# facebookresearch/robust_cvd

Hardware: NVIDIA H100
Metric: flow_residual_constraints_per_sec_per_gn_iteration (higher is better)
Workload: dtype f64

## Files before the change

include/rcvd_hooks.h:

```cpp
#ifndef RCVD_HOOKS_H_
#define RCVD_HOOKS_H_
#include "rcvd.h"
#ifdef __cplusplus
extern "C" {
#endif

int64_t rcvd_launch_count(rcvd_problem* p);
int64_t rcvd_filter_launch_count(void);
int64_t rcvd_builder_launch_count(void);
int64_t rcvd_static_flag_launch_count(void);
int64_t rcvd_builder_last_rounds(void);

int32_t rcvd_structure_info(rcvd_problem* p, int32_t out[8]);

int32_t rcvd_debug_factor_plan(const rcvd_config* cfg, int32_t np, const int32_t* pairs, int32_t nt, const int32_t* trip_centers,
                               int32_t order_slack, int32_t nranks, int32_t rank, int32_t num_sms,
                               int32_t* order, int32_t* level, int32_t* owner, int32_t* perm, int32_t out[12]);

int32_t rcvd_debug_linear_solve(rcvd_problem* p, const double* S, const double* D2, const double* b, double* y);

int32_t rcvd_debug_solve_matrix(rcvd_problem* p, const double* H, const double* D2, const double* b, double* y);
int32_t rcvd_debug_factor_dense(rcvd_problem* p, int32_t* order, double* L, double* Linv);
int32_t rcvd_debug_linear_paths(rcvd_problem* p, int64_t out[13]);

int32_t rcvd_debug_linear_residual(rcvd_problem* p, double radius, double out[6]);

int32_t rcvd_debug_last_iteration(rcvd_problem* p, double* g, double* xc, double out[2]);

int32_t rcvd_debug_profile_linear(rcvd_problem* p, int32_t reps, double out_ms[8]);
int32_t rcvd_debug_level_profile(rcvd_problem* p, double* out, int32_t max_levels);
int32_t rcvd_debug_fp64_tensor_peak(int32_t device, int32_t shape, double* tflops);

int32_t rcvd_debug_set_fast_path(rcvd_problem* p, int32_t on);
int32_t rcvd_debug_set_overlap(rcvd_problem* p, int32_t on);
int32_t rcvd_debug_set_order_slack(rcvd_problem* p, int32_t slack);
int32_t rcvd_debug_set_eval_only(rcvd_problem* p, int32_t on);
int32_t rcvd_debug_set_distributed(rcvd_problem* p, int32_t on);
int32_t rcvd_distribution_info(rcvd_problem* p, int32_t out[4]);
int32_t rcvd_debug_set_update_kernel(rcvd_problem* p, int32_t tma, int32_t side_items_per_cta);

#ifdef __cplusplus
}
#endif
#endif
```

robust_cvd_b200/csrc/rcvd_api.cu:

```cuda
#include <algorithm>
#include <chrono>
#include <cmath>
#include <cstdarg>
#include <cstdio>
#include <cstring>
#include <dlfcn.h>
#include <limits>
#include <string>
#include <vector>

#include <cub/device/device_segmented_sort.cuh>
#include "rcvd_eval.cuh"
#include "rcvd_linalg.cuh"
#include "rcvd_update.cuh"
#include "rcvd_plan.h"
#include "rcvd_dense.cuh"
#include "rcvd_filter.cuh"
#include "rcvd_bilateral.cuh"
#include "rcvd_builder.cuh"
static int64_t g_filter_launches = 0;

using namespace rcvd;

#define RCVD_API extern "C" __attribute__((visibility("default")))

constexpr int kFastSmem = (3 * kTile * kJsLd + 4 * 256) * (int)sizeof(double);
static bool run_path_ok_host(const rcvd_config& c, const Layout& L);
static bool fast_path_ok_host(const rcvd_config& c, const Layout& L) {
  return L.k == 1 && c.spatial_type == RCVD_SPATIAL_IDENTITY && c.intr_opt != RCVD_INTR_SHARED && !c.fix_poses && !c.fix_depth_xforms &&
         !c.fix_spatial_xforms && (c.depth_type != RCVD_DEPTH_GRID || !c.depth_cubic);
}

static bool run_path_ok_host(const rcvd_config& c, const Layout& L) { return fast_path_ok_host(c, L) && c.depth_type == RCVD_DEPTH_GRID && L.G < 65535; }

static thread_local std::string g_err = "";
static int set_err(int code, const char* fmt, ...) {
  char buf[512]; va_list ap; va_start(ap, fmt); vsnprintf(buf, sizeof(buf), fmt, ap); va_end(ap);
  g_err = buf; return code;
}
#define CK(call) do { cudaError_t e_ = (call); if (e_ != cudaSuccess) return set_err(RCVD_ERR_CUDA, "%s failed: %s (%s:%d)", #call, cudaGetErrorString(e_), __FILE__, __LINE__); } while (0)

struct DevGuard {
  int prev = -1; cudaError_t err = cudaSuccess;
  explicit DevGuard(int d) { if (cudaGetDevice(&prev) != cudaSuccess) prev = -1; err = cudaSetDevice(d); }
  ~DevGuard() { if (prev >= 0) cudaSetDevice(prev); }
};
#define SET_DEVICE(d) DevGuard dev_guard_(d); if (dev_guard_.err != cudaSuccess) return set_err(RCVD_ERR_CUDA, "cudaSetDevice(%d) failed: %s", (int)(d), cudaGetErrorString(dev_guard_.err))

namespace nccl {
typedef struct { char internal[128]; } UniqueId;
typedef void* Comm;
static void* lib = nullptr;
static int (*GetUniqueId)(UniqueId*) = nullptr;
static int (*CommInitRank)(Comm*, int, UniqueId, int) = nullptr;
static int (*AllReduce)(const void*, void*, size_t, int, int, Comm, cudaStream_t) = nullptr;
static int (*CommDestroy)(Comm) = nullptr;
static const char* (*GetErrorString)(int) = nullptr;
static int (*GroupStart)() = nullptr;
static int (*GroupEnd)() = nullptr;
static int (*Broadcast)(const void*, void*, size_t, int, int, Comm, cudaStream_t) = nullptr;
static int (*Reduce)(const void*, void*, size_t, int, int, int, Comm, cudaStream_t) = nullptr;
static bool load() {
  if (lib) return true;
  const char* names[] = {"libnccl.so.2", "libnccl.so"};
  for (const char* n : names) { lib = dlopen(n, RTLD_NOW | RTLD_GLOBAL); if (lib) break; }
  if (!lib) return false;
  GetUniqueId = (int (*)(UniqueId*))dlsym(lib, "ncclGetUniqueId");
  CommInitRank = (int (*)(Comm*, int, UniqueId, int))dlsym(lib, "ncclCommInitRank");
  AllReduce = (int (*)(const void*, void*, size_t, int, int, Comm, cudaStream_t))dlsym(lib, "ncclAllReduce");
  CommDestroy = (int (*)(Comm))dlsym(lib, "ncclCommDestroy");
  GetErrorString = (const char* (*)(int))dlsym(lib, "ncclGetErrorString");
  GroupStart = (int (*)())dlsym(lib, "ncclGroupStart"); GroupEnd = (int (*)())dlsym(lib, "ncclGroupEnd");
  Broadcast = (int (*)(const void*, void*, size_t, int, int, Comm, cudaStream_t))dlsym(lib, "ncclBroadcast");
  Reduce = (int (*)(const void*, void*, size_t, int, int, int, Comm, cudaStream_t))dlsym(lib, "ncclReduce");
  return GetUniqueId && CommInitRank && AllReduce && CommDestroy && GroupStart && GroupEnd && Broadcast && Reduce;
}
constexpr int kFloat64 = 8, kUint8 = 1, kSum = 0, kMax = 2;
}

enum { SC_COST = 0, SC_CAND = 1, SC_GY = 2, SC_YHY = 3, SC_STEP2 = 4, SC_X2 = 5, SC_GMAX = 6, SC_GDOTD = 7, SC_DMAX = 8, SC_N = 16 };

__global__ void k_extract_diag(const double* __restrict__ H, double* __restrict__ diag, int N, int npad) {
  const int i = blockIdx.x * blockDim.x + threadIdx.x;
  if (i >= N * npad) return;
  const int f = i / npad, l = i % npad;
  diag[i] = H[(size_t)f * npad * npad + (size_t)l * npad + l];
}
__global__ void k_jacobi_scale(const double* __restrict__ diag, double* __restrict__ S, int n, int enable) {
  const int i = blockIdx.x * blockDim.x + threadIdx.x;
  if (i < n) S[i] = enable ? 1.0 / (1.0 + sqrt(diag[i])) : 1.0;
}
__global__ void k_lm_prepare(const double* __restrict__ diagH, const double* __restrict__ S, const double* __restrict__ g, double* __restrict__ lmdiag,
                             double* __restrict__ D2, double* __restrict__ gs, int n, int reuse, double radius, double dmin, double dmax) {
  const int i = blockIdx.x * blockDim.x + threadIdx.x;
  if (i >= n) return;
  const double s = S[i];
  double d = lmdiag[i];
  if (!reuse) { d = fmin(fmax(s * s * diagH[i], dmin), dmax); lmdiag[i] = d; }
  D2[i] = d / radius;
  gs[i] = s * g[i];
}
__global__ void k_mul(const double* __restrict__ a, const double* __restrict__ b, double* __restrict__ o, int n) {
  const int i = blockIdx.x * blockDim.x + threadIdx.x;
  if (i < n) o[i] = a[i] * b[i];
}
__device__ __forceinline__ double project_lb(const rcvd_config& c, const Layout& L, const uint8_t* in_range, int f, int l, double v) {
  if (c.depth_lower_bound && l >= L.offD && l < L.offS && ((l - L.offD) % L.k) == 0 && in_range[f]) return fmax(v, 0.0);
  return v;
}
__global__ void __launch_bounds__(256) k_state_norms(rcvd_config cfg, Layout L, const uint8_t* __restrict__ in_range, const uint8_t* __restrict__ active,
                                                      const double* __restrict__ x, const double* __restrict__ g, double* __restrict__ scal, int N) {
  const int i = blockIdx.x * blockDim.x + threadIdx.x;
  double x2 = 0.0, gm = 0.0;
  if (i < N * L.nf) {
    const int f = i / L.nf, l = i % L.nf;
    const size_t v = (size_t)f * L.npad + l;
    if (active[v]) {
      x2 = x[i] * x[i];
      gm = fabs(x[i] - project_lb(cfg, L, in_range, f, l, x[i] - g[v]));
    }
  }
  x2 = warp_sum(x2);
#pragma unroll
  for (int o = 16; o > 0; o >>= 1) gm = fmax(gm, __shfl_xor_sync(0xffffffffu, gm, o));
  if ((threadIdx.x & 31) == 0) {
    red_add(scal + SC_X2, x2);
    atomicMax((unsigned long long*)(scal + SC_GMAX), (unsigned long long)__double_as_longlong(gm));
  }
}
__global__ void __launch_bounds__(256) k_dot2(const double* __restrict__ a, const double* __restrict__ b, const double* __restrict__ c,
                                               const double* __restrict__ d, int n, double* __restrict__ scal, int s0, int s1) {
  const int i = blockIdx.x * blockDim.x + threadIdx.x;
  double p = 0.0, q = 0.0;
  if (i < n) { p = a[i] * b[i]; q = c[i] * d[i]; }
  p = warp_sum(p); q = warp_sum(q);
  if ((threadIdx.x & 31) == 0) { red_add(scal + s0, p); red_add(scal + s1, q); }
}
__global__ void k_finalize_mask(rcvd_config cfg, Layout L, uint8_t* __restrict__ mask, int N) {
  const int i = blockIdx.x * blockDim.x + threadIdx.x;
  if (i >= N * L.npad) return;
  const int l = i % L.npad;
  if (l >= L.nf || is_const_local(cfg, L, l)) mask[i] = 0;
}
__global__ void k_project_state(rcvd_config cfg, Layout L, const uint8_t* __restrict__ in_range, double* __restrict__ x, int N) {
  const int i = blockIdx.x * blockDim.x + threadIdx.x;
  if (i < N * L.nf) x[i] = project_lb(cfg, L, in_range, i / L.nf, i % L.nf, x[i]);
}
__global__ void k_h_to_dense(const double* __restrict__ H, const HBlock* __restrict__ hb, int nblocks, double* __restrict__ out, int N, int nf, int npad, const int* __restrict__ uperm) {
  const int b = blockIdx.y;
  const int e = blockIdx.x * blockDim.x + threadIdx.x;
  if (e >= nf * nf) return;
  const int i = e / nf, j = e % nf;
  const HBlock hbk = hb[b];
  if (hbk.r == hbk.c && j > i) return;
  const double v = H[(size_t)b * npad * npad + (size_t)i * npad + j];
  const size_t U = (size_t)N * nf;
  const int ur = uperm[hbk.r], uc = uperm[hbk.c];
  out[((size_t)ur * nf + i) * U + (size_t)uc * nf + j] = v;
  out[((size_t)uc * nf + j) * U + (size_t)ur * nf + i] = v;
}

enum { LP_POTRF_SMEM = 0, LP_POTRF_PANEL, LP_TRSM_LL4, LP_TRSM_LL2, LP_TRSM_GEMM, LP_UPD_TMA1, LP_UPD_TMA2, LP_UPD_GEMM, LP_SUB_LEVEL, LP_SUB_FUSED,
       LP_TRINV, LP_OTHER, LP_UPD_TMA1_MULTI, LP_N };

struct rcvd_problem {
  rcvd_config cfg; Layout L; int N = 0; int device = 0;
  cudaStream_t stream = nullptr;
  std::vector<uint8_t> in_range; std::vector<double> median, adaptive;
  std::vector<int32_t> pair_frames; std::vector<int64_t> offsets; std::vector<float> records_h;
  std::vector<int32_t> struct_pairs;
  std::vector<int32_t> trip_centers; std::vector<int64_t> trip_offsets; std::vector<float> trip_records;
  float* d_trip_records = nullptr; int32_t *d_trip_tile_center = nullptr, *d_trip_tile_count = nullptr; int64_t* d_trip_tile_begin = nullptr; int num_trip_tiles = 0;
  int first_frame = 0, last_frame = -1;
  float* d_records = nullptr; int32_t *d_tile_pair = nullptr, *d_tile_count = nullptr, *d_pair_frames = nullptr, *d_blk_of = nullptr;
  int64_t* d_tile_begin = nullptr; uint8_t *d_in_range = nullptr, *d_active = nullptr;
  double *d_median = nullptr, *d_adaptive = nullptr; float* d_scale_locs = nullptr; int nscale = 0;
  int num_tiles = 0; int64_t C = 0;
  double *d_x = nullptr, *d_xc = nullptr, *d_xsave = nullptr;
  double *d_g = nullptr, *d_S = nullptr, *d_diagH = nullptr, *d_lmdiag = nullptr, *d_D2 = nullptr, *d_gs = nullptr, *d_rhs = nullptr, *d_ytmp = nullptr,
         *d_y = nullptr, *d_Sy = nullptr, *d_Hy = nullptr, *d_partial = nullptr, *d_scal = nullptr;
  double* h_scal = nullptr;
  int npartial = 0;
  double *d_H = nullptr, *d_Lb = nullptr, *d_T = nullptr, *d_invL = nullptr, *d_invT = nullptr;
  HBlock *d_hblocks = nullptr, *d_lblocks = nullptr; int* d_fail = nullptr;
  FactorPlan plan;
  int *d_lvl_frames = nullptr; GemmTask *d_trsm_tasks = nullptr, *d_upd_tasks = nullptr; int2 *d_trsm_pairs = nullptr, *d_upd_pairs = nullptr;
  SubTask* d_sub_tasks = nullptr; int* d_sub_counters = nullptr; int* d_sub_need = nullptr;
  SolveTask* d_fwd_tasks = nullptr; TrsmTask* d_trsm_ll = nullptr; bool use_trsm_ll = false;
  cudaGraphExec_t solve_graph = nullptr;
  bool structure_ready = false, constraints_set = false, frames_set = false;
  int nranks = 1, rank = 0; nccl::Comm comm = nullptr;
  int64_t launches = 0, graph_launches = 0;
  std::vector<double> h_state; bool state_dirty = false; bool use_fast = true; bool overlap = true; int order_slack = 4;
  cudaStream_t side_stream = nullptr; cudaEvent_t ev_fork = nullptr, ev_join = nullptr;
  double *d_g2 = nullptr, *d_delta = nullptr; int* h_fail = nullptr;
  cudaEvent_t ev[8] = {nullptr};
  std::vector<void*> allocs;
  std::vector<std::pair<int, cudaEvent_t>>* prof = nullptr;
  bool eval_only = false;
  bool records_sorted = false;
  bool dist_enabled = true, graph_warm = false, force_full_H = false;
  int *d_lvl_own = nullptr, *d_own_lblocks = nullptr, *d_own_hblocks = nullptr, *d_uperm = nullptr;
  UpdItem* d_upd_items = nullptr; CUtensorMap tmapT; bool gemm_tma = true, tmap_ok = false; int num_sms = 0, upd_ipc = 0;
  std::vector<double> level_ms;
  bool factored = false;
  int64_t paths[LP_N] = {0}, graph_paths[LP_N] = {0};
  rcvd_problem() {}
};

template <class T> static int dalloc(rcvd_problem* p, T** ptr, size_t count) {
  *ptr = nullptr;
  if (count == 0) count = 1;
  cudaError_t e = cudaMallocAsync((void**)ptr, count * sizeof(T), p->stream);
  if (e != cudaSuccess) return set_err(RCVD_ERR_CUDA, "cudaMallocAsync(%zu bytes) failed: %s", count * sizeof(T), cudaGetErrorString(e));
  p->allocs.push_back(*ptr);
  return RCVD_OK;
}
template <class T> static int upload(rcvd_problem* p, T** ptr, const std::vector<T>& v) {
  int rc = dalloc(p, ptr, v.size()); if (rc) return rc;
  if (!v.empty()) CK(cudaMemcpyAsync(*ptr, v.data(), v.size() * sizeof(T), cudaMemcpyHostToDevice, p->stream));
  return RCVD_OK;
}
static void free_all(rcvd_problem* p) {
  if (p->solve_graph) { cudaGraphExecDestroy(p->solve_graph); p->solve_graph = nullptr; }
  if (p->side_stream) cudaStreamSynchronize(p->side_stream);
  for (void* q : p->allocs) cudaFreeAsync(q, p->stream);
  p->allocs.clear();
  if (p->stream) cudaStreamSynchronize(p->stream);
  if (p->h_scal) { cudaFreeHost(p->h_scal); p->h_scal = nullptr; }
  p->structure_ready = false; p->factored = false;
}

static DevProblem dev_problem(const rcvd_problem* p) {
  DevProblem d; d.cfg = p->cfg; d.L = p->L; d.N = p->N; d.num_tiles = p->num_tiles; d.num_constraints = p->C;
  d.records = p->d_records; d.tile_pair = p->d_tile_pair; d.tile_begin = p->d_tile_begin; d.tile_count = p->d_tile_count;
  d.pair_frames = p->d_pair_frames; d.blk_of = p->d_blk_of; d.in_range = p->d_in_range; d.median = p->d_median;
  d.adaptive = p->adaptive.empty() ? nullptr : p->d_adaptive; d.scale_locs = p->d_scale_locs; d.num_scale_locs = p->nscale;
  d.rank = p->rank; d.nranks = p->nranks;
  d.trip_records = p->d_trip_records; d.trip_tile_center = p->d_trip_tile_center; d.trip_tile_begin = p->d_trip_tile_begin; d.trip_tile_count = p->d_trip_tile_count; d.num_trip_tiles = p->num_trip_tiles;
  return d;
}

#define UP(ptr, vec) if ((rc = upload(p, &(ptr), vec))) return rc
#define DA(ptr, n) if ((rc = dalloc(p, &(ptr), (n)))) return rc
static int upload_plan(rcvd_problem* p) {
  const FactorPlan& pl = p->plan; int rc;
  UP(p->d_blk_of, pl.blk_of); UP(p->d_hblocks, pl.hblocks); UP(p->d_lblocks, pl.lblocks); UP(p->d_lvl_frames, pl.lvl_frames); UP(p->d_lvl_own, pl.lvl_own);
  UP(p->d_own_lblocks, pl.own_lblocks); UP(p->d_own_hblocks, pl.own_hblocks); UP(p->d_uperm, pl.uperm);
  UP(p->d_trsm_tasks, pl.trsm_tasks); UP(p->d_upd_tasks, pl.upd_tasks); UP(p->d_trsm_pairs, pl.trsm_pairs); UP(p->d_upd_pairs, pl.upd_pairs);
  UP(p->d_sub_tasks, pl.sub_tasks); UP(p->d_sub_need, pl.sub_need); DA(p->d_sub_counters, (size_t)4 * p->N + 4);
  UP(p->d_fwd_tasks, pl.fwd_tasks); UP(p->d_trsm_ll, pl.trsm_ll); UP(p->d_upd_items, pl.upd_items);
  return RCVD_OK;
}

static int set_up_problem_data(rcvd_problem* p) {
  const int N = p->N; const Layout& L = p->L; const std::vector<int>& uperm = p->plan.uperm; int rc;
  const int np = (int)(p->pair_frames.size() / 2);
  std::vector<int32_t> tile_pair, tile_count; std::vector<int64_t> tile_begin;
  for (int i = 0; i < np; ++i)
    for (int64_t b = p->offsets[i]; b < p->offsets[i + 1]; b += kTile) { tile_pair.push_back(i); tile_begin.push_back(b); tile_count.push_back((int32_t)std::min<int64_t>(kTile, p->offsets[i + 1] - b)); }
  p->num_tiles = (int)tile_pair.size(); p->C = p->offsets.empty() ? 0 : p->offsets.back();
  UP(p->d_tile_pair, tile_pair); UP(p->d_tile_begin, tile_begin); UP(p->d_tile_count, tile_count);
  {
    std::vector<int32_t> pf_int(p->pair_frames.size());
    for (size_t i = 0; i < pf_int.size(); ++i) pf_int[i] = p->plan.iperm[p->pair_frames[i]];
    UP(p->d_pair_frames, pf_int); UP(p->d_records, p->records_h);
  }
  p->records_sorted = false;
  if (run_path_ok_host(p->cfg, L) && p->C > 0 && p->C < (int64_t)0x7fffffff) {
    const long long n = p->C;
    unsigned *d_k0 = nullptr, *d_k1 = nullptr; int *d_i0 = nullptr, *d_i1 = nullptr; float* d_sorted = nullptr; int64_t* d_off = nullptr; void* d_tmp = nullptr;
    int rcs;
    if ((rcs = dalloc(p, &d_k0, (size_t)n)) || (rcs = dalloc(p, &d_k1, (size_t)n)) || (rcs = dalloc(p, &d_i0, (size_t)n)) || (rcs = dalloc(p, &d_i1, (size_t)n)) || (rcs = dalloc(p, &d_sorted, (size_t)n * 6)) ||
        (rcs = upload(p, &d_off, p->offsets))) return rcs;
    k_record_keys<<<(unsigned)((n + 255) / 256), 256, 0, p->stream>>>(p->cfg, p->d_records, n, d_k0, d_i0);
    size_t tmp_bytes = 0;
    CK(cub::DeviceSegmentedSort::SortPairs(nullptr, tmp_bytes, d_k0, d_k1, d_i0, d_i1, (int)n, np, d_off, d_off + 1, p->stream));
    CK(cudaMallocAsync(&d_tmp, std::max<size_t>(tmp_bytes, 16), p->stream));
    CK(cub::DeviceSegmentedSort::SortPairs(d_tmp, tmp_bytes, d_k0, d_k1, d_i0, d_i1, (int)n, np, d_off, d_off + 1, p->stream));
    k_gather_records<<<(unsigned)((n * 6 + 255) / 256), 256, 0, p->stream>>>(p->d_records, d_i1, n, d_sorted);
    CK(cudaFreeAsync(d_tmp, p->stream));
    CK(cudaGetLastError());
    p->d_records = d_sorted; p->records_sorted = true;
  }
  {
    std::vector<int32_t> tc, tn; std::vector<int64_t> tb;
    for (size_t i = 0; i < p->trip_centers.size(); ++i)
      for (int64_t b = p->trip_offsets[i]; b < p->trip_offsets[i + 1]; b += kTile) { tc.push_back(p->trip_centers[i]); tb.push_back(b); tn.push_back((int32_t)std::min<int64_t>(kTile, p->trip_offsets[i + 1] - b)); }
    p->num_trip_tiles = (int)tc.size();
    UP(p->d_trip_tile_center, tc); UP(p->d_trip_tile_begin, tb); UP(p->d_trip_tile_count, tn); UP(p->d_trip_records, p->trip_records);
  }
  {
    std::vector<uint8_t> ir(N); std::vector<double> md(N), ad;
    for (int i = 0; i < N; ++i) { ir[i] = p->in_range[uperm[i]]; md[i] = p->median[uperm[i]]; }
    UP(p->d_in_range, ir); UP(p->d_median, md);
    if (!p->adaptive.empty()) {
      const size_t G = p->adaptive.size() / N; ad.resize(p->adaptive.size());
      for (int i = 0; i < N; ++i) std::copy(p->adaptive.begin() + (size_t)uperm[i] * G, p->adaptive.begin() + (size_t)(uperm[i] + 1) * G, ad.begin() + (size_t)i * G);
      UP(p->d_adaptive, ad);
    }
  }
  {
    std::vector<float> locs; const int gx = p->cfg.scale_grid_x, gy = p->cfg.scale_grid_y;
    for (int y = 0; y < gy; ++y) for (int x = 0; x < gx; ++x) {
      const float fx = -1.f + 2.f * x / (gx - 1);
      const float fy = -1.f + 2.f * y / (gy - 1);
      locs.push_back(fx); locs.push_back(fy);
    }
    p->nscale = (int)(locs.size() / 2);
    UP(p->d_scale_locs, locs);
  }
  p->first_frame = 0; p->last_frame = -1;
  { bool any = false; for (int f = 0; f < N; ++f) if (p->in_range[f]) { if (!any) { p->first_frame = f; any = true; } p->last_frame = f; } }
  return RCVD_OK;
}
#undef UP

static int allocate_storage(rcvd_problem* p) {
  const int N = p->N; const Layout& L = p->L; const int npad = L.npad, nLoff = p->plan.nLoff; const size_t bs = (size_t)npad * npad; int rc;
  const size_t Upad = (size_t)N * npad, U = (size_t)N * L.nf;
  DA(p->d_x, U); DA(p->d_xc, U); DA(p->d_xsave, U);
  DA(p->d_g, 2 * Upad + 8); p->d_diagH = p->d_g + Upad + 8;
  DA(p->d_S, Upad); DA(p->d_lmdiag, Upad); DA(p->d_D2, Upad); DA(p->d_gs, Upad); DA(p->d_rhs, Upad);
  DA(p->d_g2, Upad + 8); DA(p->d_delta, Upad);
  DA(p->d_ytmp, Upad); DA(p->d_y, Upad); DA(p->d_Sy, Upad); DA(p->d_Hy, Upad); DA(p->d_scal, SC_N); DA(p->d_active, Upad); DA(p->d_fail, 1);
  const RegCounts rcn = reg_counts(p->cfg, L, N, p->nscale);
  p->npartial = p->num_tiles + (rcn.total + 127) / 128 + p->num_trip_tiles + 1;
  DA(p->d_partial, (size_t)p->npartial);
  if (p->eval_only) { DA(p->d_H, 1); DA(p->d_Lb, 1); DA(p->d_T, 1); DA(p->d_invL, 1); DA(p->d_invT, 1); }
  else {
    DA(p->d_H, p->plan.hblocks.size() * bs); DA(p->d_Lb, (size_t)(N + nLoff) * bs); DA(p->d_T, (size_t)std::max(nLoff, 1) * bs);
    DA(p->d_invL, (size_t)N * bs); DA(p->d_invT, (size_t)N * npad * 16);
  }
#undef DA
  {
    p->tmap_ok = false;
    typedef CUresult (*EncodeFn)(CUtensorMap*, CUtensorMapDataType, cuuint32_t, void*, const cuuint64_t*, const cuuint64_t*, const cuuint32_t*, const cuuint32_t*,
                                 CUtensorMapInterleave, CUtensorMapSwizzle, CUtensorMapL2promotion, CUtensorMapFloatOOBfill);
    void* fn = nullptr; cudaDriverEntryPointQueryResult qres;
    if (cudaGetDriverEntryPoint("cuTensorMapEncodeTiled", &fn, cudaEnableDefault, &qres) == cudaSuccess && fn && qres == cudaDriverEntryPointSuccess) {
      const cuuint64_t gdim[2] = {(cuuint64_t)npad, (cuuint64_t)std::max(nLoff, 1) * npad};
      const cuuint64_t gstr[1] = {(cuuint64_t)npad * sizeof(double)};
      const cuuint32_t box[2] = {16u, (cuuint32_t)p->plan.upd_rb};
      const cuuint32_t estr[2] = {1u, 1u};
      const CUresult r = ((EncodeFn)fn)(&p->tmapT, CU_TENSOR_MAP_DATA_TYPE_FLOAT64, 2, p->d_T, gdim, gstr, box, estr, CU_TENSOR_MAP_INTERLEAVE_NONE,
                                        CU_TENSOR_MAP_SWIZZLE_128B, CU_TENSOR_MAP_L2_PROMOTION_L2_128B, CU_TENSOR_MAP_FLOAT_OOB_FILL_NONE);
      p->tmap_ok = (r == CUDA_SUCCESS);
    }
    cudaGetLastError();
    if (p->tmap_ok) { CK(cudaFuncSetAttribute(k_update_tma<1>, cudaFuncAttributeMaxDynamicSharedMemorySize, (int)upd_smem_bytes(p->plan.upd_rb, 1))); CK(cudaFuncSetAttribute(k_update_tma<2>, cudaFuncAttributeMaxDynamicSharedMemorySize, (int)upd_smem_bytes(p->plan.upd_rb, 2))); }
    else if (p->gemm_tma) return set_err(RCVD_ERR_CUDA, "cuTensorMapEncodeTiled unavailable or failed: the TMA update kernel cannot run");
  }
  CK(cudaMallocHost((void**)&p->h_scal, (SC_N + 2) * sizeof(double)));
  p->h_fail = (int*)(p->h_scal + SC_N);
  CK(cudaMemsetAsync(p->d_x, 0, U * sizeof(double), p->stream));
  CK(cudaMemsetAsync(p->d_lmdiag, 0, Upad * sizeof(double), p->stream));
  CK(cudaMemsetAsync(p->d_S, 0, Upad * sizeof(double), p->stream));
  CK(cudaMemsetAsync(p->d_active, 0, Upad, p->stream));
  DevProblem d = dev_problem(p);
  if (p->num_tiles > 0) k_mark_static<<<p->num_tiles, kTile, 0, p->stream>>>(d, p->d_active);
  if (rcn.total > 0) {
    DevProblem d1 = d; d1.nranks = 1; d1.rank = 0;
    k_regularisers<2><<<(rcn.total + 127) / 128, 128, 0, p->stream>>>(d1, rcn, p->d_x, nullptr, nullptr, nullptr, p->d_active, p->first_frame, p->last_frame);
  }
  if (p->num_trip_tiles > 0) k_triplets<2><<<p->num_trip_tiles, kTile, 0, p->stream>>>(d, p->d_x, nullptr, nullptr, nullptr, p->d_active);
  k_finalize_mask<<<(int)((Upad + 255) / 256), 256, 0, p->stream>>>(p->cfg, L, p->d_active, N);
  CK(cudaGetLastError());
  if (p->nranks > 1) {
    const int r = nccl::AllReduce(p->d_active, p->d_active, Upad, nccl::kUint8, nccl::kMax, p->comm, p->stream);
    if (r != 0) return set_err(RCVD_ERR_NCCL, "ncclAllReduce(active mask) failed");
  }
  if ((npad * 16 + 16 * (npad + 1)) * (int)sizeof(double) > 220 * 1024) return set_err(RCVD_ERR_INVALID, "frame block too large for the panel-inverse kernel (npad=%d)", npad);
  CK(cudaFuncSetAttribute(k_trinv, cudaFuncAttributeMaxDynamicSharedMemorySize, (npad * 16 + 16 * (npad + 1)) * (int)sizeof(double)));
  CK(cudaFuncSetAttribute(k_accumulate_fast, cudaFuncAttributeMaxDynamicSharedMemorySize, kFastSmem));
  CK(cudaFuncSetAttribute(k_accumulate_runs, cudaFuncAttributeMaxDynamicSharedMemorySize, kRunSmem));
  p->use_trsm_ll = trsm_ll_smem_bytes(npad) <= 220 * 1024;
  if (p->use_trsm_ll) { CK(cudaFuncSetAttribute(k_trsm_ll<2>, cudaFuncAttributeMaxDynamicSharedMemorySize, (int)trsm_ll_smem_bytes(npad, 2))); if (trsm_ll_smem_bytes(npad, 4) <= 220 * 1024) CK(cudaFuncSetAttribute(k_trsm_ll<4>, cudaFuncAttributeMaxDynamicSharedMemorySize, (int)trsm_ll_smem_bytes(npad, 4))); }
  if (potrf_smem_bytes(npad) <= 220 * 1024) CK(cudaFuncSetAttribute(k_potrf_smem, cudaFuncAttributeMaxDynamicSharedMemorySize, (int)potrf_smem_bytes(npad)));
  return RCVD_OK;
}

static int build_structure(rcvd_problem* p) {
  free_all(p);
  CK(cudaSetDevice(p->device));
  if (const char* e = make_factor_plan(p->plan, p->cfg, p->struct_pairs.empty() ? p->pair_frames : p->struct_pairs, p->trip_centers, p->order_slack,
                                       p->nranks, p->rank, p->dist_enabled, p->num_sms))
    return set_err(RCVD_ERR_INVALID, "%s", e);
  int rc;
  if ((rc = upload_plan(p)) || (rc = set_up_problem_data(p)) || (rc = allocate_storage(p))) return rc;
  CK(cudaStreamSynchronize(p->stream));
  p->structure_ready = true;
  return RCVD_OK;
}

static int allreduce(rcvd_problem* p, double* buf, size_t count) {
  if (p->nranks <= 1) return RCVD_OK;
  const int r = nccl::AllReduce(buf, buf, count, nccl::kFloat64, nccl::kSum, p->comm, p->stream);
  if (r != 0) return set_err(RCVD_ERR_NCCL, "ncclAllReduce failed: %s", nccl::GetErrorString ? nccl::GetErrorString(r) : "?");
  return RCVD_OK;
}
struct Seg { size_t first, count; };
static int grouped(rcvd_problem* p, double* base, size_t unit, const std::vector<Seg>& segs, bool bcast) {
  int r = nccl::GroupStart();
  for (size_t i = 0; i < segs.size() && r == 0; ++i) {
    if (segs[i].count == 0) continue;
    const int root = (int)(i % (size_t)p->nranks);
    double* ptr = base + segs[i].first * unit;
    r = bcast ? nccl::Broadcast(ptr, ptr, segs[i].count * unit, nccl::kFloat64, root, p->comm, p->stream)
              : nccl::Reduce(ptr, ptr, segs[i].count * unit, nccl::kFloat64, nccl::kSum, root, p->comm, p->stream);
  }
  const int r2 = nccl::GroupEnd();
  if (r == 0) r = r2;
  if (r != 0) return set_err(RCVD_ERR_NCCL, "grouped NCCL %s failed: %s", bcast ? "broadcast" : "reduce", nccl::GetErrorString ? nccl::GetErrorString(r) : "?");
  return RCVD_OK;
}

static int enqueue_factor_solve(rcvd_problem* p) {
  const Layout& L = p->L; const int N = p->N, npad = L.npad; cudaStream_t st = p->stream;
  const int nL = N + p->plan.nLoff;
  const int tiles = (npad + 63) / 64;
  enum { P_LOAD = 0, P_POTRF, P_TRINV, P_TRSM, P_GEMM, P_SOLVE };
  int prof_level = 0;
  auto mark = [&](int cls) {
    if (!p->prof) return;
    cudaEvent_t e; cudaEventCreate(&e); cudaEventRecord(e, st); p->prof->push_back({cls < 0 ? cls : (cls | (prof_level << 8)), e});
  };
  const int neff = std::min(npad, (L.nf + 7) / 8 * 8);
  auto gemm = [&](cudaStream_t cs, int ntasks, double* dstp, const double* A, const double* B, const GemmTask* tasks, const int2* prs, double alpha, double beta) {
    k_gemm_nt<<<dim3(tiles, tiles, ntasks), 128, 0, cs>>>(dstp, A, B, tasks, prs, npad, beta != 0.0 ? neff : npad, alpha, beta);
  };
  mark(-1);
  k_load_factor<<<dim3((npad * npad + 255) / 256, p->plan.dist ? (int)p->plan.own_lblocks.size() : nL), 256, 0, st>>>(p->d_H, p->d_Lb, p->d_lblocks, p->d_S, p->d_D2, npad, L.nf, p->plan.dist ? p->d_own_lblocks : nullptr);
  p->launches += 1; p->paths[LP_OTHER]++; mark(P_LOAD);
  cudaStream_t side = p->side_stream;
  bool side_pending = false, side_used = false;
  const size_t bsz = (size_t)npad * npad;
  auto phase_boundary = [&]() -> int {
    if (side_pending || side_used) { CK(cudaEventRecord(p->ev_join, side)); CK(cudaStreamWaitEvent(st, p->ev_join, 0)); side_pending = false; }
    std::vector<Seg> inv, tr;
    for (int q = 0; q < p->nranks; ++q) inv.push_back({(size_t)p->plan.fa_off[q], (size_t)p->plan.fa_cnt[q]});
    for (int q = 0; q < p->nranks; ++q) tr.push_back({(size_t)p->plan.fb_off[q], (size_t)p->plan.fb_cnt[q]});
    for (int q = 0; q < p->nranks; ++q) tr.push_back({(size_t)N + (size_t)p->plan.bseg[2 * q], (size_t)p->plan.bseg[2 * q + 1]});
    int rc = grouped(p, p->d_invL, bsz, inv, true); if (rc) return rc;
    return grouped(p, p->d_Lb, bsz, tr, true);
  };
  for (size_t li = 0; li < p->plan.levels.size(); ++li) {
    const Level& lv = p->plan.levels[li]; prof_level = (int)li;
    if (p->plan.dist && (int)li == p->plan.LB) { int rc = phase_boundary(); if (rc) return rc; }
    const int* lframes = p->d_lvl_own + lv.own_off; const int nfr = lv.nown;
    if (nfr > 0) {
    if (potrf_smem_bytes(npad) <= 220 * 1024) {
      k_potrf_smem<<<nfr, kPotrfSmemThreads, potrf_smem_bytes(npad), st>>>(p->d_Lb, p->d_invT, lframes, npad, p->d_fail);
      p->paths[LP_POTRF_SMEM]++;
    } else {
      const int nt16 = npad / 16;
      for (int jb = 0; jb < nt16; ++jb) {
        k_potrf_panel<<<nfr, kPotrfThreads, 0, st>>>(p->d_Lb, p->d_invT, lframes, npad, jb, p->d_fail);
        p->launches += 1; p->paths[LP_POTRF_PANEL]++;
        const int m = npad - (jb + 1) * 16;
        if (m > 0) { const int n64 = (m + 63) / 64; k_potrf_trail<<<dim3(n64 * (n64 + 1) / 2, nfr), 128, 0, st>>>(p->d_Lb, lframes, npad, jb); p->launches += 1; p->paths[LP_OTHER]++; }
      }
      p->launches -= 1;
    }
    p->launches += 1; mark(P_POTRF);
    if (p->use_trsm_ll) {
      cudaStream_t is = st;
      if (p->overlap) { CK(cudaEventRecord(p->ev_fork, st)); CK(cudaStreamWaitEvent(side, p->ev_fork, 0)); is = side; side_used = true; }
      k_trinv<<<dim3(npad / 16, nfr), 256, (npad * 16 + 16 * (npad + 1)) * sizeof(double), is>>>(p->d_Lb, p->d_invT, p->d_invL, lframes, npad);
      p->launches += 1; p->paths[LP_TRINV]++; mark(P_TRINV);
      if (lv.ntrsm > 0) {
        const int strips = (npad + kTrsmStrip - 1) / kTrsmStrip;
        if (strips * lv.ntrsm <= p->num_sms && trsm_ll_smem_bytes(npad, 4) <= 220 * 1024) {
          k_trsm_ll<4><<<dim3(strips, lv.ntrsm), 128, trsm_ll_smem_bytes(npad, 4), st>>>(p->d_T, p->d_Lb, p->d_invT, p->d_trsm_ll + lv.trsm_off, npad);
          p->paths[LP_TRSM_LL4]++;
        } else {
          k_trsm_ll<2><<<dim3(strips, lv.ntrsm), 128, trsm_ll_smem_bytes(npad, 2), st>>>(p->d_T, p->d_Lb, p->d_invT, p->d_trsm_ll + lv.trsm_off, npad);
          p->paths[LP_TRSM_LL2]++;
        }
        p->launches++; mark(P_TRSM);
      }
    } else {
      k_trinv<<<dim3(npad / 16, nfr), 256, (npad * 16 + 16 * (npad + 1)) * sizeof(double), st>>>(p->d_Lb, p->d_invT, p->d_invL, lframes, npad);
      p->launches += 1; p->paths[LP_TRINV]++; mark(P_TRINV);
      if (lv.ntrsm > 0) { gemm(st, lv.ntrsm, p->d_T, p->d_Lb, p->d_invL, p->d_trsm_tasks + lv.trsm_off, p->d_trsm_pairs, 1.0, 0.0); p->launches++; p->paths[LP_TRSM_GEMM]++; mark(P_TRSM); }
    }
    }
    if (p->plan.dist && (int)li < p->plan.LB) {
      std::vector<Seg> segs;
      for (int q = 0; q < p->nranks; ++q) segs.push_back({(size_t)p->plan.tseg[(li * p->nranks + q) * 2], (size_t)p->plan.tseg[(li * p->nranks + q) * 2 + 1]});
      int rc = grouped(p, p->d_T, bsz, segs, true); if (rc) return rc;
    }
    if (lv.nupd2 > 0 && p->overlap) {
      CK(cudaEventRecord(p->ev_fork, st)); CK(cudaStreamWaitEvent(side, p->ev_fork, 0));
    }
    if (side_pending) { CK(cudaStreamWaitEvent(st, p->ev_join, 0)); side_pending = false; }
    auto update = [&](cudaStream_t cs, int off, int n) {
      if (n <= p->num_sms) {
        k_update_tma<2><<<n, UpdShape<2>::threads, upd_smem_bytes(p->plan.upd_rb, 2), cs>>>(p->tmapT, p->d_Lb, p->d_upd_items + off, n, p->d_upd_pairs, npad, p->plan.upd_neff, p->plan.upd_rb, 0);
        p->paths[LP_UPD_TMA2]++;
      } else {
        int grid = std::min(n, 2 * p->num_sms);
        if (p->upd_ipc > 0) grid = std::max(grid, (n + p->upd_ipc - 1) / p->upd_ipc);
        k_update_tma<1><<<grid, UpdShape<1>::threads, upd_smem_bytes(p->plan.upd_rb, 1), cs>>>(p->tmapT, p->d_Lb, p->d_upd_items + off, n, p->d_upd_pairs, npad, p->plan.upd_neff, p->plan.upd_rb, 0);
        p->paths[LP_UPD_TMA1]++; if (grid < n) p->paths[LP_UPD_TMA1_MULTI]++;
      }
    };
    if (p->gemm_tma) {
      if (lv.nit > 0) { update(st, lv.it_off, lv.nit); p->launches++; mark(P_GEMM); }
      if (lv.nit2 > 0) {
        update(p->overlap ? side : st, lv.it2_off, lv.nit2); p->launches++; mark(P_GEMM);
        if (p->overlap) { CK(cudaEventRecord(p->ev_join, side)); side_pending = true; side_used = true; }
      }
      continue;
    }
    if (lv.nupd > 0) { gemm(st, lv.nupd, p->d_Lb, p->d_T, p->d_T, p->d_upd_tasks + lv.upd_off, p->d_upd_pairs, -1.0, 1.0); p->launches++; p->paths[LP_UPD_GEMM]++; mark(P_GEMM); }
    if (lv.nupd2 > 0) {
      gemm(p->overlap ? side : st, lv.nupd2, p->d_Lb, p->d_T, p->d_T, p->d_upd_tasks + lv.upd2_off, p->d_upd_pairs, -1.0, 1.0); p->launches++; p->paths[LP_UPD_GEMM]++; mark(P_GEMM);
      if (p->overlap) { CK(cudaEventRecord(p->ev_join, side)); side_pending = true; side_used = true; }
    }
  }
  if (p->plan.dist && p->plan.LB >= (int)p->plan.levels.size()) { int rc = phase_boundary(); if (rc) return rc; }
  if (side_pending || side_used) { CK(cudaEventRecord(p->ev_join, side)); CK(cudaStreamWaitEvent(st, p->ev_join, 0)); }
  CK(cudaMemcpyAsync(p->d_rhs, p->d_gs, (size_t)N * npad * sizeof(double), cudaMemcpyDeviceToDevice, st));
  const int nlv = (int)p->plan.levels.size();
  const int LS = p->plan.sub_first_level;
  for (int l = 0; l < LS; ++l) {
    const Level& lv = p->plan.levels[l];
    k_fwd_diag<<<dim3((npad + 7) / 8, lv.nframes), 256, 0, st>>>(p->d_invL, p->d_rhs, p->d_ytmp, p->d_lvl_frames + lv.frame_off, npad);
    p->launches++; p->paths[LP_SUB_LEVEL]++;
    if (lv.nfwd > 0) { k_fwd_update<<<dim3((npad + 7) / 8, lv.nfwd), 256, 0, st>>>(p->d_T, p->d_ytmp, p->d_rhs, p->d_fwd_tasks + lv.fwd_off, npad); p->launches++; p->paths[LP_SUB_LEVEL]++; }
  }
  if (LS < nlv && !p->plan.sub_tasks.empty()) {
    CK(cudaMemsetAsync(p->d_sub_counters, 0, ((size_t)4 * N + 4) * sizeof(int), st));
    SubCounters cn; cn.ticket = p->d_sub_counters; cn.fin = p->d_sub_counters + 4; cn.fdone = cn.fin + N; cn.bin = cn.fdone + N; cn.bdone = cn.bin + N;
    cn.fin_need = p->d_sub_need; cn.bin_need = p->d_sub_need + N;
    k_substitution<<<std::min((int)p->plan.sub_tasks.size(), p->num_sms), kSubThreads, substitution_smem_bytes(npad), st>>>(p->d_invL, p->d_T, p->d_rhs, p->d_ytmp, p->d_y, p->d_sub_tasks, (int)p->plan.sub_tasks.size(), cn, npad);
    p->launches++; p->paths[LP_SUB_FUSED]++;
  }
  for (int l = LS - 1; l >= 0; --l) {
    const Level& lv = p->plan.levels[l];
    if (lv.nfwd > 0) { k_bwd_update<<<dim3((npad + 31) / 32, lv.nfwd), 256, 0, st>>>(p->d_T, p->d_y, p->d_ytmp, p->d_fwd_tasks + lv.fwd_off, npad); p->launches++; p->paths[LP_SUB_LEVEL]++; }
    k_bwd_diag<<<dim3((npad + 31) / 32, lv.nframes), 256, 0, st>>>(p->d_invL, p->d_ytmp, p->d_y, p->d_lvl_frames + lv.frame_off, npad);
    p->launches += 1; p->paths[LP_SUB_LEVEL]++;
  }
  mark(P_SOLVE);
  CK(cudaGetLastError());
  return RCVD_OK;
}

static int factor_solve(rcvd_problem* p) {
  if (p->nranks > 1 && !p->graph_warm) {
    p->graph_warm = true; p->factored = true;
    return enqueue_factor_solve(p);
  }
  if (!p->solve_graph) {
    cudaGraph_t graph;
    const int64_t l0 = p->launches;
    int64_t paths0[LP_N]; std::copy(p->paths, p->paths + LP_N, paths0);
    CK(cudaStreamBeginCapture(p->stream, cudaStreamCaptureModeThreadLocal));
    int rc = enqueue_factor_solve(p);
    cudaError_t e = cudaStreamEndCapture(p->stream, &graph);
    for (int i = 0; i < LP_N; ++i) { p->graph_paths[i] = p->paths[i] - paths0[i]; p->paths[i] = paths0[i]; }
    if (rc) return rc;
    if (e != cudaSuccess) return set_err(RCVD_ERR_CUDA, "graph capture failed: %s", cudaGetErrorString(e));
    CK(cudaGraphInstantiate(&p->solve_graph, graph, 0));
    cudaGraphDestroy(graph);
    p->graph_launches = p->launches - l0;
    p->launches = l0;
  }
  CK(cudaGraphLaunch(p->solve_graph, p->stream));
  p->launches += p->graph_launches;
  for (int i = 0; i < LP_N; ++i) p->paths[i] += p->graph_paths[i];
  p->factored = true;
  return RCVD_OK;
}


static int enqueue_evaluate(rcvd_problem* p, const double* x, bool wantG, bool wantH, double* gout, int slot) {
  if (wantH && p->eval_only) return set_err(RCVD_ERR_INVALID, "this handle was set to evaluation-only (rcvd_debug_set_eval_only): no normal matrix");
  const Layout& L = p->L; const int N = p->N, npad = L.npad; cudaStream_t st = p->stream;
  const size_t bs = (size_t)npad * npad, Upad = (size_t)N * npad;
  DevProblem d = dev_problem(p);
  const RegCounts rcn = reg_counts(p->cfg, L, N, p->nscale);
  const int regblocks = (rcn.total + 127) / 128;
  if (wantH) CK(cudaMemsetAsync(p->d_H, 0, p->plan.hblocks.size() * bs * sizeof(double), st));
  if (wantG) CK(cudaMemsetAsync(gout, 0, (Upad + 8) * sizeof(double), st));
  if (p->num_tiles > 0) {
    if (wantH && p->use_fast && p->records_sorted) k_accumulate_runs<<<p->num_tiles, kTile, kRunSmem, st>>>(d, x, p->d_H, gout, p->d_partial);
    else if (wantH && p->use_fast && fast_path_ok_host(p->cfg, L)) k_accumulate_fast<<<p->num_tiles, kTile, kFastSmem, st>>>(d, x, p->d_H, gout, p->d_partial);
    else if (wantH) k_accumulate_generic<true><<<p->num_tiles, kTile, 0, st>>>(d, x, p->d_H, gout, p->d_partial);
    else if (wantG) k_accumulate_generic<false><<<p->num_tiles, kTile, 0, st>>>(d, x, nullptr, gout, p->d_partial);
    else k_cost_static<<<p->num_tiles, kTile, 0, st>>>(d, x, p->d_partial);
    p->launches++;
  }
  if (regblocks > 0) {
    double* part = p->d_partial + p->num_tiles;
    if (wantH) k_regularisers<1><<<regblocks, 128, 0, st>>>(d, rcn, x, p->d_H, gout, part, nullptr, p->first_frame, p->last_frame);
    else if (wantG) k_regularisers<3><<<regblocks, 128, 0, st>>>(d, rcn, x, nullptr, gout, part, nullptr, p->first_frame, p->last_frame);
    else k_regularisers<0><<<regblocks, 128, 0, st>>>(d, rcn, x, nullptr, nullptr, part, nullptr, p->first_frame, p->last_frame);
    p->launches++;
  }
  if (p->num_trip_tiles > 0) {
    double* part = p->d_partial + p->num_tiles + regblocks;
    if (wantH) k_triplets<1><<<p->num_trip_tiles, kTile, 0, st>>>(d, x, p->d_H, gout, part, nullptr);
    else if (wantG) k_triplets<3><<<p->num_trip_tiles, kTile, 0, st>>>(d, x, nullptr, gout, part, nullptr);
    else k_triplets<0><<<p->num_trip_tiles, kTile, 0, st>>>(d, x, nullptr, nullptr, part, nullptr);
    p->launches++;
  }
  k_reduce_partials<<<1, 1024, 0, st>>>(p->d_partial, p->num_tiles + regblocks + p->num_trip_tiles, p->d_scal, slot);
  p->launches++;
  CK(cudaGetLastError());
  if (p->nranks > 1) {
    int rc;
    if (wantG) {
      CK(cudaMemcpyAsync(gout + Upad, p->d_scal + slot, sizeof(double), cudaMemcpyDeviceToDevice, st));
      size_t cnt = Upad + 8;
      if (wantH && gout == p->d_g) { k_extract_diag<<<(int)((Upad + 255) / 256), 256, 0, st>>>(p->d_H, p->d_diagH, N, npad); p->launches++; cnt = 2 * Upad + 8; }
      if ((rc = allreduce(p, gout, cnt))) return rc;
      CK(cudaMemcpyAsync(p->d_scal + slot, gout + Upad, sizeof(double), cudaMemcpyDeviceToDevice, st));
    } else if ((rc = allreduce(p, p->d_scal + slot, 1))) return rc;
    if (wantH) {
      if (p->plan.dist && !p->force_full_H) {
        std::vector<Seg> segs;
        for (int q = 0; q < p->nranks; ++q) segs.push_back({(size_t)p->plan.fa_off[q], (size_t)(p->plan.fa_cnt[q] + p->plan.fb_cnt[q])});
        for (int q = 0; q < p->nranks; ++q) segs.push_back({(size_t)p->plan.hseg[2 * q], (size_t)p->plan.hseg[2 * q + 1]});
        if ((rc = grouped(p, p->d_H, bs, segs, false))) return rc;
      } else if ((rc = allreduce(p, p->d_H, p->plan.hblocks.size() * bs))) return rc;
    }
  }
  return RCVD_OK;
}

static int upload_frames(rcvd_problem* p, double* dst, const double* src_user, int stride_dst, int stride_src, int count) {
  std::vector<double> tmp((size_t)p->N * stride_dst, 0.0);
  for (int i = 0; i < p->N; ++i) memcpy(tmp.data() + (size_t)i * stride_dst, src_user + (size_t)p->plan.uperm[i] * stride_src, (size_t)count * sizeof(double));
  CK(cudaMemcpyAsync(dst, tmp.data(), tmp.size() * sizeof(double), cudaMemcpyHostToDevice, p->stream));
  CK(cudaStreamSynchronize(p->stream));
  return RCVD_OK;
}
static int download_frames(rcvd_problem* p, double* dst_user, const double* src, int stride_dst, int stride_src, int count) {
  std::vector<double> tmp((size_t)p->N * stride_src);
  CK(cudaMemcpyAsync(tmp.data(), src, tmp.size() * sizeof(double), cudaMemcpyDeviceToHost, p->stream));
  CK(cudaStreamSynchronize(p->stream));
  for (int i = 0; i < p->N; ++i) memcpy(dst_user + (size_t)p->plan.uperm[i] * stride_dst, tmp.data() + (size_t)i * stride_src, (size_t)count * sizeof(double));
  return RCVD_OK;
}
static int save_state(rcvd_problem* p) {
  DevGuard g(p->device); cudaStreamSynchronize(p->stream);
  if (p->h_state.size() != (size_t)p->N * p->L.nf) p->h_state.assign((size_t)p->N * p->L.nf, 0.0);
  return download_frames(p, p->h_state.data(), p->d_x, p->L.nf, p->L.nf, p->L.nf);
}

static int ensure_ready(rcvd_problem* p) {
  if (!p->structure_ready) {
    if (p->offsets.empty()) { p->offsets.assign(1, 0); }
    if (p->in_range.empty()) p->in_range.assign(p->N, 1);
    if (p->median.empty()) p->median.assign(p->N, 1.0);
    int rc = build_structure(p); if (rc) return rc;
    p->state_dirty = true;
  }
  if (p->state_dirty) {
    if (p->h_state.size() != (size_t)p->N * p->L.nf) p->h_state.assign((size_t)p->N * p->L.nf, 0.0);
    { int rc = upload_frames(p, p->d_x, p->h_state.data(), p->L.nf, p->L.nf, p->L.nf); if (rc) return rc; }
    p->state_dirty = false;
  }
  return RCVD_OK;
}

static int read_scalars(rcvd_problem* p) {
  CK(cudaMemcpyAsync(p->h_scal, p->d_scal, SC_N * sizeof(double), cudaMemcpyDeviceToHost, p->stream));
  CK(cudaMemcpyAsync(p->h_fail, p->d_fail, sizeof(int), cudaMemcpyDeviceToHost, p->stream));
  CK(cudaStreamSynchronize(p->stream));
  return RCVD_OK;
}

// ... 125 lines not shown
  CK(cudaMemcpyAsync(p->d_xsave, p->d_x, U * sizeof(double), cudaMemcpyDeviceToDevice, st));

  auto full_eval = [&]() -> int {
    CK(cudaMemsetAsync(p->d_scal, 0, SC_N * sizeof(double), st));
    CK(cudaEventRecord(p->ev[0], st));
    int r = enqueue_evaluate(p, p->d_x, true, true, p->d_g, SC_COST); if (r) return r;
    CK(cudaEventRecord(p->ev[1], st));
    if (p->nranks <= 1) k_extract_diag<<<nblk(Upad), 256, 0, st>>>(p->d_H, p->d_diagH, N, npad);
    k_state_norms<<<nblk(U), 256, 0, st>>>(p->cfg, L, p->d_in_range, p->d_active, p->d_x, p->d_g, p->d_scal, N);
    p->launches += 2;
    r = read_scalars(p); if (r) return r;
    sum.eval_ms += ev_ms(p->ev[0], p->ev[1]);
    return RCVD_OK;
  };
  if ((rc = full_eval())) return rc;
  double xCost = p->h_scal[SC_COST], xNorm = std::sqrt(p->h_scal[SC_X2]), gmax = p->h_scal[SC_GMAX];
  sum.initial_cost = xCost;
  k_jacobi_scale<<<nblk(Upad), 256, 0, st>>>(p->d_diagH, p->d_S, (int)Upad, o.jacobi_scaling);
  p->launches++;
  double radius = o.initial_radius, decrease = 2.0; bool reuseDiag = false;
  double minimumCost = xCost;
  int iter = 0, invalid = 0; bool stepSuccessful = true;
  auto finish = [&](int term, const char* msg) { sum.termination = term; snprintf(sum.message, sizeof(sum.message), "%s", msg); };
  finish(RCVD_TERM_NO_CONVERGENCE, "");
  if (o.verbose) fprintf(stderr, "[rcvd] iter      cost      cost_change  |gradient|   |step|    tr_ratio  tr_radius\n[rcvd] %4d %.6e %10.2e %10.2e %10.2e %10.2e %10.2e\n", 0, xCost, 0.0, gmax, 0.0, 0.0, radius);
  for (;;) {
    if (stepSuccessful) {
      ++sum.num_successful_steps;
      if (xCost < minimumCost || iter == 0) { minimumCost = xCost; CK(cudaMemcpyAsync(p->d_xsave, p->d_x, U * sizeof(double), cudaMemcpyDeviceToDevice, st)); }
    } else ++sum.num_unsuccessful_steps;
    if (iter >= o.max_iterations) { finish(RCVD_TERM_NO_CONVERGENCE, "Maximum number of iterations reached."); break; }
    if (stepSuccessful && gmax <= o.gradient_tolerance) { finish(RCVD_TERM_CONVERGENCE, "Gradient tolerance reached."); break; }
    if (radius <= o.min_radius) { finish(RCVD_TERM_CONVERGENCE, "Minimum trust region radius reached."); break; }
    ++iter; stepSuccessful = false;
    CK(cudaMemsetAsync(p->d_scal, 0, SC_N * sizeof(double), st));
    CK(cudaMemsetAsync(p->d_fail, 0, sizeof(int), st));
    CK(cudaEventRecord(p->ev[2], st));
    k_lm_prepare<<<nblk(Upad), 256, 0, st>>>(p->d_diagH, p->d_S, p->d_g, p->d_lmdiag, p->d_D2, p->d_gs, (int)Upad, reuseDiag ? 1 : 0, radius, o.min_lm_diagonal, o.max_lm_diagonal);
    p->launches++;
    reuseDiag = true;
    if ((rc = factor_solve(p))) return rc;
    if ((rc = enqueue_model_terms(p))) return rc;
    CK(cudaEventRecord(p->ev[3], st));
    double alpha = 1.0;
    if (!constrained) {
      if ((rc = enqueue_candidate(p, 1.0, p->d_g))) return rc;
      if ((rc = enqueue_evaluate(p, p->d_xc, false, false, nullptr, SC_CAND))) return rc;
      CK(cudaEventRecord(p->ev[4], st));
    }
    if ((rc = read_scalars(p))) return rc;
    sum.linear_ms += ev_ms(p->ev[2], p->ev[3]);
    if (!constrained) sum.cost_ms += ev_ms(p->ev[3], p->ev[4]);
    const double gy = p->h_scal[SC_GY], yHy = p->h_scal[SC_YHY];
    const double modelChange = gy - 0.5 * yHy;
    const bool ok = (*p->h_fail == 0) && std::isfinite(gy) && std::isfinite(yHy);
    if (!(ok && modelChange > 0.0)) {
      if (++invalid >= o.max_consecutive_invalid_steps) { finish(RCVD_TERM_FAILURE, "Number of consecutive invalid steps more than max_num_consecutive_invalid_steps."); break; }
      radius = radius / decrease; decrease *= 2.0; reuseDiag = true;
      if (o.verbose) fprintf(stderr, "[rcvd] %4d invalid step (fail=%d model=%g), radius %.3e\n", iter, *p->h_fail, modelChange, radius);
      continue;
    }
    invalid = 0;
    if (constrained) {
      auto trial = [&](double a, ls::Sample& s) -> int {
        CK(cudaMemsetAsync(p->d_scal, 0, SC_N * sizeof(double), st));
        int r = enqueue_candidate(p, a, p->d_g); if (r) return r;
        r = enqueue_evaluate(p, p->d_xc, true, false, p->d_g2, SC_CAND); if (r) return r;
        k_dot2<<<nblk(Upad), 256, 0, st>>>(p->d_g2, p->d_delta, p->d_g2, p->d_delta, (int)Upad, p->d_scal, SC_GY, SC_YHY);
        p->launches++;
        r = read_scalars(p); if (r) return r;
        s.x = a; s.value = p->h_scal[SC_CAND]; s.valueValid = std::isfinite(s.value);
        s.gradient = p->h_scal[SC_GY]; s.gradValid = s.valueValid && std::isfinite(s.gradient);
        return RCVD_OK;
      };
      ls::Sample cur, prev{0, 0, 0, false, false};
      if ((rc = trial(1.0, cur))) return rc;
      const double gd = p->h_scal[SC_GDOTD], dirMax = p->h_scal[SC_DMAX];
      ls::Sample init{0.0, xCost, gd, true, true};
      int lsIter = 0; bool success = true;
      while (!cur.valueValid || cur.value > xCost + 1e-4 * gd * cur.x) {
        if (++lsIter >= 20) { success = false; break; }
        const double lo = 1e-3 * cur.x, hi = 0.6 * cur.x;
        double ss;
        if (!cur.valueValid) ss = std::min(std::max(cur.x * 0.5, lo), hi);
        else { std::vector<ls::Sample> sm{init, cur}; if (prev.valueValid) sm.push_back(prev); ss = ls::minimizeInterpolating(sm, lo, hi); }
        if (ss * dirMax < 1e-9) { success = false; break; }
        prev = cur;
        if ((rc = trial(ss, cur))) return rc;
      }
      alpha = success ? cur.x : 1.0;
      CK(cudaMemsetAsync(p->d_scal, 0, SC_N * sizeof(double), st));
      if ((rc = enqueue_candidate(p, alpha, p->d_g))) return rc;
      if ((rc = enqueue_evaluate(p, p->d_xc, false, false, nullptr, SC_CAND))) return rc;
      if ((rc = read_scalars(p))) return rc;
    }
    double candCost = p->h_scal[SC_CAND];
    if (!std::isfinite(candCost)) candCost = std::numeric_limits<double>::max();
    const double stepNorm = std::sqrt(p->h_scal[SC_STEP2]);
    if (stepNorm <= o.parameter_tolerance * (xNorm + o.parameter_tolerance)) { finish(RCVD_TERM_CONVERGENCE, "Parameter tolerance reached."); break; }
    const double costChange = xCost - candCost;
    if (std::fabs(costChange) <= o.function_tolerance * xCost) { finish(RCVD_TERM_CONVERGENCE, "Function tolerance reached."); break; }
    const double relDecrease = (candCost >= std::numeric_limits<double>::max()) ? std::numeric_limits<double>::lowest() : costChange / modelChange;
    if (relDecrease > o.min_relative_decrease) {
      std::swap(p->d_x, p->d_xc);
      if ((rc = full_eval())) return rc;
      xCost = p->h_scal[SC_COST]; xNorm = std::sqrt(p->h_scal[SC_X2]); gmax = p->h_scal[SC_GMAX];
      stepSuccessful = true;
      radius = radius / std::max(1.0 / 3.0, 1.0 - std::pow(2.0 * relDecrease - 1.0, 3));
      radius = std::min(o.max_radius, radius); decrease = 2.0; reuseDiag = false;
    } else {
      radius = radius / decrease; decrease *= 2.0; reuseDiag = true;
    }
    if (o.verbose) fprintf(stderr, "[rcvd] %4d %.6e %10.2e %10.2e %10.2e %10.2e %10.2e\n", iter, stepSuccessful ? xCost : candCost, costChange, gmax, stepNorm, relDecrease, radius);
  }
  CK(cudaMemcpyAsync(p->d_x, p->d_xsave, U * sizeof(double), cudaMemcpyDeviceToDevice, st));
  CK(cudaStreamSynchronize(st));
  sum.iterations = iter; sum.final_cost = minimumCost;
  sum.gpu_launches = p->launches - launches0;
  sum.total_ms = std::chrono::duration<double, std::milli>(clk::now() - t0).count();
  return RCVD_OK;
}

RCVD_API const char* rcvd_last_error(void) { return g_err.c_str(); }
RCVD_API int32_t rcvd_abi_version(void) { return 1; }
RCVD_API int32_t rcvd_frame_stride(const rcvd_config* c) { Layout L; return (c && make_layout(*c, L)) ? L.nf : -1; }
RCVD_API int32_t rcvd_depth_param_offset(const rcvd_config* c) { Layout L; return (c && make_layout(*c, L)) ? L.offD : -1; }
RCVD_API int32_t rcvd_spatial_param_offset(const rcvd_config* c) { Layout L; return (c && make_layout(*c, L)) ? L.offS : -1; }
RCVD_API void rcvd_default_solve_options(rcvd_solve_options* o) {
  o->max_iterations = 1000; o->verbose = 0; o->function_tolerance = 1e-6; o->gradient_tolerance = 1e-10; o->parameter_tolerance = 1e-8;
  o->initial_radius = 1e4; o->max_radius = 1e16; o->min_radius = 1e-32; o->min_relative_decrease = 1e-3; o->min_lm_diagonal = 1e-6;
  o->max_lm_diagonal = 1e32; o->max_consecutive_invalid_steps = 5; o->jacobi_scaling = 1;
}

RCVD_API int32_t rcvd_problem_create(const rcvd_config* cfg, int32_t device, rcvd_problem** out) {
  if (!cfg || !out) return set_err(RCVD_ERR_INVALID, "null argument");
  Layout L;
  if (!make_layout(*cfg, L) || cfg->num_frames <= 0) return set_err(RCVD_ERR_INVALID, "unsupported transform configuration");
  int ndev = 0;
  cudaError_t e = cudaGetDeviceCount(&ndev);
  if (e != cudaSuccess || ndev <= 0 || device < 0 || device >= ndev)
    return set_err(RCVD_ERR_NO_DEVICE, "no usable CUDA device (%s); this library has no CPU fallback", e != cudaSuccess ? cudaGetErrorString(e) : "device ordinal out of range");
  SET_DEVICE(device);
  {
    cudaMemPool_t pool; unsigned long long keep = ~0ull;
    if (cudaDeviceGetDefaultMemPool(&pool, device) == cudaSuccess) cudaMemPoolSetAttribute(pool, cudaMemPoolAttrReleaseThreshold, &keep);
  }
  rcvd_problem* p = new rcvd_problem();
  p->cfg = *cfg; p->L = L; p->N = cfg->num_frames; p->device = device;
  e = cudaDeviceGetAttribute(&p->num_sms, cudaDevAttrMultiProcessorCount, device);
  if (e != cudaSuccess) { delete p; return set_err(RCVD_ERR_CUDA, "cudaDeviceGetAttribute(multiprocessor count): %s", cudaGetErrorString(e)); }
  int prio_lo = 0, prio_hi = 0; cudaDeviceGetStreamPriorityRange(&prio_lo, &prio_hi);
  e = cudaStreamCreateWithPriority(&p->stream, cudaStreamNonBlocking, prio_hi);
  if (e == cudaSuccess) e = cudaStreamCreateWithPriority(&p->side_stream, cudaStreamNonBlocking, prio_lo);
  if (e == cudaSuccess) e = cudaEventCreateWithFlags(&p->ev_fork, cudaEventDisableTiming);
  if (e == cudaSuccess) e = cudaEventCreateWithFlags(&p->ev_join, cudaEventDisableTiming);
  if (e != cudaSuccess) { delete p; return set_err(RCVD_ERR_CUDA, "cudaStreamCreate: %s", cudaGetErrorString(e)); }
  *out = p; return RCVD_OK;
}
RCVD_API void rcvd_problem_destroy(rcvd_problem* p) {
  if (!p) return;
  DevGuard dev_guard_(p->device);
  free_all(p);
  for (int i = 0; i < 8; ++i) if (p->ev[i]) cudaEventDestroy(p->ev[i]);
  if (p->comm && nccl::CommDestroy) nccl::CommDestroy(p->comm);
  if (p->ev_fork) cudaEventDestroy(p->ev_fork);
  if (p->ev_join) cudaEventDestroy(p->ev_join);
  if (p->side_stream) cudaStreamDestroy(p->side_stream);
  if (p->stream) cudaStreamDestroy(p->stream);
  delete p;
}
RCVD_API int32_t rcvd_problem_set_frames(rcvd_problem* p, const uint8_t* in_range, const double* median, const double* adaptive) {
  if (!p) return set_err(RCVD_ERR_INVALID, "null problem");
  if (in_range) p->in_range.assign(in_range, in_range + p->N); else p->in_range.assign(p->N, 1);
  if (median) p->median.assign(median, median + p->N); else p->median.assign(p->N, 1.0);
  if (adaptive && p->cfg.depth_type == RCVD_DEPTH_GRID) p->adaptive.assign(adaptive, adaptive + (size_t)p->N * p->cfg.depth_grid_x * p->cfg.depth_grid_y); else p->adaptive.clear();
  if (p->cfg.adaptive_deform > 0.0 && p->adaptive.empty()) return set_err(RCVD_ERR_INVALID, "adaptive deformation cost requires node weights");
  if (p->structure_ready) { int rc_ = save_state(p); if (rc_) return rc_; }
  p->structure_ready = false;
  return RCVD_OK;
}
RCVD_API int32_t rcvd_problem_set_constraints(rcvd_problem* p, int32_t np, const int32_t* pf, const int64_t* off, const float* rec) {
  if (!p || np < 0 || (np > 0 && (!pf || !off))) return set_err(RCVD_ERR_INVALID, "bad constraint arrays");
  if (p->structure_ready) { int rc_ = save_state(p); if (rc_) return rc_; }
  p->pair_frames.assign(pf, pf + 2 * (size_t)np);
  if (np > 0) p->offsets.assign(off, off + np + 1); else p->offsets.assign(1, 0);
  for (int i = 0; i < np; ++i) {
    if (p->offsets[i + 1] < p->offsets[i]) return set_err(RCVD_ERR_INVALID, "offsets must be non-decreasing");
    if (pf[2 * i] < 0 || pf[2 * i] >= p->N || pf[2 * i + 1] < 0 || pf[2 * i + 1] >= p->N || pf[2 * i] == pf[2 * i + 1]) return set_err(RCVD_ERR_INVALID, "bad frame pair %d", i);
  }
  const int64_t C = p->offsets.back();
  if (C > 0 && !rec) return set_err(RCVD_ERR_INVALID, "null records");
  p->records_h.assign(rec, rec + (size_t)C * 6);
  p->structure_ready = false;
  return RCVD_OK;
}
RCVD_API int32_t rcvd_problem_set_triplets(rcvd_problem* p, int32_t nt, const int32_t* centers, const int64_t* off, const float* rec) {
  if (!p || nt < 0 || (nt > 0 && (!centers || !off))) return set_err(RCVD_ERR_INVALID, "bad triplet arrays");
  if (p->structure_ready) { int rc_ = save_state(p); if (rc_) return rc_; }
  p->trip_centers.assign(centers, centers + nt);
  if (nt > 0) p->trip_offsets.assign(off, off + nt + 1); else p->trip_offsets.assign(1, 0);
  for (int i = 0; i < nt; ++i) if (p->trip_offsets[i + 1] < p->trip_offsets[i] || centers[i] < 1 || centers[i] + 1 >= p->N) return set_err(RCVD_ERR_INVALID, "bad triplet group %d", i);
  const int64_t n = p->trip_offsets.back();
  if (n > 0 && !rec) return set_err(RCVD_ERR_INVALID, "null triplet records");
  p->trip_records.assign(rec, rec + (size_t)n * 10);
  p->structure_ready = false;
  return RCVD_OK;
}
RCVD_API int32_t rcvd_problem_set_structure(rcvd_problem* p, int32_t np, const int32_t* pf) {
  if (!p) return set_err(RCVD_ERR_INVALID, "null problem");
  p->struct_pairs.assign(pf, pf + 2 * (size_t)np);
  p->structure_ready = false;
  return RCVD_OK;
}
RCVD_API int32_t rcvd_nccl_unique_id(uint8_t out[128]) {
  if (!nccl::load()) return set_err(RCVD_ERR_NCCL, "libnccl.so.2 not found");
  nccl::UniqueId id; const int r = nccl::GetUniqueId(&id);
  if (r != 0) return set_err(RCVD_ERR_NCCL, "ncclGetUniqueId failed (%d)", r);
  memcpy(out, id.internal, 128); return RCVD_OK;
}
RCVD_API int32_t rcvd_problem_init_comm(rcvd_problem* p, int32_t nranks, int32_t rank, const uint8_t uid[128]) {
  if (!p || nranks < 1 || rank < 0 || rank >= nranks) return set_err(RCVD_ERR_INVALID, "bad rank/nranks");
  if (nranks == 1) { p->nranks = 1; p->rank = 0; return RCVD_OK; }
  if (!nccl::load()) return set_err(RCVD_ERR_NCCL, "libnccl.so.2 not found");
  SET_DEVICE(p->device);
  nccl::UniqueId id; memcpy(id.internal, uid, 128);
  const int r = nccl::CommInitRank(&p->comm, nranks, id, rank);
  if (r != 0) return set_err(RCVD_ERR_NCCL, "ncclCommInitRank failed: %s", nccl::GetErrorString ? nccl::GetErrorString(r) : "?");
  p->nranks = nranks; p->rank = rank; p->structure_ready = false;
  return RCVD_OK;
}
RCVD_API int32_t rcvd_problem_set_state(rcvd_problem* p, const double* x) {
  if (!p || !x) return set_err(RCVD_ERR_INVALID, "null argument");
  p->h_state.assign(x, x + (size_t)p->N * p->L.nf); p->state_dirty = true;
  return RCVD_OK;
}
RCVD_API int32_t rcvd_problem_get_state(rcvd_problem* p, double* x) {
  if (!p || !x) return set_err(RCVD_ERR_INVALID, "null argument");
  const size_t U = (size_t)p->N * p->L.nf;
  if (!p->structure_ready || p->state_dirty) { if (p->h_state.size() != U) p->h_state.assign(U, 0.0); memcpy(x, p->h_state.data(), U * sizeof(double)); return RCVD_OK; }
  SET_DEVICE(p->device);
  return download_frames(p, x, p->d_x, p->L.nf, p->L.nf, p->L.nf);
}
RCVD_API int32_t rcvd_evaluate(rcvd_problem* p, double* cost, double* gradient) {
  if (!p || !cost) return set_err(RCVD_ERR_INVALID, "null argument");
  SET_DEVICE(p->device);
  int rc = ensure_ready(p); if (rc) return rc;
  CK(cudaMemsetAsync(p->d_scal, 0, SC_N * sizeof(double), p->stream));
  rc = enqueue_evaluate(p, p->d_x, gradient != nullptr, false, p->d_g, SC_COST); if (rc) return rc;
  rc = read_scalars(p); if (rc) return rc;
  *cost = p->h_scal[SC_COST];
  if (gradient) {
    if ((rc = download_frames(p, gradient, p->d_g, p->L.nf, p->L.npad, p->L.nf))) return rc;
  }
  return RCVD_OK;
}
RCVD_API int32_t rcvd_normal_matrix_dense(rcvd_problem* p, double* Hout) {
  if (!p || !Hout) return set_err(RCVD_ERR_INVALID, "null argument");
  SET_DEVICE(p->device);
  int rc = ensure_ready(p); if (rc) return rc;
  p->force_full_H = true;
  rc = enqueue_evaluate(p, p->d_x, true, true, p->d_g, SC_COST);
  p->force_full_H = false;
  if (rc) return rc;
  const size_t U = (size_t)p->N * p->L.nf;
  double* d_out = nullptr;
  CK(cudaMalloc((void**)&d_out, U * U * sizeof(double)));
  CK(cudaMemsetAsync(d_out, 0, U * U * sizeof(double), p->stream));
  k_h_to_dense<<<dim3(nblk((size_t)p->L.nf * p->L.nf), (int)p->plan.hblocks.size()), 256, 0, p->stream>>>(p->d_H, p->d_hblocks, (int)p->plan.hblocks.size(), d_out, p->N, p->L.nf, p->L.npad, p->d_uperm);
  cudaError_t e = cudaMemcpyAsync(Hout, d_out, U * U * sizeof(double), cudaMemcpyDeviceToHost, p->stream);
  cudaStreamSynchronize(p->stream); cudaFree(d_out);
  if (e != cudaSuccess) return set_err(RCVD_ERR_CUDA, "copy failed: %s", cudaGetErrorString(e));
  return RCVD_OK;
}
static int solve_loaded(rcvd_problem* p, const double* S, const double* D2, const double* b, double* y) {
  const int N = p->N, nf = p->L.nf, npad = p->L.npad; const size_t Upad = (size_t)N * npad;
  std::vector<double> hs(Upad, 1.0), hd(Upad, 1.0), hb(Upad, 0.0);
  for (int f = 0; f < N; ++f) for (int l = 0; l < nf; ++l) { const size_t u = (size_t)p->plan.uperm[f] * nf + l; hs[(size_t)f * npad + l] = S ? S[u] : 1.0; hd[(size_t)f * npad + l] = D2[u]; hb[(size_t)f * npad + l] = b[u]; }
  CK(cudaMemcpyAsync(p->d_S, hs.data(), Upad * 8, cudaMemcpyHostToDevice, p->stream));
  CK(cudaMemcpyAsync(p->d_D2, hd.data(), Upad * 8, cudaMemcpyHostToDevice, p->stream));
  CK(cudaMemcpyAsync(p->d_gs, hb.data(), Upad * 8, cudaMemcpyHostToDevice, p->stream));
  CK(cudaMemsetAsync(p->d_fail, 0, sizeof(int), p->stream));
  int rc = factor_solve(p); if (rc) return rc;
  std::vector<double> hy(Upad);
  CK(cudaMemcpyAsync(hy.data(), p->d_y, Upad * 8, cudaMemcpyDeviceToHost, p->stream));
  rc = read_scalars(p); if (rc) return rc;
  for (int f = 0; f < N; ++f) for (int l = 0; l < nf; ++l) y[(size_t)p->plan.uperm[f] * nf + l] = hy[(size_t)f * npad + l];
  if (*p->h_fail) return set_err(RCVD_ERR_NUMERIC, "factorisation hit a non-positive pivot");
  return RCVD_OK;
}
RCVD_API int32_t rcvd_debug_linear_solve(rcvd_problem* p, const double* S, const double* D2, const double* b, double* y) {
  if (!p) return set_err(RCVD_ERR_INVALID, "null argument");
  SET_DEVICE(p->device);
  int rc = ensure_ready(p); if (rc) return rc;
  rc = enqueue_evaluate(p, p->d_x, true, true, p->d_g, SC_COST); if (rc) return rc;
  return solve_loaded(p, S, D2, b, y);
}
RCVD_API int32_t rcvd_debug_solve_matrix(rcvd_problem* p, const double* H, const double* D2, const double* b, double* y) {
  if (!p || !H || !D2 || !b || !y) return set_err(RCVD_ERR_INVALID, "null argument");
  if (p->nranks > 1) return set_err(RCVD_ERR_INVALID, "rcvd_debug_solve_matrix works on single-GPU handles only");
  if (p->eval_only) return set_err(RCVD_ERR_INVALID, "this handle was set to evaluation-only (rcvd_debug_set_eval_only): no factor storage");
  SET_DEVICE(p->device);
  int rc = ensure_ready(p); if (rc) return rc;
  const int N = p->N, nf = p->L.nf, npad = p->L.npad; const size_t U = (size_t)N * nf, bs = (size_t)npad * npad;
  std::vector<uint8_t> coupled((size_t)N * N, 0);
  for (const HBlock& hb : p->plan.hblocks) { const int a = p->plan.uperm[hb.r], c = p->plan.uperm[hb.c]; coupled[(size_t)a * N + c] = coupled[(size_t)c * N + a] = 1; }
  for (int a = 0; a < N; ++a) for (int c = 0; c < N; ++c) {
    if (coupled[(size_t)a * N + c]) continue;
    for (int i = 0; i < nf; ++i) for (int j = 0; j < nf; ++j)
      if (H[((size_t)a * nf + i) * U + (size_t)c * nf + j] != 0.0)
        return set_err(RCVD_ERR_INVALID, "H couples frames %d and %d, which the problem's frame graph does not couple", a, c);
  }
  std::vector<double> hH(p->plan.hblocks.size() * bs, 0.0);
  for (int h = 0; h < (int)p->plan.hblocks.size(); ++h) {
    const int a = p->plan.uperm[p->plan.hblocks[h].r], c = p->plan.uperm[p->plan.hblocks[h].c];
    for (int i = 0; i < nf; ++i) for (int j = 0; j < nf; ++j) hH[h * bs + (size_t)i * npad + j] = H[((size_t)a * nf + i) * U + (size_t)c * nf + j];
  }
  CK(cudaMemcpyAsync(p->d_H, hH.data(), hH.size() * sizeof(double), cudaMemcpyHostToDevice, p->stream));
  return solve_loaded(p, nullptr, D2, b, y);
}
RCVD_API int32_t rcvd_debug_factor_dense(rcvd_problem* p, int32_t* order, double* L, double* Linv) {
  if (!p || !order || !L) return set_err(RCVD_ERR_INVALID, "null argument");
  if (!p->structure_ready || !p->factored) return set_err(RCVD_ERR_INVALID, "no factorisation has run on this handle");
  if (p->plan.dist) return set_err(RCVD_ERR_INVALID, "the distributed factorisation keeps its blocks on their owners");
  SET_DEVICE(p->device);
  CK(cudaStreamSynchronize(p->side_stream)); CK(cudaStreamSynchronize(p->stream));
  const int N = p->N, nf = p->L.nf, npad = p->L.npad, nT = p->plan.nLoff; const size_t U = (size_t)N * nf, bs = (size_t)npad * npad;
  std::vector<double> hL((size_t)N * bs), hT((size_t)nT * bs);
  CK(cudaMemcpy(hL.data(), p->d_Lb, hL.size() * sizeof(double), cudaMemcpyDeviceToHost));
  if (nT > 0) CK(cudaMemcpy(hT.data(), p->d_T, hT.size() * sizeof(double), cudaMemcpyDeviceToHost));
  std::vector<size_t> off(N);
  for (int q = 0; q < N; ++q) { off[p->plan.elim_order[q]] = (size_t)q * nf; order[q] = p->plan.uperm[p->plan.elim_order[q]]; }
  std::fill(L, L + U * U, 0.0);
  for (int f = 0; f < N; ++f)
    for (int i = 0; i < nf; ++i) for (int j = 0; j <= i; ++j) L[(off[f] + i) * U + off[f] + j] = hL[f * bs + (size_t)i * npad + j];
  for (int t = 0; t < nT; ++t) {
    const HBlock& b = p->plan.lblocks[N + t];
    for (int i = 0; i < nf; ++i) for (int j = 0; j < nf; ++j) L[(off[b.r] + i) * U + off[b.c] + j] = hT[t * bs + (size_t)i * npad + j];
  }
  if (Linv) {
    CK(cudaMemcpy(hL.data(), p->d_invL, hL.size() * sizeof(double), cudaMemcpyDeviceToHost));
    for (int f = 0; f < N; ++f) {
      double* out = Linv + off[f] * nf;
      for (int i = 0; i < nf; ++i) for (int j = 0; j < nf; ++j) out[(size_t)i * nf + j] = j <= i ? hL[f * bs + (size_t)i * npad + j] : 0.0;
    }
  }
  return RCVD_OK;
}
RCVD_API int32_t rcvd_debug_linear_paths(rcvd_problem* p, int64_t out[13]) {
  if (!p || !out) return set_err(RCVD_ERR_INVALID, "null argument");
  static_assert(LP_N == 13, "include/rcvd_hooks.h documents thirteen counters");
  std::copy(p->paths, p->paths + LP_N, out);
  return RCVD_OK;
}
RCVD_API int32_t rcvd_time_accumulate(rcvd_problem* p, int32_t iters, double* ms) {
  if (!p || iters <= 0) return set_err(RCVD_ERR_INVALID, "bad argument");
  SET_DEVICE(p->device);
  int rc = ensure_ready(p); if (rc) return rc;
  for (int i = 0; i < 2; ++i) if (!p->ev[i]) CK(cudaEventCreate(&p->ev[i]));
  if ((rc = enqueue_evaluate(p, p->d_x, true, true, p->d_g, SC_COST))) return rc;
  CK(cudaEventRecord(p->ev[0], p->stream));
  for (int i = 0; i < iters; ++i) if ((rc = enqueue_evaluate(p, p->d_x, true, true, p->d_g, SC_COST))) return rc;
  CK(cudaEventRecord(p->ev[1], p->stream));
  CK(cudaStreamSynchronize(p->stream));
  *ms = ev_ms(p->ev[0], p->ev[1]) / iters;
  return RCVD_OK;
}
RCVD_API int32_t rcvd_time_iteration(rcvd_problem* p, int32_t iters, double radius, double* ms_iter, double* ms_acc, double* ms_lin, double* ms_cost) {
  if (!p || iters <= 0) return set_err(RCVD_ERR_INVALID, "bad argument");
  SET_DEVICE(p->device);
  int rc = ensure_ready(p); if (rc) return rc;
  const int N = p->N, npad = p->L.npad; const size_t Upad = (size_t)N * npad; cudaStream_t st = p->stream;
  for (int i = 0; i < 8; ++i) if (!p->ev[i]) CK(cudaEventCreate(&p->ev[i]));
  double ta = 0, tl = 0, tc = 0, tt = 0;
  for (int it = -1; it < iters; ++it) {
    CK(cudaMemsetAsync(p->d_scal, 0, SC_N * sizeof(double), st));
    CK(cudaMemsetAsync(p->d_fail, 0, sizeof(int), st));
    CK(cudaEventRecord(p->ev[0], st));
    if ((rc = enqueue_evaluate(p, p->d_x, true, true, p->d_g, SC_COST))) return rc;
    if (p->nranks <= 1) k_extract_diag<<<nblk(Upad), 256, 0, st>>>(p->d_H, p->d_diagH, N, npad);
    k_jacobi_scale<<<nblk(Upad), 256, 0, st>>>(p->d_diagH, p->d_S, (int)Upad, 1);
    CK(cudaEventRecord(p->ev[1], st));
    k_lm_prepare<<<nblk(Upad), 256, 0, st>>>(p->d_diagH, p->d_S, p->d_g, p->d_lmdiag, p->d_D2, p->d_gs, (int)Upad, 0, radius, 1e-6, 1e32);
    if ((rc = factor_solve(p))) return rc;
    if ((rc = enqueue_model_terms(p))) return rc;
    CK(cudaEventRecord(p->ev[2], st));
    if ((rc = enqueue_candidate(p, 1.0, p->d_g))) return rc;
    if ((rc = enqueue_evaluate(p, p->d_xc, false, false, nullptr, SC_CAND))) return rc;
    CK(cudaEventRecord(p->ev[3], st));
    if ((rc = read_scalars(p))) return rc;
    if (it >= 0) { ta += ev_ms(p->ev[0], p->ev[1]); tl += ev_ms(p->ev[1], p->ev[2]); tc += ev_ms(p->ev[2], p->ev[3]); tt += ev_ms(p->ev[0], p->ev[3]); }
  }
  *ms_iter = tt / iters; if (ms_acc) *ms_acc = ta / iters; if (ms_lin) *ms_lin = tl / iters; if (ms_cost) *ms_cost = tc / iters;
  return RCVD_OK;
}
RCVD_API int32_t rcvd_debug_last_iteration(rcvd_problem* p, double* g, double* xc, double out[2]) {
  if (!p || !g || !xc || !out) return set_err(RCVD_ERR_INVALID, "null argument");
  if (!p->structure_ready) return set_err(RCVD_ERR_INVALID, "no iteration has run on this handle");
  SET_DEVICE(p->device);
  int rc = read_scalars(p); if (rc) return rc;
  out[0] = p->h_scal[SC_COST]; out[1] = p->h_scal[SC_CAND];
  if ((rc = download_frames(p, g, p->d_g, p->L.nf, p->L.npad, p->L.nf))) return rc;
  return download_frames(p, xc, p->d_xc, p->L.nf, p->L.nf, p->L.nf);
}
RCVD_API int32_t rcvd_debug_profile_linear(rcvd_problem* p, int32_t reps, double out_ms[8]) {
  const bool keep_overlap = reps < 0; if (reps < 0) reps = -reps;
  if (!p || !out_ms || reps == 0) return set_err(RCVD_ERR_INVALID, "bad argument");
  SET_DEVICE(p->device);
  int rc = ensure_ready(p); if (rc) return rc;
  const bool ov = p->overlap; if (!keep_overlap) p->overlap = false;
  for (int i = 0; i < 8; ++i) out_ms[i] = 0.0;
  std::vector<std::pair<int, cudaEvent_t>> evs;
  p->level_ms.assign(p->plan.levels.size() * 6, 0.0);
  for (int r = -1; r < reps; ++r) {
    CK(cudaMemsetAsync(p->d_fail, 0, sizeof(int), p->stream));
    evs.clear(); p->prof = &evs;
    rc = enqueue_factor_solve(p);
    p->prof = nullptr; p->factored = true;
    cudaStreamSynchronize(p->stream); cudaStreamSynchronize(p->side_stream);
    double ngemm = 0;
    for (size_t i = 1; i < evs.size(); ++i) {
      float ms = 0; cudaEventElapsedTime(&ms, evs[i - 1].second, evs[i].second);
      const int cls = evs[i].first < 0 ? -1 : (evs[i].first & 0xff), lvl = evs[i].first < 0 ? 0 : (evs[i].first >> 8);
      if (r >= 0 && cls >= 0 && cls < 6) out_ms[cls] += ms;
      if (cls == 4) ngemm += 1;
      if (r == reps - 1 && cls >= 0 && cls < 6 && p->level_ms.size() >= (size_t)(lvl + 1) * 6) p->level_ms[(size_t)lvl * 6 + cls] += ms;
    }
    for (auto& e : evs) cudaEventDestroy(e.second);
    out_ms[6] = ngemm;
    if (rc) break;
  }
  p->overlap = ov;
  for (int i = 0; i < 6; ++i) out_ms[i] /= reps;
  out_ms[7] = p->plan.upd_flops;
  return rc;
}
template <int SHAPE>
__global__ void k_dmma_peak(double* out, int iters) {
  double c[8][4];
#pragma unroll
  for (int i = 0; i < 8; ++i) { c[i][0] = 0; c[i][1] = 0; c[i][2] = 0; c[i][3] = 0; }
  const double a = threadIdx.x * 1e-3, b = 1.0 + threadIdx.x * 1e-6;
  for (int it = 0; it < iters; ++it) {
#pragma unroll
    for (int i = 0; i < 8; ++i) {
      if (SHAPE == 0) dmma_8x8x4(c[i][0], c[i][1], a, b);
      if (SHAPE == 1) dmma_16x8x4(c[i][0], c[i][1], c[i][2], c[i][3], a, a, b);
      if (SHAPE == 2)
        asm volatile("mma.sync.aligned.m16n8k8.row.col.f64.f64.f64.f64 {%0,%1,%2,%3}, {%4,%4,%4,%4}, {%5,%5}, {%0,%1,%2,%3};"
                     : "+d"(c[i][0]), "+d"(c[i][1]), "+d"(c[i][2]), "+d"(c[i][3]) : "d"(a), "d"(b));
      if (SHAPE == 3)
        asm volatile("mma.sync.aligned.m16n8k16.row.col.f64.f64.f64.f64 {%0,%1,%2,%3}, {%4,%4,%4,%4,%4,%4,%4,%4}, {%5,%5,%5,%5}, {%0,%1,%2,%3};"
                     : "+d"(c[i][0]), "+d"(c[i][1]), "+d"(c[i][2]), "+d"(c[i][3]) : "d"(a), "d"(b));
    }
  }
  double s = 0;
#pragma unroll
  for (int i = 0; i < 8; ++i) s += c[i][0] + c[i][1] + c[i][2] + c[i][3];
  out[(size_t)blockIdx.x * blockDim.x + threadIdx.x] = s;
}
RCVD_API int32_t rcvd_debug_fp64_tensor_peak(int32_t device, int32_t shape, double* tflops) {
  if (!tflops || shape < 0 || shape > 3) return set_err(RCVD_ERR_INVALID, "bad argument");
  int ndev = 0;
  if (cudaGetDeviceCount(&ndev) != cudaSuccess || device < 0 || device >= ndev) return set_err(RCVD_ERR_NO_DEVICE, "no usable CUDA device");
  SET_DEVICE(device);
  cudaDeviceProp prop; CK(cudaGetDeviceProperties(&prop, device));
  const int threads = 512, blocks = prop.multiProcessorCount * 4, iters = 20000 >> shape;
  const double flops_per_mma = 512.0 * (1 << shape);
  double* out = nullptr; CK(cudaMalloc((void**)&out, (size_t)blocks * threads * sizeof(double)));
  cudaEvent_t e0, e1; cudaEventCreate(&e0); cudaEventCreate(&e1);
  double best = 0;
  for (int rep = 0; rep < 4; ++rep) {
    cudaEventRecord(e0);
    switch (shape) {
      case 0: k_dmma_peak<0><<<blocks, threads>>>(out, iters); break;
      case 1: k_dmma_peak<1><<<blocks, threads>>>(out, iters); break;
      case 2: k_dmma_peak<2><<<blocks, threads>>>(out, iters); break;
      default: k_dmma_peak<3><<<blocks, threads>>>(out, iters); break;
    }
    cudaEventRecord(e1); cudaEventSynchronize(e1);
    float ms = 0; cudaEventElapsedTime(&ms, e0, e1);
    const double tf = flops_per_mma * 8 * iters * (double)blocks * (threads / 32) / (ms * 1e-3) / 1e12;
    if (rep > 0 && tf > best) best = tf;
  }
  cudaEventDestroy(e0); cudaEventDestroy(e1); cudaFree(out);
  CK(cudaGetLastError());
  *tflops = best; return RCVD_OK;
}
__global__ void __launch_bounds__(256) k_lin_residual(const double* __restrict__ S, const double* __restrict__ HSy, const double* __restrict__ D2,
                                                       const double* __restrict__ y, const double* __restrict__ gs, const double* __restrict__ g,
                                                       int n, double* __restrict__ out) {
  const int i = blockIdx.x * blockDim.x + threadIdx.x;
  double r2 = 0.0, b2 = 0.0, g2 = 0.0, y2 = 0.0;
  if (i < n) { const double r = S[i] * HSy[i] + D2[i] * y[i] - gs[i]; r2 = r * r; b2 = gs[i] * gs[i]; g2 = g[i] * g[i]; y2 = y[i] * y[i]; }
  r2 = warp_sum(r2); b2 = warp_sum(b2); g2 = warp_sum(g2); y2 = warp_sum(y2);
  if ((threadIdx.x & 31) == 0) { red_add(out + 0, r2); red_add(out + 1, b2); red_add(out + 2, g2); red_add(out + 3, y2); }
}
RCVD_API int32_t rcvd_debug_linear_residual(rcvd_problem* p, double radius, double out[6]) {
  if (!p || !out || !(radius > 0.0)) return set_err(RCVD_ERR_INVALID, "bad argument");
  SET_DEVICE(p->device);
  int rc = ensure_ready(p); if (rc) return rc;
  const int N = p->N, npad = p->L.npad; const size_t Upad = (size_t)N * npad; cudaStream_t st = p->stream;
  CK(cudaMemsetAsync(p->d_scal, 0, SC_N * sizeof(double), st));
  CK(cudaMemsetAsync(p->d_fail, 0, sizeof(int), st));
  if ((rc = enqueue_evaluate(p, p->d_x, true, true, p->d_g, SC_COST))) return rc;
  if (p->nranks <= 1) k_extract_diag<<<nblk(Upad), 256, 0, st>>>(p->d_H, p->d_diagH, N, npad);
  k_jacobi_scale<<<nblk(Upad), 256, 0, st>>>(p->d_diagH, p->d_S, (int)Upad, 1);
  k_lm_prepare<<<nblk(Upad), 256, 0, st>>>(p->d_diagH, p->d_S, p->d_g, p->d_lmdiag, p->d_D2, p->d_gs, (int)Upad, 0, radius, 1e-6, 1e32);
  if ((rc = factor_solve(p))) return rc;
  if ((rc = enqueue_model_terms(p))) return rc;
  if (p->plan.dist && (rc = allreduce(p, p->d_Hy, Upad))) return rc;
  double* d_out = p->d_scal + 9;
  k_lin_residual<<<nblk(Upad), 256, 0, st>>>(p->d_S, p->d_Hy, p->d_D2, p->d_y, p->d_gs, p->d_g, (int)Upad, d_out);
  p->launches += 4;
  if ((rc = read_scalars(p))) return rc;
  const double r2 = p->h_scal[9], b2 = p->h_scal[10];
  out[0] = b2 > 0.0 ? std::sqrt(r2 / b2) : std::sqrt(r2); out[1] = std::sqrt(b2); out[2] = p->h_scal[SC_COST];
  out[3] = std::sqrt(p->h_scal[11]); out[4] = std::sqrt(p->h_scal[12]); out[5] = (double)*p->h_fail;
  return RCVD_OK;
}
RCVD_API int32_t rcvd_debug_level_profile(rcvd_problem* p, double* out, int32_t max_levels) {
  if (!p || !out) return -1;
  const int n = std::min<int>(max_levels, (int)(p->level_ms.size() / 6));
  for (int i = 0; i < n * 6; ++i) out[i] = p->level_ms[i];
  return n;
}
RCVD_API int64_t rcvd_launch_count(rcvd_problem* p) { return p ? p->launches : 0; }
RCVD_API int32_t rcvd_debug_set_order_slack(rcvd_problem* p, int32_t slack) { if (!p) return RCVD_ERR_INVALID; p->order_slack = slack; p->structure_ready = false; return RCVD_OK; }
RCVD_API int32_t rcvd_debug_set_overlap(rcvd_problem* p, int32_t on) { if (!p) return RCVD_ERR_INVALID; p->overlap = on != 0; if (p->solve_graph) { cudaGraphExecDestroy(p->solve_graph); p->solve_graph = nullptr; } return RCVD_OK; }
RCVD_API int32_t rcvd_debug_set_update_kernel(rcvd_problem* p, int32_t tma, int32_t side_items_per_cta) {
  if (!p) return RCVD_ERR_INVALID;
  p->gemm_tma = tma != 0; p->upd_ipc = side_items_per_cta;
  if (p->solve_graph) { cudaGraphExecDestroy(p->solve_graph); p->solve_graph = nullptr; }
  if (p->gemm_tma && !p->tmap_ok) p->structure_ready = false;
  return RCVD_OK;
}
RCVD_API int32_t rcvd_debug_set_eval_only(rcvd_problem* p, int32_t on) { if (!p) return RCVD_ERR_INVALID; p->eval_only = on != 0; p->structure_ready = false; return RCVD_OK; }
RCVD_API int32_t rcvd_debug_set_distributed(rcvd_problem* p, int32_t on) { if (!p) return RCVD_ERR_INVALID; p->dist_enabled = on != 0; if (p->structure_ready) { int rc_ = save_state(p); if (rc_) return rc_; p->state_dirty = true; } p->structure_ready = false; return RCVD_OK; }
RCVD_API int32_t rcvd_distribution_info(rcvd_problem* p, int32_t out[4]) {
  if (!p || !out) return set_err(RCVD_ERR_INVALID, "null argument");
  SET_DEVICE(p->device);
  int rc = ensure_ready(p); if (rc) return rc;
  out[0] = p->plan.dist ? 1 : 0; out[1] = p->plan.LB; out[2] = (int)p->plan.levels.size(); out[3] = p->plan.dist ? p->plan.fa_cnt[p->rank] + p->plan.fb_cnt[p->rank] : p->N;
  return RCVD_OK;
}
RCVD_API int32_t rcvd_debug_set_fast_path(rcvd_problem* p, int32_t on) { if (!p) return RCVD_ERR_INVALID; p->use_fast = on != 0; return RCVD_OK; }
RCVD_API int32_t rcvd_solve(rcvd_problem* p, const rcvd_solve_options* opt, rcvd_solve_summary* summary) {
  if (!p || !summary) return set_err(RCVD_ERR_INVALID, "null argument");
  SET_DEVICE(p->device);
  rcvd_solve_options o; if (opt) o = *opt; else rcvd_default_solve_options(&o);
  return lm_solve(p, o, *summary);
}
RCVD_API int32_t rcvd_debug_factor_plan(const rcvd_config* cfg, int32_t np, const int32_t* pairs, int32_t nt, const int32_t* trip_centers,
                                        int32_t order_slack, int32_t nranks, int32_t rank, int32_t num_sms,
                                        int32_t* order, int32_t* level, int32_t* owner, int32_t* perm, int32_t out[12]) {
  if (!cfg || np < 0 || nt < 0 || (np > 0 && !pairs) || (nt > 0 && !trip_centers) || !order || !level || !owner || !perm || !out)
    return set_err(RCVD_ERR_INVALID, "null or negative argument");
  if (nranks < 1 || rank < 0 || rank >= nranks || num_sms < 1) return set_err(RCVD_ERR_INVALID, "bad rank/nranks/num_sms");
  FactorPlan pl;
  if (const char* e = make_factor_plan(pl, *cfg, std::vector<int32_t>(pairs, pairs + 2 * (size_t)np), std::vector<int32_t>(trip_centers, trip_centers + nt),
                                       order_slack, nranks, rank, true, num_sms))
    return set_err(RCVD_ERR_INVALID, "%s", e);
  const int N = cfg->num_frames;
  for (int i = 0; i < N; ++i) {
    const int f = pl.uperm[i];
    order[i] = pl.uperm[pl.elim_order[i]]; level[f] = pl.level[i]; owner[f] = pl.owner[i]; perm[i] = f;
  }
  int upd = 0; for (const Level& l : pl.levels) upd += l.nupd + l.nupd2;
  const int32_t v[12] = {(int32_t)pl.levels.size(), pl.nLoff, (int32_t)pl.hblocks.size(), upd, (int32_t)pl.upd_items.size(), (int32_t)pl.sub_tasks.size(),
                         pl.dist ? 1 : 0, pl.LB, pl.sub_first_level, (int32_t)pl.own_lblocks.size(), (int32_t)pl.own_hblocks.size(),
                         pl.dist ? pl.fa_cnt[rank] + pl.fb_cnt[rank] : N};
  std::copy(v, v + 12, out);
// ... 410 lines not shown
```

robust_cvd_b200/csrc/rcvd_linalg.cuh:

```cuda
#pragma once
#include "rcvd_device.cuh"

namespace rcvd {

constexpr int kPotrfThreads = 256;

__global__ void __launch_bounds__(kPotrfThreads) k_potrf_panel(double* __restrict__ Lb, double* __restrict__ invT,
                                                                const int* __restrict__ frames, int npad, int jb, int* __restrict__ fail) {
  __shared__ double D[16][17];
  __shared__ double Di[16][17];
  const int frame = frames[blockIdx.x];
  double* A = Lb + (size_t)frame * npad * npad;
  double* iT = invT + (size_t)frame * npad * 16;
  const int tid = threadIdx.x;
  const int j0 = jb * 16;
  {
    const int r = tid >> 4, cc = tid & 15;
    D[r][cc] = (cc <= r) ? A[(size_t)(j0 + r) * npad + j0 + cc] : 0.0;
  }
  __syncthreads();
  if (tid < 32) {
    const int i = tid;
    for (int j = 0; j < 16; ++j) {
      if (i == j) {
        double d = D[j][j];
        for (int q = 0; q < j; ++q) d -= D[j][q] * D[j][q];
        if (!(d > 0.0) || !isfinite(d)) { *fail = 1; d = 1.0; }
        D[j][j] = sqrt(d);
      }
      __syncwarp();
      if (i > j && i < 16) {
        double s = D[i][j];
        for (int q = 0; q < j; ++q) s -= D[i][q] * D[j][q];
        D[i][j] = s / D[j][j];
      }
      __syncwarp();
    }
    if (i < 16) {
      const int cidx = i;
      double xcol[16];
#pragma unroll
      for (int r = 0; r < 16; ++r) {
        double s = (r == cidx) ? 1.0 : 0.0;
#pragma unroll
        for (int q = 0; q < 16; ++q) if (q < r) s -= D[r][q] * xcol[q];
        xcol[r] = (r < cidx) ? 0.0 : s / D[r][r];
      }
#pragma unroll
      for (int r = 0; r < 16; ++r) Di[r][cidx] = xcol[r];
    }
  }
  __syncthreads();
  {
    const int r = tid >> 4, cc = tid & 15;
    A[(size_t)(j0 + r) * npad + j0 + cc] = D[r][cc];
    iT[(size_t)jb * 256 + r * 16 + cc] = Di[r][cc];
  }
  const int below = npad - (j0 + 16);
  for (int rr = tid; rr < below; rr += kPotrfThreads) {
    double a[16], xo[16];
    double* row = A + (size_t)(j0 + 16 + rr) * npad + j0;
#pragma unroll
    for (int q = 0; q < 16; ++q) a[q] = row[q];
#pragma unroll
    for (int cc = 0; cc < 16; ++cc) {
      double s = 0.0;
#pragma unroll
      for (int q = 0; q < 16; ++q) if (q <= cc) s += a[q] * Di[cc][q];
      xo[cc] = s;
    }
#pragma unroll
    for (int q = 0; q < 16; ++q) row[q] = xo[q];
  }
}

constexpr int kPotrfSmemThreads = 512;
constexpr int kTileSz = 256;
__host__ __device__ inline size_t potrf_smem_bytes(int npad) { const int nt = npad / 16; return (size_t)(nt * (nt + 1) / 2 + 1) * kTileSz * sizeof(double); }
__device__ __forceinline__ int swz(int r, int k) { return r * 16 + (k ^ ((r & 3) << 2)); }
__device__ __forceinline__ void cp_async16_fwd(void* smem, const void* gmem) {
  const unsigned sa = (unsigned)__cvta_generic_to_shared(smem);
  asm volatile("cp.async.cg.shared.global [%0], [%1], 16;" ::"r"(sa), "l"(gmem) : "memory");
}
__device__ __forceinline__ void dmma_8x8x4_fwd(double& c0, double& c1, double a, double b) {
  asm volatile("mma.sync.aligned.m8n8k4.row.col.f64.f64.f64.f64 {%0,%1}, {%2}, {%3}, {%0,%1};"
               : "+d"(c0), "+d"(c1) : "d"(a), "d"(b));
}

__device__ __forceinline__ void tile_mma_nt(const double* __restrict__ At, const double* __restrict__ Bt, double acc[2][2][2], int g, int t) {
#pragma unroll
  for (int k4 = 0; k4 < 4; ++k4) {
    double af[2], bf[2];
#pragma unroll
    for (int i = 0; i < 2; ++i) { af[i] = At[swz(i * 8 + g, k4 * 4 + t)]; bf[i] = Bt[swz(i * 8 + g, k4 * 4 + t)]; }
#pragma unroll
    for (int i = 0; i < 2; ++i)
#pragma unroll
      for (int j = 0; j < 2; ++j) dmma_8x8x4_fwd(acc[i][j][0], acc[i][j][1], af[i], bf[j]);
  }
}

#ifdef RCVD_POTRF_PHASES
__device__ long long g_potrf_phase[16];
#define POTRF_PHASE(n) do { if (threadIdx.x == 0 && blockIdx.x == 0) { const long long now_ = clock64(); g_potrf_phase[n] += now_ - last_; last_ = now_; } } while (0)
#define CHOL_PHASE(n) do { if (threadIdx.x == 0 && blockIdx.x == 0) { const long long now_ = clock64(); g_potrf_phase[n] += now_ - cl_; cl_ = now_; } } while (0)
#else
#define CHOL_PHASE(n) do { } while (0)
#define POTRF_PHASE(n) do { } while (0)
#endif

__device__ __forceinline__ void warp_chol16_blocked(double* __restrict__ D, double* __restrict__ pinv, int lane, int* __restrict__ fail) {
  const int g = lane >> 2, t = lane & 3;
  double c[3][2];
  const int ui[3] = {0, 1, 1}, uj[3] = {0, 0, 1};
#pragma unroll
  for (int u = 0; u < 3; ++u) { const double2 v = *reinterpret_cast<const double2*>(&D[swz(8 * ui[u] + g, 8 * uj[u] + 2 * t)]); c[u][0] = v.x; c[u][1] = v.y; }
  bool bad = false;
#ifdef RCVD_POTRF_PHASES
  long long cl_ = clock64();
#endif
#pragma unroll
  for (int b = 0; b < 4; ++b) {
    const int k0 = 4 * b;
    if (b > 0) {
#pragma unroll
      for (int u = 0; u < 3; ++u) if (8 * uj[u] + 2 * t >= k0) *reinterpret_cast<double2*>(&D[swz(8 * ui[u] + g, 8 * uj[u] + 2 * t)]) = make_double2(c[u][0], c[u][1]);
    }
    __syncwarp();
    double a00 = D[swz(k0, k0)], a10 = D[swz(k0 + 1, k0)], a11 = D[swz(k0 + 1, k0 + 1)], a20 = D[swz(k0 + 2, k0)], a21 = D[swz(k0 + 2, k0 + 1)],
           a22 = D[swz(k0 + 2, k0 + 2)], a30 = D[swz(k0 + 3, k0)], a31 = D[swz(k0 + 3, k0 + 1)], a32 = D[swz(k0 + 3, k0 + 2)], a33 = D[swz(k0 + 3, k0 + 3)];
    CHOL_PHASE(8);
    double t01 = a10 * a10;
    double det01 = fma(a00, a11, -t01);
    if (!(a00 > 0.0) || !isfinite(a00)) { bad = true; a00 = 1.0; det01 = 1.0; }
    if (!(det01 > 0.0) || !isfinite(det01)) { bad = true; det01 = a00; }
    const double p0 = rsqrt(a00), r01 = rsqrt(det01);
    const double sq0 = a00 * p0;
    const double p1 = r01 * sq0;
    const double l11 = det01 * r01 * p0;
    const double l10 = a10 * p0, l20 = a20 * p0, l30 = a30 * p0;
    const double l21 = (a21 - l20 * l10) * p1, l31 = (a31 - l30 * l10) * p1;
    double b22 = fma(-l21, l21, fma(-l20, l20, a22)), b33 = fma(-l31, l31, fma(-l30, l30, a33));
    const double b32 = fma(-l31, l21, fma(-l30, l20, a32));
    double det23 = fma(b22, b33, -(b32 * b32));
    if (!(b22 > 0.0) || !isfinite(b22)) { bad = true; b22 = 1.0; det23 = 1.0; }
    if (!(det23 > 0.0) || !isfinite(det23)) { bad = true; det23 = b22; }
    const double p2 = rsqrt(b22), r23 = rsqrt(det23);
    const double sq2 = b22 * p2;
    const double p3 = r23 * sq2;
    const double l33 = det23 * r23 * p2;
    const double l32 = b32 * p2;
    CHOL_PHASE(9);
    const int r = lane & 15;
    const bool below = lane < 16 && r >= k0 + 4;
    double x0 = D[swz(r, k0)] * p0;
    double x1 = (D[swz(r, k0 + 1)] - x0 * l10) * p1;
    double x2 = (D[swz(r, k0 + 2)] - x0 * l20 - x1 * l21) * p2;
    double x3 = (D[swz(r, k0 + 3)] - x0 * l30 - x1 * l31 - x2 * l32) * p3;
    if (below) { D[swz(r, k0)] = x0; D[swz(r, k0 + 1)] = x1; D[swz(r, k0 + 2)] = x2; D[swz(r, k0 + 3)] = x3; }
    __syncwarp();
    CHOL_PHASE(10);
    if (lane == 0) {
      *reinterpret_cast<double2*>(&D[swz(k0, k0)]) = make_double2(sq0, 0.0);         *reinterpret_cast<double2*>(&D[swz(k0, k0 + 2)]) = make_double2(0.0, 0.0);
      *reinterpret_cast<double2*>(&D[swz(k0 + 1, k0)]) = make_double2(l10, l11);     *reinterpret_cast<double2*>(&D[swz(k0 + 1, k0 + 2)]) = make_double2(0.0, 0.0);
      *reinterpret_cast<double2*>(&D[swz(k0 + 2, k0)]) = make_double2(l20, l21);          *reinterpret_cast<double2*>(&D[swz(k0 + 2, k0 + 2)]) = make_double2(sq2, 0.0);
      *reinterpret_cast<double2*>(&D[swz(k0 + 3, k0)]) = make_double2(l30, l31);          *reinterpret_cast<double2*>(&D[swz(k0 + 3, k0 + 2)]) = make_double2(l32, l33);
      *reinterpret_cast<double2*>(&pinv[k0]) = make_double2(p0, p1);                      *reinterpret_cast<double2*>(&pinv[k0 + 2]) = make_double2(p2, p3);
    }
    if (b < 3) {
      double pa[2];
#pragma unroll
      for (int i = 0; i < 2; ++i) { const int r = 8 * i + g; pa[i] = r >= k0 + 4 ? D[swz(r, k0 + t)] : 0.0; }
#pragma unroll
      for (int u = 0; u < 3; ++u) dmma_8x8x4_fwd(c[u][0], c[u][1], -pa[ui[u]], pa[uj[u]]);
    }
    CHOL_PHASE(11);
  }
  if (bad && lane == 0) *fail = 1;
}


__global__ void __launch_bounds__(kPotrfSmemThreads) k_potrf_smem(double* __restrict__ Lb, double* __restrict__ invT,
                                                                   const int* __restrict__ frames, int npad, int* __restrict__ fail) {
  extern __shared__ __align__(16) double tiles[];
  const int frame = frames[blockIdx.x];
  double* A = Lb + (size_t)frame * npad * npad;
  double* iT = invT + (size_t)frame * npad * 16;
  const int nt = npad / 16, ntl = nt * (nt + 1) / 2;
  double* pinv = tiles + (size_t)ntl * kTileSz;
  const int tid = threadIdx.x, warp = tid >> 5, lane = tid & 31, nw = kPotrfSmemThreads / 32;
  const int g = lane >> 2, t = lane & 3;
#ifdef RCVD_POTRF_PHASES
  long long last_ = clock64();
#endif
  for (int idx = tid; idx < ntl * 128; idx += kPotrfSmemThreads) {
    const int tl = idx >> 7, e = idx & 127, r = e >> 3, c = (e & 7) * 2;
    int ti = (int)((sqrtf(8.f * tl + 1.f) - 1.f) * 0.5f);
    while ((ti + 1) * (ti + 2) / 2 <= tl) ++ti;
    while (ti * (ti + 1) / 2 > tl) --ti;
    const int tj = tl - ti * (ti + 1) / 2;
    cp_async16_fwd(&tiles[(size_t)tl * kTileSz + swz(r, c)], &A[(size_t)(ti * 16 + r) * npad + tj * 16 + c]);
  }
  asm volatile("cp.async.commit_group;" ::: "memory");
  asm volatile("cp.async.wait_group 0;" ::: "memory");
  __syncthreads();
  POTRF_PHASE(0);
  if (warp == 0) warp_chol16_blocked(tiles, pinv, lane, fail);
  __syncthreads();
  POTRF_PHASE(1);
  for (int jb = 0; jb < nt; ++jb) {
    const double* D = tiles + (size_t)(jb * (jb + 1) / 2 + jb) * kTileSz;
    const double* pv = pinv + jb * 16;
    const int rows = (nt - jb - 1) * 16;
    int prow = -1;
    const int nwork = nw - 1, widx = warp - 1;
    if (warp == 0) { if (lane < 16 && rows > 0) prow = lane; } else if (widx * 32 + lane < rows - 16) prow = 16 + widx * 32 + lane;
    if (warp != 0) asm volatile("bar.sync 2, %0;" ::"n"(kPotrfSmemThreads) : "memory");
    if (prow >= 0) {
      const int ti = jb + 1 + (prow >> 4), r = prow & 15;
      double* Tt = tiles + (size_t)(ti * (ti + 1) / 2 + jb) * kTileSz;
      double a[16];
#pragma unroll
      for (int q = 0; q < 16; q += 2) { const double2 v = *reinterpret_cast<const double2*>(&Tt[swz(r, q)]); a[q] = v.x; a[q + 1] = v.y; }
#pragma unroll
      for (int q = 0; q < 16; q += 2) {
        const double2 pq = *reinterpret_cast<const double2*>(&pv[q]);
        const double2 dq = *reinterpret_cast<const double2*>(&D[swz(q + 1, q)]);
        a[q] *= pq.x;
        a[q + 1] = (a[q + 1] - a[q] * dq.x) * pq.y;
#pragma unroll
        for (int c = 0; c < 16; ++c) if (c > q + 1) { const double2 l = *reinterpret_cast<const double2*>(&D[swz(c, q)]); a[c] -= a[q] * l.x; a[c] -= a[q + 1] * l.y; }
      }
#pragma unroll
      for (int q = 0; q < 16; q += 2) *reinterpret_cast<double2*>(&Tt[swz(r, q)]) = make_double2(a[q], a[q + 1]);
    } else if (warp == nw - 1 && lane < 16) {
      const int cidx = lane;
      double xcol[16];
#pragma unroll
      for (int r = 0; r < 16; ++r) xcol[r] = (r == cidx) ? 1.0 : 0.0;
#pragma unroll
      for (int q = 0; q < 16; q += 2) {
        const double2 pq = *reinterpret_cast<const double2*>(&pv[q]);
        const double2 dq = *reinterpret_cast<const double2*>(&D[swz(q + 1, q)]);
        xcol[q] *= pq.x;
        xcol[q + 1] = (xcol[q + 1] - xcol[q] * dq.x) * pq.y;
#pragma unroll
        for (int r = 0; r < 16; ++r) if (r > q + 1) { const double2 l = *reinterpret_cast<const double2*>(&D[swz(r, q)]); xcol[r] -= l.x * xcol[q]; xcol[r] -= l.y * xcol[q + 1]; }
      }
#pragma unroll
      for (int r = 0; r < 16; ++r) iT[(size_t)jb * 256 + r * 16 + cidx] = xcol[r];
    }
    POTRF_PHASE(2);
    if (warp != 0) asm volatile("bar.sync 3, %0;" ::"n"(kPotrfSmemThreads - 32) : "memory");
    POTRF_PHASE(3);
    const int m = nt - jb - 1, ntr = m * (m + 1) / 2;
    auto upd_tile = [&](int gi, int gj) -> double* {
      const double* Xi = tiles + (size_t)(gi * (gi + 1) / 2 + jb) * kTileSz;
      const double* Xj = tiles + (size_t)(gj * (gj + 1) / 2 + jb) * kTileSz;
      double* Ct = tiles + (size_t)(gi * (gi + 1) / 2 + gj) * kTileSz;
      double acc[2][2][2] = {{{0.0, 0.0}, {0.0, 0.0}}, {{0.0, 0.0}, {0.0, 0.0}}};
      tile_mma_nt(Xi, Xj, acc, g, t);
#pragma unroll
      for (int i = 0; i < 2; ++i)
#pragma unroll
        for (int j = 0; j < 2; ++j) {
          double2* ptr = reinterpret_cast<double2*>(&Ct[swz(i * 8 + g, j * 8 + 2 * t)]);
          double2 v = *ptr; v.x -= acc[i][j][0]; v.y -= acc[i][j][1]; *ptr = v;
        }
      return Ct;
    };
    auto tile_of = [&](int tl, int& gi, int& gj) {
      int ti = (int)((sqrtf(8.f * tl + 1.f) - 1.f) * 0.5f);
      while ((ti + 1) * (ti + 2) / 2 <= tl) ++ti;
      while (ti * (ti + 1) / 2 > tl) --ti;
      gi = jb + 1 + ti; gj = jb + 1 + (tl - ti * (ti + 1) / 2);
    };
    if (warp == 0) {
      double* Ct = nullptr;
      if (ntr > 0) { __syncwarp(); Ct = upd_tile(jb + 1, jb + 1); }
      __threadfence_block();
      asm volatile("bar.arrive 2, %0;" ::"n"(kPotrfSmemThreads) : "memory");
      POTRF_PHASE(4);
      if (ntr > 0) { __syncwarp(); warp_chol16_blocked(Ct, pinv + (jb + 1) * 16, lane, fail); }
      POTRF_PHASE(5);
    } else {
      for (int tl = 1 + widx; tl < ntr; tl += nwork) { int gi, gj; tile_of(tl, gi, gj); upd_tile(gi, gj); }
    }
    POTRF_PHASE(6);
    __syncthreads();
    POTRF_PHASE(7);
  }
  for (int idx = tid; idx < ntl * 128; idx += kPotrfSmemThreads) {
    const int tl = idx >> 7, e = idx & 127, r = e >> 3, c = (e & 7) * 2;
    int ti = (int)((sqrtf(8.f * tl + 1.f) - 1.f) * 0.5f);
    while ((ti + 1) * (ti + 2) / 2 <= tl) ++ti;
    while (ti * (ti + 1) / 2 > tl) --ti;
    const int tj = tl - ti * (ti + 1) / 2;
    double2 v = *reinterpret_cast<const double2*>(&tiles[(size_t)tl * kTileSz + swz(r, c)]);
    if (ti == tj) { if (c > r) v.x = 0.0; if (c + 1 > r) v.y = 0.0; }
    *reinterpret_cast<double2*>(&A[(size_t)(ti * 16 + r) * npad + tj * 16 + c]) = v;
  }
}

__global__ void __launch_bounds__(256) k_trinv(const double* __restrict__ Lb, const double* __restrict__ invT, double* __restrict__ invL,
                                                const int* __restrict__ frames, int npad) {
  extern __shared__ double Z[];
  __shared__ double W[16][17];
  const int frame = frames[blockIdx.y];
  const int j = blockIdx.x;
  const int nt = npad / 16;
  double* Lrow_s = Z + (size_t)nt * 256;
  const int ldp = npad + 1;
  const double* A = Lb + (size_t)frame * npad * npad;
  const double* iT = invT + (size_t)frame * npad * 16;
  double* out = invL + (size_t)frame * npad * npad;
  const int tid = threadIdx.x, r = tid >> 4, c = tid & 15;
  for (int i = 0; i < j; ++i) out[(size_t)(i * 16 + r) * npad + j * 16 + c] = 0.0;
  Z[(size_t)j * 256 + tid] = iT[(size_t)j * 256 + tid];
  out[(size_t)(j * 16 + r) * npad + j * 16 + c] = Z[(size_t)j * 256 + tid];
  __syncthreads();
  for (int i = j + 1; i < nt; ++i) {
    const int kw = (i - j) * 16;
    for (int e = tid; e < 16 * kw; e += 256) { const int rr = e / kw, kk = e % kw; Lrow_s[rr * ldp + kk] = A[(size_t)(i * 16 + rr) * npad + j * 16 + kk]; }
    __syncthreads();
    double s0 = 0.0, s1 = 0.0, s2 = 0.0, s3 = 0.0;
    const double* lr = Lrow_s + r * ldp;
    const double* zp = Z + (size_t)j * 256 + c;
    for (int kk = 0; kk < kw; kk += 4) {
      s0 += lr[kk] * zp[(size_t)kk * 16]; s1 += lr[kk + 1] * zp[(size_t)(kk + 1) * 16];
      s2 += lr[kk + 2] * zp[(size_t)(kk + 2) * 16]; s3 += lr[kk + 3] * zp[(size_t)(kk + 3) * 16];
    }
    W[r][c] = (s0 + s1) + (s2 + s3);
    __syncthreads();
    double zv = 0.0;
    const double* ti = iT + (size_t)i * 256;
#pragma unroll
    for (int q = 0; q < 16; ++q) zv -= ti[r * 16 + q] * W[q][c];
    Z[(size_t)i * 256 + tid] = zv;
    out[(size_t)(i * 16 + r) * npad + j * 16 + c] = zv;
    __syncthreads();
  }
}

struct GemmTask { int dst; int first; int count; int lower_only; };

constexpr int kGemmLd = 20;

__device__ __forceinline__ void cp_async16(void* smem, const void* gmem, bool valid) {
  const unsigned s = (unsigned)__cvta_generic_to_shared(smem);
  const int sz = valid ? 16 : 0;
  asm volatile("cp.async.cg.shared.global [%0], [%1], 16, %2;" ::"r"(s), "l"(gmem), "r"(sz) : "memory");
}
__device__ __forceinline__ void cp_async_commit() { asm volatile("cp.async.commit_group;" ::: "memory"); }
template <int N> __device__ __forceinline__ void cp_async_wait() { asm volatile("cp.async.wait_group %0;" ::"n"(N) : "memory"); }

__device__ __forceinline__ void dmma_8x8x4(double& c0, double& c1, double a, double b) {
  asm volatile("mma.sync.aligned.m8n8k4.row.col.f64.f64.f64.f64 {%0,%1}, {%2}, {%3}, {%0,%1};"
               : "+d"(c0), "+d"(c1) : "d"(a), "d"(b));
}
__device__ __forceinline__ void dmma_16x8x4(double& c0, double& c1, double& c2, double& c3, double a0, double a1, double b) {
  asm volatile("mma.sync.aligned.m16n8k4.row.col.f64.f64.f64.f64 {%0,%1,%2,%3}, {%4,%5}, {%6}, {%0,%1,%2,%3};"
               : "+d"(c0), "+d"(c1), "+d"(c2), "+d"(c3) : "d"(a0), "d"(a1), "d"(b));
}

template <int NI, int NJ, int K4 = 4>
__device__ __forceinline__ void gemm_stage(const double* __restrict__ as, const double* __restrict__ bsm, double (&acc)[4][4][2], int wm, int wn, int g, int t) {
#pragma unroll
  for (int k4 = 0; k4 < K4; ++k4) {
    double af[NI > 0 ? NI : 1], bf[NJ > 0 ? NJ : 1];
#pragma unroll
    for (int i = 0; i < NI; ++i) af[i] = as[(wm + i * 8 + g) * kGemmLd + k4 * 4 + t];
#pragma unroll
    for (int j = 0; j < NJ; ++j) bf[j] = bsm[(wn + j * 8 + g) * kGemmLd + k4 * 4 + t];
#pragma unroll
    for (int i = 0; i < NI; ++i)
#pragma unroll
      for (int j = 0; j < NJ; ++j) dmma_8x8x4(acc[i][j][0], acc[i][j][1], af[i], bf[j]);
  }
}

__global__ void __launch_bounds__(128, 4) k_gemm_nt(double* __restrict__ dst, const double* __restrict__ Abase, const double* __restrict__ Bbase,
                                                  const GemmTask* __restrict__ tasks, const int2* __restrict__ pairs,
                                                  int npad, int neff, double alpha, double beta) {
  __shared__ __align__(16) double As[2][64 * kGemmLd];
  __shared__ __align__(16) double Bs[2][64 * kGemmLd];
  const GemmTask task = tasks[blockIdx.z];
  const int m0 = blockIdx.y * 64, n0 = blockIdx.x * 64;
  if ((task.lower_only & 1) && n0 > m0) return;
  const size_t bs = (size_t)npad * npad;
  const int tid = threadIdx.x, warp = tid >> 5, lane = tid & 31;
  const int wm = (warp >> 1) * 32, wn = (warp & 1) * 32;
  const int g = lane >> 2, t = lane & 3;
  const int kchunks = (task.lower_only & 2) ? min(npad, n0 + 64) / 16 : npad / 16;
  const int total = task.count * kchunks;
  const int ni = min(4, max(0, (neff - (m0 + wm)) / 8)), nj = min(4, max(0, (neff - (n0 + wn)) / 8));
  const int lastk = (task.lower_only & 2) ? -1 : kchunks - 1;
  const int tailk4 = (neff - 16 * (npad / 16 - 1) + 3) / 4;
  double acc[4][4][2];
#pragma unroll
  for (int i = 0; i < 4; ++i)
#pragma unroll
    for (int j = 0; j < 4; ++j) { acc[i][j][0] = 0.0; acc[i][j][1] = 0.0; }

  auto load_stage = [&](int st, int kk) {
    const int2 pr = pairs[task.first + kk / kchunks];
    const int k0 = (kk % kchunks) * 16;
    const double* Ag = Abase + (size_t)pr.x * bs + k0;
    const double* Bg = Bbase + (size_t)pr.y * bs + k0;
#pragma unroll
    for (int q = 0; q < 4; ++q) {
      const int cidx = tid + q * 128;
      const int row = cidx >> 3, kc = (cidx & 7) * 2;
      const bool va = (m0 + row) < npad, vb = (n0 + row) < npad;
      cp_async16(&As[st][row * kGemmLd + kc], Ag + (size_t)(va ? m0 + row : 0) * npad + kc, va);
      cp_async16(&Bs[st][row * kGemmLd + kc], Bg + (size_t)(vb ? n0 + row : 0) * npad + kc, vb);
    }
    cp_async_commit();
  };

  if (total > 0) load_stage(0, 0);
  for (int kk = 0; kk < total; ++kk) {
    const int st = kk & 1;
    if (kk + 1 < total) { load_stage(st ^ 1, kk + 1); cp_async_wait<1>(); } else { cp_async_wait<0>(); }
    __syncthreads();
    const double* as = As[st]; const double* bsm = Bs[st];
    const bool tail = (kk % kchunks) == lastk && tailk4 == 2;
#define RCVD_GS(NI_, NJ_) case NI_ * 8 + NJ_: if (tail) gemm_stage<NI_, NJ_, 2>(as, bsm, acc, wm, wn, g, t); else gemm_stage<NI_, NJ_, 4>(as, bsm, acc, wm, wn, g, t); break;
    if (ni == 4 && nj == 4 && !tail) gemm_stage<4, 4, 4>(as, bsm, acc, wm, wn, g, t);
    else switch (ni * 8 + nj) {
      RCVD_GS(4, 4) RCVD_GS(4, 3) RCVD_GS(4, 2) RCVD_GS(4, 1)
      RCVD_GS(3, 4) RCVD_GS(3, 3) RCVD_GS(3, 2) RCVD_GS(3, 1)
      RCVD_GS(2, 4) RCVD_GS(2, 3) RCVD_GS(2, 2) RCVD_GS(2, 1)
      RCVD_GS(1, 4) RCVD_GS(1, 3) RCVD_GS(1, 2) RCVD_GS(1, 1)
      default: break;
    }
#undef RCVD_GS
    __syncthreads();
  }
  double* C = dst + (size_t)task.dst * bs;
#pragma unroll
  for (int i = 0; i < 4; ++i) {
    const int row = m0 + wm + i * 8 + g;
    if (row >= neff) continue;
#pragma unroll
    for (int j = 0; j < 4; ++j) {
      const int col = n0 + wn + j * 8 + 2 * t;
      if (col >= neff) continue;
      double2* ptr = reinterpret_cast<double2*>(C + (size_t)row * npad + col);
      double2 o;
      if (beta != 0.0) { o = *ptr; o.x = beta * o.x + alpha * acc[i][j][0]; o.y = beta * o.y + alpha * acc[i][j][1]; }
      else { o.x = alpha * acc[i][j][0]; o.y = alpha * acc[i][j][1]; }
      *ptr = o;
    }
  }
}

__global__ void __launch_bounds__(128, 4) k_potrf_trail(double* __restrict__ Lb, const int* __restrict__ frames, int npad, int jb) {
  __shared__ __align__(16) double Ps[2][64 * kGemmLd];
  const int frame = frames[blockIdx.y];
  double* A = Lb + (size_t)frame * npad * npad;
  const int j0 = jb * 16, j1 = j0 + 16;
  int ti = (int)((sqrtf(8.f * blockIdx.x + 1.f) - 1.f) * 0.5f);
  while ((ti + 1) * (ti + 2) / 2 <= (int)blockIdx.x) ++ti;
  while (ti * (ti + 1) / 2 > (int)blockIdx.x) --ti;
  const int tj = blockIdx.x - ti * (ti + 1) / 2;
  const int m0 = j1 + ti * 64, n0 = j1 + tj * 64;
  const int tid = threadIdx.x, warp = tid >> 5, lane = tid & 31, g = lane >> 2, t = lane & 3;
  const int wm = (warp >> 1) * 32, wn = (warp & 1) * 32;
  for (int e = tid; e < 64 * 8; e += 128) {
    const int row = e >> 3, kc = (e & 7) * 2;
    const bool va = (m0 + row) < npad, vb = (n0 + row) < npad;
    cp_async16(&Ps[0][row * kGemmLd + kc], A + (size_t)(va ? m0 + row : 0) * npad + j0 + kc, va);
    cp_async16(&Ps[1][row * kGemmLd + kc], A + (size_t)(vb ? n0 + row : 0) * npad + j0 + kc, vb);
  }
  cp_async_commit(); cp_async_wait<0>();
  __syncthreads();
  const int ni = min(4, max(0, (npad - (m0 + wm)) / 8)), nj = min(4, max(0, (npad - (n0 + wn)) / 8));
  double acc[4][4][2];
#pragma unroll
  for (int i = 0; i < 4; ++i)
#pragma unroll
    for (int j = 0; j < 4; ++j) { acc[i][j][0] = 0.0; acc[i][j][1] = 0.0; }
  if (ni == 4 && nj == 4) gemm_stage<4, 4>(Ps[0], Ps[1], acc, wm, wn, g, t);
  else if (ni == 4 && nj == 2) gemm_stage<4, 2>(Ps[0], Ps[1], acc, wm, wn, g, t);
  else if (ni == 2 && nj == 4) gemm_stage<2, 4>(Ps[0], Ps[1], acc, wm, wn, g, t);
  else if (ni == 2 && nj == 2) gemm_stage<2, 2>(Ps[0], Ps[1], acc, wm, wn, g, t);
#pragma unroll
  for (int i = 0; i < 4; ++i) {
    const int row = m0 + wm + i * 8 + g;
    if (i >= ni) continue;
#pragma unroll
    for (int j = 0; j < 4; ++j) {
      const int col = n0 + wn + j * 8 + 2 * t;
      if (j >= nj || col > row) continue;
      double* ptr = A + (size_t)row * npad + col;
      if (col + 1 <= row) { double2 o = *reinterpret_cast<double2*>(ptr); o.x -= acc[i][j][0]; o.y -= acc[i][j][1]; *reinterpret_cast<double2*>(ptr) = o; }
      else ptr[0] -= acc[i][j][0];
    }
  }
}

struct TrsmTask { int dst; int src; int kframe; };
constexpr int kTrsmRW = 8;
constexpr int kTrsmStrip = 4 * kTrsmRW;
__host__ __device__ inline size_t trsm_ll_smem_bytes(int npad, int ahead = 2) { return ((size_t)kTrsmStrip * (npad + 4) + ahead * 16 * (size_t)(npad + 4) + ahead * 16 * 20) * sizeof(double); }

template <int kTrsmAhead>
__global__ void __launch_bounds__(128) k_trsm_ll(double* __restrict__ T, const double* __restrict__ Lb, const double* __restrict__ invT,
                                                  const TrsmTask* __restrict__ tasks, int npad) {
  extern __shared__ __align__(16) double smx[];
  const int ld = npad + 4;
  double* Xs = smx;
  double* Ls = smx + (size_t)kTrsmStrip * ld;
  double* Ds = Ls + (size_t)kTrsmAhead * 16 * ld;
  const TrsmTask task = tasks[blockIdx.y];
  const int m0 = blockIdx.x * kTrsmStrip;
  const size_t bs = (size_t)npad * npad;
  const double* A = Lb + (size_t)task.src * bs;
  const double* Lk = Lb + (size_t)task.kframe * bs;
  const double* iT = invT + (size_t)task.kframe * npad * 16;
  double* X = T + (size_t)task.dst * bs;
  const int tid = threadIdx.x, warp = tid >> 5, lane = tid & 31, g = lane >> 2, t = lane & 3;
  const int nt = npad / 16;
  const int rows = min(kTrsmStrip, npad - m0);
  for (int r = tid >> 3; r < kTrsmStrip; r += 16) {
    const bool v = r < rows;
    const double* src = A + (size_t)(v ? m0 + r : 0) * npad;
    for (int c = (tid & 7) * 2; c < npad; c += 16) cp_async16(&Xs[(size_t)r * ld + c], src + c, v);
  }
  auto stage = [&](int jt) {
    if (jt < nt) {
      double* ls = Ls + (size_t)(jt % kTrsmAhead) * 16 * ld; double* dsm = Ds + (jt % kTrsmAhead) * 320;
      const int kw = jt * 16;
      { const int r = tid >> 3; const double* src = Lk + (size_t)(jt * 16 + r) * npad; for (int c = (tid & 7) * 2; c < kw; c += 16) cp_async16(&ls[(size_t)r * ld + c], src + c, true); }
      { const int r = tid >> 3, c = (tid & 7) * 2; cp_async16(&dsm[r * 20 + c], iT + (size_t)jt * 256 + r * 16 + c, true); }
    }
    cp_async_commit();
  };
#pragma unroll
  for (int q = 0; q < kTrsmAhead; ++q) stage(q);
  constexpr int NI = kTrsmRW / 8;
  const int wr = warp * kTrsmRW;
  for (int jt = 0; jt < nt; ++jt) {
    cp_async_wait<kTrsmAhead - 1>();
    __syncthreads();
    const double* ls = Ls + (size_t)(jt % kTrsmAhead) * 16 * ld; const double* dsm = Ds + (jt % kTrsmAhead) * 320;
    double acc[NI][2][2];
#pragma unroll
    for (int i = 0; i < NI; ++i) { acc[i][0][0] = acc[i][0][1] = acc[i][1][0] = acc[i][1][1] = 0.0; }
    {
      double af[2][4][NI], bf[2][4][2];
      auto frag = [&](int kt, int buf) {
#pragma unroll
        for (int q = 0; q < 4; ++q) {
#pragma unroll
          for (int i = 0; i < NI; ++i) af[buf][q][i] = Xs[(size_t)(wr + i * 8 + g) * ld + kt * 16 + q * 4 + t];
#pragma unroll
          for (int j = 0; j < 2; ++j) bf[buf][q][j] = ls[(size_t)(j * 8 + g) * ld + kt * 16 + q * 4 + t];
        }
      };
      if (jt > 0) frag(0, 0);
      for (int kt = 0; kt < jt; kt += 2) {
        if (kt + 1 < jt) frag(kt + 1, 1);
#pragma unroll
        for (int q = 0; q < 4; ++q)
#pragma unroll
          for (int i = 0; i < NI; ++i)
#pragma unroll
            for (int j = 0; j < 2; ++j) dmma_8x8x4(acc[i][j][0], acc[i][j][1], af[0][q][i], bf[0][q][j]);
        if (kt + 1 < jt) {
          if (kt + 2 < jt) frag(kt + 2, 0);
#pragma unroll
          for (int q = 0; q < 4; ++q)
#pragma unroll
            for (int i = 0; i < NI; ++i)
#pragma unroll
              for (int j = 0; j < 2; ++j) dmma_8x8x4(acc[i][j][0], acc[i][j][1], af[1][q][i], bf[1][q][j]);
        }
      }
    }
#pragma unroll
    for (int i = 0; i < NI; ++i)
#pragma unroll
      for (int j = 0; j < 2; ++j) {
        double2* ptr = reinterpret_cast<double2*>(&Xs[(size_t)(wr + i * 8 + g) * ld + jt * 16 + j * 8 + 2 * t]);
        double2 v = *ptr; v.x -= acc[i][j][0]; v.y -= acc[i][j][1]; *ptr = v;
      }
    __syncwarp();
    double out[NI][2][2];
#pragma unroll
    for (int i = 0; i < NI; ++i) { out[i][0][0] = out[i][0][1] = out[i][1][0] = out[i][1][1] = 0.0; }
#pragma unroll
    for (int k4 = 0; k4 < 4; ++k4) {
      double af[NI], bf[2];
#pragma unroll
      for (int i = 0; i < NI; ++i) af[i] = Xs[(size_t)(wr + i * 8 + g) * ld + jt * 16 + k4 * 4 + t];
#pragma unroll
      for (int j = 0; j < 2; ++j) bf[j] = dsm[(j * 8 + g) * 20 + k4 * 4 + t];
#pragma unroll
      for (int i = 0; i < NI; ++i)
#pragma unroll
        for (int j = 0; j < 2; ++j) dmma_8x8x4(out[i][j][0], out[i][j][1], af[i], bf[j]);
    }
    __syncwarp();
#pragma unroll
    for (int i = 0; i < NI; ++i)
#pragma unroll
      for (int j = 0; j < 2; ++j) {
        const int r = wr + i * 8 + g, cidx = jt * 16 + j * 8 + 2 * t;
        const double2 v = make_double2(out[i][j][0], out[i][j][1]);
        *reinterpret_cast<double2*>(&Xs[(size_t)r * ld + cidx]) = v;
        if (r < rows) *reinterpret_cast<double2*>(&X[(size_t)(m0 + r) * npad + cidx]) = v;
      }
    __syncthreads();
    stage(jt + kTrsmAhead);
  }
}


__global__ void __launch_bounds__(256) k_fwd_diag(const double* __restrict__ invL, const double* __restrict__ rhs, double* __restrict__ y,
                                                   const int* __restrict__ frames, int npad) {
  const int frame = frames[blockIdx.y];
  const int row = blockIdx.x * 8 + (threadIdx.x >> 5);
  const int lane = threadIdx.x & 31;
  if (row >= npad) return;
  const double* M = invL + (size_t)frame * npad * npad + (size_t)row * npad;
  const double* b = rhs + (size_t)frame * npad;
  double s = 0.0;
  for (int q = lane; q <= row; q += 32) s += M[q] * b[q];
  s = warp_sum(s);
  if (lane == 0) y[(size_t)frame * npad + row] = s;
}
struct SolveTask { int blk; int r; int k; };
__global__ void __launch_bounds__(256) k_fwd_update(const double* __restrict__ T, const double* __restrict__ y, double* __restrict__ rhs,
                                                     const SolveTask* __restrict__ tasks, int npad) {
  const SolveTask tk = tasks[blockIdx.y];
  const int row = blockIdx.x * 8 + (threadIdx.x >> 5);
  const int lane = threadIdx.x & 31;
  if (row >= npad) return;
  const double* M = T + (size_t)tk.blk * npad * npad + (size_t)row * npad;
  const double* v = y + (size_t)tk.k * npad;
  double s = 0.0;
  for (int q = lane; q < npad; q += 32) s += M[q] * v[q];
  s = warp_sum(s);
  if (lane == 0) red_add(rhs + (size_t)tk.r * npad + row, -s);
}
__global__ void __launch_bounds__(256) k_bwd_update(const double* __restrict__ T, const double* __restrict__ x, double* __restrict__ y,
                                                     const SolveTask* __restrict__ tasks, int npad) {
  __shared__ double red[8][33];
  const SolveTask tk = tasks[blockIdx.y];
  const int cl = threadIdx.x & 31, rg = threadIdx.x >> 5;
  const int j = blockIdx.x * 32 + cl;
  double acc = 0.0;
  if (j < npad) {
    const double* M = T + (size_t)tk.blk * npad * npad + j;
    const double* xr = x + (size_t)tk.r * npad;
    for (int i = rg; i < npad; i += 8) acc += M[(size_t)i * npad] * xr[i];
  }
  red[rg][cl] = acc;
  __syncthreads();
  if (rg == 0 && j < npad) {
    double s = 0.0;
#pragma unroll
    for (int q = 0; q < 8; ++q) s += red[q][cl];
    if (s != 0.0) red_add(y + (size_t)tk.k * npad + j, -s);
  }
}
__global__ void __launch_bounds__(256) k_bwd_diag(const double* __restrict__ invL, const double* __restrict__ y, double* __restrict__ x,
                                                   const int* __restrict__ frames, int npad) {
  __shared__ double red[8][33];
  const int frame = frames[blockIdx.y];
  const int cl = threadIdx.x & 31, rg = threadIdx.x >> 5;
  const int j = blockIdx.x * 32 + cl;
  double acc = 0.0;
  if (j < npad) {
    const double* M = invL + (size_t)frame * npad * npad + j;
    const double* v = y + (size_t)frame * npad;
    const int i0 = j - (j % 8) + rg;
    for (int i = (i0 < j ? i0 + 8 : i0); i < npad; i += 8) acc += M[(size_t)i * npad] * v[i];
  }
  red[rg][cl] = acc;
  __syncthreads();
  if (rg == 0 && j < npad) {
    double s = 0.0;
#pragma unroll
    for (int q = 0; q < 8; ++q) s += red[q][cl];
    x[(size_t)frame * npad + j] = s;
  }
}

constexpr int kSubChunk = 64;
constexpr int kSubThreads = 256;
struct SubTask { int type; int blk; int r; int k; int chunk; };
struct SubCounters { int* ticket; int* fin; int* fdone; int* bin; int* bdone; const int* fin_need; const int* bin_need; };

__device__ __forceinline__ int ld_acquire_gpu(const int* p) { int v; asm volatile("ld.acquire.gpu.global.s32 %0, [%1];" : "=r"(v) : "l"(p) : "memory"); return v; }
__device__ __forceinline__ void sub_wait(const int* c, int need) { while (ld_acquire_gpu(c) < need) __nanosleep(20); }

__device__ __forceinline__ void red_release_add(int* p, int v) { asm volatile("red.release.gpu.global.add.s32 [%0], %1;" ::"l"(p), "r"(v) : "memory"); }
__device__ __forceinline__ double2 ldcg2(const double* p) { return __ldcg(reinterpret_cast<const double2*>(p)); }

__global__ void __launch_bounds__(kSubThreads) k_substitution(const double* __restrict__ invL, const double* __restrict__ T, double* rhs, double* y, double* x,
                                                              const SubTask* __restrict__ tasks, int ntasks, SubCounters cn, int npad) {
  extern __shared__ __align__(16) double red[];
  __shared__ int s_task;
  const int tid = threadIdx.x, warp = tid >> 5, lane = tid & 31;
  const int nchunks = (npad + kSubChunk - 1) / kSubChunk;
  const size_t bs = (size_t)npad * npad;
  for (;;) {
    if (tid == 0) s_task = atomicAdd(cn.ticket, 1);
    __syncthreads();
    const int ti = s_task;
    if (ti >= ntasks) break;
    const SubTask tk = tasks[ti];
    const int c0 = tk.chunk * kSubChunk, c1 = min(npad, c0 + kSubChunk);
    const double* vin = tk.type == 0 ? rhs + (size_t)tk.k * npad : (tk.type == 2 ? x + (size_t)tk.r * npad : y + (size_t)tk.k * npad);
    const double* M = (tk.type == 0 || tk.type == 3) ? invL + (size_t)tk.k * bs : T + (size_t)tk.blk * bs;
    auto dep_wait = [&]() {
      if (tid == 0) {
        if (tk.type == 0) sub_wait(cn.fin + tk.k, cn.fin_need[tk.k]);
        else if (tk.type == 1) sub_wait(cn.fdone + tk.k, nchunks);
        else if (tk.type == 2) sub_wait(cn.bdone + tk.r, nchunks);
        else { sub_wait(cn.fdone + tk.k, nchunks); sub_wait(cn.bin + tk.k, cn.bin_need[tk.k]); }
      }
      __syncthreads();
    };
    if (tk.type <= 1) {
      constexpr int RW = kSubChunk / (kSubThreads / 32);
      const int r0 = c0 + warp * RW;
      double acc[RW];
#pragma unroll
      for (int i = 0; i < RW; ++i) acc[i] = 0.0;
      for (int qb = 0; qb < npad; qb += 256) {
        double2 m[4][RW];
#pragma unroll
        for (int qi = 0; qi < 4; ++qi) {
          const int q = qb + qi * 64 + 2 * lane;
#pragma unroll
          for (int i = 0; i < RW; ++i) {
            const int row = r0 + i;
            const int len = tk.type == 0 ? row + 1 : npad;
            m[qi][i] = (row < c1 && q < len) ? *reinterpret_cast<const double2*>(M + (size_t)row * npad + q) : make_double2(0.0, 0.0);
            if (q + 1 >= len) m[qi][i].y = 0.0;
          }
        }
        if (qb == 0) dep_wait();
        double2 v[4];
#pragma unroll
        for (int qi = 0; qi < 4; ++qi) { const int q = qb + qi * 64 + 2 * lane; v[qi] = q < npad ? ldcg2(vin + q) : make_double2(0.0, 0.0); }
#pragma unroll
        for (int qi = 0; qi < 4; ++qi)
#pragma unroll
          for (int i = 0; i < RW; ++i) acc[i] += m[qi][i].x * v[qi].x + m[qi][i].y * v[qi].y;
      }
#pragma unroll
      for (int i = 0; i < RW; ++i) {
        const double sum = warp_sum(acc[i]);
        const int row = r0 + i;
        if (lane == 0 && row < c1) { if (tk.type == 0) y[(size_t)tk.k * npad + row] = sum; else red_add(rhs + (size_t)tk.r * npad + row, -sum); }
      }
    } else {
      const int cl = tid & 31, rg = tid >> 5, j = c0 + 2 * cl;
      double ax = 0.0, ay = 0.0;
      const int ifirst = tk.type == 3 ? j + ((rg - j) & 7) : rg;
      for (int ib = ifirst; ib < npad || ib == ifirst; ib += 256) {
        double2 m[32];
#pragma unroll
        for (int u = 0; u < 32; ++u) { const int i = ib + 8 * u; m[u] = (i < npad && j < c1) ? *reinterpret_cast<const double2*>(M + (size_t)i * npad + j) : make_double2(0.0, 0.0); }
        if (ib == ifirst) dep_wait();
        double vi[32];
#pragma unroll
        for (int u = 0; u < 32; ++u) { const int i = ib + 8 * u; vi[u] = i < npad ? __ldcg(vin + i) : 0.0; }
#pragma unroll
        for (int u = 0; u < 32; ++u) { const int i = ib + 8 * u; ax += m[u].x * vi[u]; if (tk.type != 3 || i > j) ay += m[u].y * vi[u]; }
      }
      red[rg * (kSubChunk + 2) + 2 * cl] = ax; red[rg * (kSubChunk + 2) + 2 * cl + 1] = ay;
      __syncthreads();
      if (tid < kSubChunk && c0 + tid < c1) {
        double sum = 0.0;
#pragma unroll
        for (int q = 0; q < 8; ++q) sum += red[q * (kSubChunk + 2) + tid];
        if (tk.type == 3) x[(size_t)tk.k * npad + c0 + tid] = sum; else red_add(y + (size_t)tk.k * npad + c0 + tid, -sum);
      }
    }
    __syncthreads();
    if (tid == 0) red_release_add(tk.type == 0 ? cn.fdone + tk.k : (tk.type == 1 ? cn.fin + tk.r : (tk.type == 2 ? cn.bin + tk.k : cn.bdone + tk.k)), 1);
  }
}
__host__ __device__ inline size_t substitution_smem_bytes(int) { return (size_t)8 * (kSubChunk + 2) * sizeof(double); }

struct HBlock { int lblk; int r; int c; };
__global__ void __launch_bounds__(256) k_load_factor(const double* __restrict__ H, double* __restrict__ Lb, const HBlock* __restrict__ lb,
                                                      const double* __restrict__ S, const double* __restrict__ D2, int npad, int nf, const int* __restrict__ blist) {
  const int bid = blist ? blist[blockIdx.y] : blockIdx.y;
  const HBlock b = lb[bid];
  const int e = blockIdx.x * 256 + threadIdx.x;
  if (e >= npad * npad) return;
  const int i = e / npad, j = e % npad;
  const size_t bs = (size_t)npad * npad;
  double v = 0.0;
  if (b.r == b.c) {
    if (j > i) v = 0.0;
    else if (i >= nf) v = (i == j) ? 1.0 : 0.0;
    else {
      v = H[(size_t)b.lblk * bs + e] * S[(size_t)b.r * npad + i] * S[(size_t)b.c * npad + j];
      if (i == j) v += D2[(size_t)b.r * npad + i];
    }
  } else if (b.lblk >= 0 && i < nf && j < nf) {
    v = H[(size_t)b.lblk * bs + e] * S[(size_t)b.r * npad + i] * S[(size_t)b.c * npad + j];
  }
  Lb[(size_t)bid * bs + e] = v;
}

__global__ void __launch_bounds__(256) k_spmv_sym(const double* __restrict__ H, const HBlock* __restrict__ hb, const double* __restrict__ v,
                                                   double* __restrict__ out, int npad, const int* __restrict__ blist) {
  const int bid = blist ? blist[blockIdx.y] : blockIdx.y;
  const HBlock b = hb[bid];
  const int row = blockIdx.x * 8 + (threadIdx.x >> 5);
  const int lane = threadIdx.x & 31;
  if (row >= npad) return;
  const double* M = H + (size_t)bid * npad * npad + (size_t)row * npad;
  const double* vc = v + (size_t)b.c * npad;
  const double vr = v[(size_t)b.r * npad + row];
  double s = 0.0;
  if (b.r == b.c) {
    for (int q = lane; q <= row; q += 32) {
      const double m = M[q];
      s += m * vc[q];
      if (q < row && m != 0.0) red_add(out + (size_t)b.c * npad + q, m * vr);
    }
  } else {
    for (int q = lane; q < npad; q += 32) {
      const double m = M[q];
      s += m * vc[q];
      if (m != 0.0 && vr != 0.0) red_add(out + (size_t)b.c * npad + q, m * vr);
    }
  }
  s = warp_sum(s);
  if (lane == 0 && s != 0.0) red_add(out + (size_t)b.r * npad + row, s);
}

}
```

robust_cvd_b200/csrc/rcvd_update.cuh:

```cuda
#pragma once
#include <cuda.h>
#include <stdint.h>
#include "rcvd_linalg.cuh"

namespace rcvd {

struct UpdItem {
  int dst;
  int first, count;
  short m0, n0;
  short mrows, ncols;
  int flags;
};

constexpr int kUpdMaxTile = 80;
constexpr int kUpdPartial = 4 * 25 * 32 * 2;
template <int TEAMS> struct UpdShape { static constexpr int stages = TEAMS == 2 ? 8 : 5, threads = TEAMS * 128 + 32, ctas = TEAMS == 2 ? 1 : 2; };
__host__ __device__ inline size_t upd_smem_bytes(int rb, int teams) {
  const int stages = teams == 2 ? 8 : 5;
  return (size_t)stages * 2 * rb * 16 * sizeof(double) + (teams == 2 ? (size_t)kUpdPartial * sizeof(double) : 0) + 2 * stages * sizeof(uint64_t) + 1024;
}

__device__ __forceinline__ uint32_t smem_u32(const void* p) { return (uint32_t)__cvta_generic_to_shared(p); }
__device__ __forceinline__ void mbar_init(uint64_t* bar, int count) { asm volatile("mbarrier.init.shared::cta.b64 [%0], %1;" ::"r"(smem_u32(bar)), "r"(count) : "memory"); }
__device__ __forceinline__ void mbar_expect_tx(uint64_t* bar, uint32_t bytes) {
  asm volatile("mbarrier.arrive.expect_tx.shared::cta.b64 _, [%0], %1;" ::"r"(smem_u32(bar)), "r"(bytes) : "memory");
}
__device__ __forceinline__ void mbar_arrive(uint64_t* bar) { asm volatile("mbarrier.arrive.shared::cta.b64 _, [%0];" ::"r"(smem_u32(bar)) : "memory"); }
__device__ __forceinline__ void mbar_wait(uint64_t* bar, uint32_t parity) {
  asm volatile(
      "{\n"
      ".reg .pred P1;\n"
      "LAB_WAIT:\n"
      "mbarrier.try_wait.parity.shared::cta.b64 P1, [%0], %1;\n"
      "@P1 bra DONE;\n"
      "bra LAB_WAIT;\n"
      "DONE:\n"
      "}" ::"r"(smem_u32(bar)), "r"(parity) : "memory");
}
__device__ __forceinline__ void tma_load_2d(void* dst, const CUtensorMap* map, uint64_t* bar, int c0, int c1) {
  asm volatile("cp.async.bulk.tensor.2d.shared::cluster.global.mbarrier::complete_tx::bytes [%0], [%1, {%3, %4}], [%2];"
               ::"r"(smem_u32(dst)), "l"(reinterpret_cast<uint64_t>(map)), "r"(smem_u32(bar)), "r"(c0), "r"(c1) : "memory");
}

template <int NI, int NJ>
__device__ __forceinline__ void upd_mma(const double (&af)[NI], const double (&bf)[NJ], double (&acc)[5][5][2]) {
#pragma unroll
  for (int i = 0; i + 1 < NI; i += 2)
#pragma unroll
    for (int j = 0; j < NJ; ++j) dmma_16x8x4(acc[i][j][0], acc[i][j][1], acc[i + 1][j][0], acc[i + 1][j][1], af[i], af[i + 1], bf[j]);
  if (NI & 1) {
#pragma unroll
    for (int j = 0; j < NJ; ++j) dmma_8x8x4(acc[NI - 1][j][0], acc[NI - 1][j][1], af[NI - 1], bf[j]);
  }
}

template <int NI, int NJ>
__device__ __forceinline__ void upd_stage(const unsigned char* __restrict__ As, const unsigned char* __restrict__ Bs, const int (&kc)[4], int k4n, double (&acc)[5][5][2]) {
  if (k4n == 4) {
#pragma unroll
    for (int k4 = 0; k4 < 4; ++k4) {
      double af[NI], bf[NJ];
#pragma unroll
      for (int i = 0; i < NI; ++i) af[i] = *reinterpret_cast<const double*>(As + kc[k4] + i * 1024);
#pragma unroll
      for (int j = 0; j < NJ; ++j) bf[j] = *reinterpret_cast<const double*>(Bs + kc[k4] + j * 1024);
      upd_mma<NI, NJ>(af, bf, acc);
    }
  } else {
#pragma unroll
    for (int k4 = 0; k4 < 4; ++k4) {
      if (k4 < k4n) {
        double af[NI], bf[NJ];
#pragma unroll
        for (int i = 0; i < NI; ++i) af[i] = *reinterpret_cast<const double*>(As + kc[k4] + i * 1024);
#pragma unroll
        for (int j = 0; j < NJ; ++j) bf[j] = *reinterpret_cast<const double*>(Bs + kc[k4] + j * 1024);
        upd_mma<NI, NJ>(af, bf, acc);
      }
    }
  }
}

template <int NI, int NJ>
__device__ __forceinline__ void upd_epilogue(double* __restrict__ C, int npad, const double (&acc)[5][5][2], int t, const double* __restrict__ part) {
  const bool hi = (t & 2) != 0;
#pragma unroll
  for (int i = 0; i < NI; ++i) {
    double2 v[NJ];
#pragma unroll
    for (int j = 0; j < NJ; ++j) v[j] = *reinterpret_cast<const double2*>(C + (size_t)i * 8 * npad + j * 8);
#pragma unroll
    for (int j = 0; j < NJ; ++j) {
      double a0 = acc[i][j][0], a1 = acc[i][j][1];
      if (part) { const double2 q = *reinterpret_cast<const double2*>(part + (size_t)(i * 5 + j) * 64); a0 += q.x; a1 += q.y; }
      const double give = hi ? a0 : a1;
      const double got = __shfl_xor_sync(0xffffffffu, give, 2);
      const double lo = hi ? got : a0, up = hi ? a1 : got;
      v[j].x -= lo; v[j].y -= up;
      *reinterpret_cast<double2*>(C + (size_t)i * 8 * npad + j * 8) = v[j];
    }
  }
}
template <int NI, int NJ>
__device__ __forceinline__ void upd_store_partial(double* __restrict__ part, const double (&acc)[5][5][2]) {
#pragma unroll
  for (int i = 0; i < NI; ++i)
#pragma unroll
    for (int j = 0; j < NJ; ++j) *reinterpret_cast<double2*>(part + (size_t)(i * 5 + j) * 64) = make_double2(acc[i][j][0], acc[i][j][1]);
}
__device__ __forceinline__ void named_bar_sync(int id, int n) { asm volatile("bar.sync %0, %1;" ::"r"(id), "r"(n) : "memory"); }
__device__ __forceinline__ void named_bar_arrive(int id, int n) { asm volatile("bar.arrive %0, %1;" ::"r"(id), "r"(n) : "memory"); }

#define RCVD_UPD_CASES(M) \
  M(1, 1) M(1, 2) M(1, 3) M(1, 4) M(1, 5) M(2, 1) M(2, 2) M(2, 3) M(2, 4) M(2, 5) M(3, 1) M(3, 2) M(3, 3) M(3, 4) M(3, 5) \
  M(4, 1) M(4, 2) M(4, 3) M(4, 4) M(4, 5) M(5, 1) M(5, 2) M(5, 3) M(5, 4) M(5, 5)

template <int TEAMS>
__global__ void __launch_bounds__(UpdShape<TEAMS>::threads, UpdShape<TEAMS>::ctas) k_update_tma(const __grid_constant__ CUtensorMap tmap, double* __restrict__ dst,
                                                               const UpdItem* __restrict__ items, int nitems, const int2* __restrict__ pairs,
                                                               int npad, int neff, int rb, int dbg) {
  extern __shared__ __align__(1024) unsigned char ring[];
  if (smem_u32(ring) & 1023u) __trap();
  constexpr int kUpdStages = UpdShape<TEAMS>::stages;
  const int tile_bytes = rb * 128, stage_bytes = 2 * tile_bytes;
  double* partial = reinterpret_cast<double*>(ring + (size_t)kUpdStages * stage_bytes);
  uint64_t* full = reinterpret_cast<uint64_t*>(partial + (TEAMS == 2 ? kUpdPartial : 0));
  uint64_t* empty = full + kUpdStages;
  const int tid = threadIdx.x, warp = tid >> 5, lane = tid & 31;
  if (tid == 0) {
    for (int s = 0; s < kUpdStages; ++s) { mbar_init(&full[s], 1); mbar_init(&empty[s], 4); }
    asm volatile("fence.mbarrier_init.release.cluster;" ::: "memory");
    asm volatile("fence.proxy.async.shared::cta;" ::: "memory");
  }
  __syncthreads();
  const int nk = (neff + 15) >> 4;
  const size_t bs = (size_t)npad * npad;
  if (warp == 4 * TEAMS) {
    if (lane != 0 || (dbg & 1)) return;
    int stage = 0; uint32_t phase = 0;
    for (int w = blockIdx.x; w < nitems; w += gridDim.x) {
      const UpdItem it = items[w];
      for (int p = 0; p < it.count; ++p) {
        const int2 pr = pairs[it.first + p];
        const int rowA = pr.x * npad + it.m0, rowB = pr.y * npad + it.n0;
        for (int kk = 0; kk < nk; ++kk) {
          mbar_wait(&empty[stage], phase ^ 1);
          unsigned char* sa = ring + (size_t)stage * stage_bytes;
          mbar_expect_tx(&full[stage], (uint32_t)stage_bytes);
          tma_load_2d(sa, &tmap, &full[stage], kk * 16, rowA);
          tma_load_2d(sa + tile_bytes, &tmap, &full[stage], kk * 16, rowB);
          if (++stage == kUpdStages) { stage = 0; phase ^= 1; }
        }
      }
    }
    return;
  }
  const int team = warp >> 2, tw = warp & 3;
  const int g = lane >> 2, t = lane & 3;
  const int pg = ((g & 3) << 1) | (g >> 2);
  int kc[4];
#pragma unroll
  for (int k4 = 0; k4 < 4; ++k4) kc[k4] = (((2 * k4 + (t >> 1)) ^ pg) << 4) + ((t & 1) << 3);
  const int wr = tw >> 1, wc = tw & 1;
  double* mypart = partial + (size_t)tw * (25 * 64) + lane * 2;
  if (TEAMS == 2 && team == 0) named_bar_arrive(2, 256);
  int stage = 0; uint32_t phase = 0; unsigned sidx = 0;
  for (int w = blockIdx.x; w < nitems; w += gridDim.x) {
    const UpdItem it = items[w];
    const int hm = ((it.mrows >> 3) + 1) >> 1 << 3, hn = ((it.ncols >> 3) + 1) >> 1 << 3;
    const int wm = wr * hm, wn = wc * hn;
    int ni = wr ? (it.mrows - hm) >> 3 : hm >> 3, nj = wc ? (it.ncols - hn) >> 3 : hn >> 3;
    if ((it.flags & 1) && wr == 0 && wc == 1) ni = 0;
    if (ni == 0 || nj == 0) { ni = 0; nj = 0; }
    double acc[5][5][2];
#pragma unroll
    for (int i = 0; i < 5; ++i)
#pragma unroll
      for (int j = 0; j < 5; ++j) { acc[i][j][0] = 0.0; acc[i][j][1] = 0.0; }
    const int code = ni * 8 + nj;
    const int steps = it.count * nk;
    int kk = 0;
    for (int s = 0; s < steps; ++s, ++sidx) {
      if (TEAMS == 1 || (int)(sidx & 1u) == team) {
        if (!(dbg & 1)) mbar_wait(&full[stage], phase);
        const int k4n = min(4, (neff - kk * 16 + 3) >> 2);
        const unsigned char* sa = ring + (size_t)stage * stage_bytes + (size_t)(wm + pg) * 128;
        const unsigned char* sb = ring + (size_t)stage * stage_bytes + tile_bytes + (size_t)(wn + pg) * 128;
        switch (code) {
#define RCVD_UPD_STAGE(NI_, NJ_) case NI_ * 8 + NJ_: upd_stage<NI_, NJ_>(sa, sb, kc, k4n, acc); break;
          RCVD_UPD_CASES(RCVD_UPD_STAGE)
#undef RCVD_UPD_STAGE
          default: break;
        }
        __syncwarp();
        if (lane == 0 && !(dbg & 1)) mbar_arrive(&empty[stage]);
      }
      if (++stage == kUpdStages) { stage = 0; phase ^= 1; }
      if (++kk == nk) kk = 0;
    }
    if (TEAMS == 2 && team == 1) {
      named_bar_sync(2, 256);
      switch (code) {
#define RCVD_UPD_PART(NI_, NJ_) case NI_ * 8 + NJ_: upd_store_partial<NI_, NJ_>(mypart, acc); break;
        RCVD_UPD_CASES(RCVD_UPD_PART)
#undef RCVD_UPD_PART
        default: break;
      }
      named_bar_arrive(1, 256);
      continue;
    }
    if (TEAMS == 2) named_bar_sync(1, 256);
    if (dbg & 2) { if (acc[0][0][0] == 1.2345e300) dst[0] = acc[4][4][1] + acc[2][3][0]; if (TEAMS == 2) named_bar_arrive(2, 256); continue; }
    double* C = dst + (size_t)it.dst * bs + (size_t)(it.m0 + wm + pg) * npad + it.n0 + wn + ((t & 1) << 2) + (t & 2);
    switch (code) {
#define RCVD_UPD_EPI(NI_, NJ_) case NI_ * 8 + NJ_: upd_epilogue<NI_, NJ_>(C, npad, acc, t, TEAMS == 2 ? mypart : nullptr); break;
      RCVD_UPD_CASES(RCVD_UPD_EPI)
#undef RCVD_UPD_EPI
      default: break;
    }
    if (TEAMS == 2) named_bar_arrive(2, 256);
  }
}

}
```

robust_cvd_b200/solver.py:

```python
import ctypes as C
import os
import numpy as np

from . import abi

_HERE = os.path.dirname(os.path.abspath(__file__))
_LIB = None


def lib():
    global _LIB
    if _LIB is None:
        path = os.path.join(_HERE, "librcvd_b200.so")
        if not os.path.exists(path):
            raise RuntimeError(f"{path} is missing: run `python -c 'import __graft_entry__ as g; g.build()'` "
                               "(the CUDA extension is mandatory, there is no CPU fallback)")
        L = C.CDLL(path)
        L.rcvd_last_error.restype = C.c_char_p
        L.rcvd_launch_count.restype = C.c_int64
        L.rcvd_problem_create.argtypes = [C.POINTER(abi.Config), C.c_int32, C.POINTER(C.c_void_p)]
        L.rcvd_problem_destroy.argtypes = [C.c_void_p]
        for name in ("rcvd_frame_stride", "rcvd_depth_param_offset", "rcvd_spatial_param_offset"):
            getattr(L, name).argtypes = [C.POINTER(abi.Config)]
        _LIB = L
    return _LIB


def _p(a, t):
    return a.ctypes.data_as(C.POINTER(t)) if a is not None else None


def _check(rc):
    if rc != 0:
        raise RuntimeError(f"rcvd error {rc}: {lib().rcvd_last_error().decode()}")


def frame_stride(cfg):
    return lib().rcvd_frame_stride(C.byref(cfg))


def depth_param_offset(cfg):
    return lib().rcvd_depth_param_offset(C.byref(cfg))


def spatial_param_offset(cfg):
    return lib().rcvd_spatial_param_offset(C.byref(cfg))


FACTOR_PLAN_COUNTS = ("levels", "offdiag_factor_blocks", "h_blocks", "update_targets", "update_items", "substitution_tasks",
                      "distributed", "first_replicated_level", "first_substitution_level", "rank_l_blocks", "rank_h_blocks", "rank_frames")


def factor_plan(cfg, pairs, trip_centers=(), order_slack=4, nranks=1, rank=0, num_sms=132):
    n = cfg.num_frames
    pf = np.ascontiguousarray(np.asarray(pairs, np.int32).reshape(-1, 2))
    tc = np.ascontiguousarray(np.asarray(trip_centers, np.int32).reshape(-1))
    arrays = {k: np.zeros(n, np.int32) for k in ("order", "level", "owner", "perm")}
    out = (C.c_int32 * len(FACTOR_PLAN_COUNTS))()
    _check(lib().rcvd_debug_factor_plan(C.byref(cfg), C.c_int32(pf.shape[0]), _p(pf, C.c_int32), C.c_int32(tc.size), _p(tc, C.c_int32),
                                        C.c_int32(order_slack), C.c_int32(nranks), C.c_int32(rank), C.c_int32(num_sms),
                                        *(_p(a, C.c_int32) for a in arrays.values()), out))
    return {**arrays, **dict(zip(FACTOR_PLAN_COUNTS, list(out)))}


class Problem:
    def __init__(self, cfg, device=0):
        self.cfg = cfg
        self.L = lib()
        self.h = C.c_void_p()
        _check(self.L.rcvd_problem_create(C.byref(cfg), C.c_int32(device), C.byref(self.h)))
        self.N = cfg.num_frames
        self.stride = frame_stride(cfg)
        self.U = self.N * self.stride
        self.num_constraints = 0

    def close(self):
        if getattr(self, "h", None):
            self.L.rcvd_problem_destroy(self.h)
            self.h = None

    def __del__(self):
        try:
            self.close()
        except Exception:
            pass

    def set_frames(self, in_range=None, median_depth=None, adaptive_weights=None):
        ir = None if in_range is None else np.ascontiguousarray(in_range, np.uint8)
        md = None if median_depth is None else np.ascontiguousarray(median_depth, np.float64)
        aw = None if adaptive_weights is None else np.ascontiguousarray(adaptive_weights, np.float64)
        _check(self.L.rcvd_problem_set_frames(self.h, _p(ir, C.c_uint8), _p(md, C.c_double), _p(aw, C.c_double)))

    def set_constraints(self, pair_frames, offsets, records):
        pf = np.ascontiguousarray(pair_frames, np.int32).reshape(-1, 2)
        off = np.ascontiguousarray(offsets, np.int64)
        rec = np.ascontiguousarray(records, np.float32).reshape(-1, 6)
        assert off.shape[0] == pf.shape[0] + 1 and off[-1] == rec.shape[0]
        self.num_constraints = int(rec.shape[0])
        _check(self.L.rcvd_problem_set_constraints(self.h, C.c_int32(pf.shape[0]), _p(pf, C.c_int32), _p(off, C.c_int64), _p(rec, C.c_float)))

    def set_triplets(self, centers, offsets, records):
        ce = np.ascontiguousarray(centers, np.int32); off = np.ascontiguousarray(offsets, np.int64)
        rec = np.ascontiguousarray(records, np.float32).reshape(-1, 10)
        assert off.shape[0] == ce.shape[0] + 1 and off[-1] == rec.shape[0]
        _check(self.L.rcvd_problem_set_triplets(self.h, C.c_int32(ce.shape[0]), _p(ce, C.c_int32), _p(off, C.c_int64), _p(rec, C.c_float)))

    def set_structure(self, pair_frames):
        pf = np.ascontiguousarray(pair_frames, np.int32).reshape(-1, 2)
        _check(self.L.rcvd_problem_set_structure(self.h, C.c_int32(pf.shape[0]), _p(pf, C.c_int32)))

    def init_comm(self, nranks, rank, unique_id):
        uid = np.ascontiguousarray(unique_id, np.uint8)
        assert uid.size == 128
        _check(self.L.rcvd_problem_init_comm(self.h, C.c_int32(nranks), C.c_int32(rank), _p(uid, C.c_uint8)))

    def set_state(self, x):
        x = np.ascontiguousarray(x, np.float64).reshape(-1)
        assert x.size == self.U
        _check(self.L.rcvd_problem_set_state(self.h, _p(x, C.c_double)))

    def get_state(self):
        x = np.empty(self.U, np.float64)
        _check(self.L.rcvd_problem_get_state(self.h, _p(x, C.c_double)))
        return x.reshape(self.N, self.stride)

    def evaluate(self, gradient=False):
        cost = C.c_double()
        g = np.zeros(self.U, np.float64) if gradient else None
        _check(self.L.rcvd_evaluate(self.h, C.byref(cost), _p(g, C.c_double)))
        return (cost.value, g) if gradient else cost.value

    def normal_matrix_dense(self):
        H = np.zeros((self.U, self.U), np.float64)
        _check(self.L.rcvd_normal_matrix_dense(self.h, _p(H, C.c_double)))
        return H

    def debug_linear_solve(self, S, D2, b):
        S = np.ascontiguousarray(S, np.float64); D2 = np.ascontiguousarray(D2, np.float64)
        b = np.ascontiguousarray(b, np.float64); y = np.zeros_like(b)
        _check(self.L.rcvd_debug_linear_solve(self.h, _p(S, C.c_double), _p(D2, C.c_double), _p(b, C.c_double), _p(y, C.c_double)))
        return y

    def solve_matrix(self, H, D2, b):
        H = np.ascontiguousarray(H, np.float64); D2 = np.ascontiguousarray(D2, np.float64); b = np.ascontiguousarray(b, np.float64)
        assert H.shape == (self.U, self.U) and D2.size == self.U and b.size == self.U
        y = np.zeros(self.U, np.float64)
        _check(self.L.rcvd_debug_solve_matrix(self.h, _p(H, C.c_double), _p(D2, C.c_double), _p(b, C.c_double), _p(y, C.c_double)))
        return y

    def factor_dense(self, inverses=False):
        order = np.zeros(self.N, np.int32); Lf = np.zeros((self.U, self.U), np.float64)
        Li = np.zeros((self.N, self.stride, self.stride), np.float64) if inverses else None
        _check(self.L.rcvd_debug_factor_dense(self.h, _p(order, C.c_int32), _p(Lf, C.c_double), _p(Li, C.c_double)))
        return order, Lf, Li

    LINEAR_PATHS = ("potrf_smem", "potrf_panel", "trsm_ll4", "trsm_ll2", "trsm_gemm", "update_tma1", "update_tma2", "update_gemm",
                    "substitution_levels", "substitution_fused", "trinv", "other", "update_tma1_multi_item")

    def linear_paths(self):
        out = (C.c_int64 * len(self.LINEAR_PATHS))()
        _check(self.L.rcvd_debug_linear_paths(self.h, out))
        return dict(zip(self.LINEAR_PATHS, list(out)))

    def solve(self, options=None):
        opt = options or abi.default_solve_options()
        s = abi.SolveSummary()
        _check(self.L.rcvd_solve(self.h, C.byref(opt), C.byref(s)))
        return s

    def time_accumulate(self, iters=10):
        ms = C.c_double()
        _check(self.L.rcvd_time_accumulate(self.h, C.c_int32(iters), C.byref(ms)))
        return ms.value

    def time_iteration(self, iters=5, radius=1e4):
        a, b, c, d = C.c_double(), C.c_double(), C.c_double(), C.c_double()
        _check(self.L.rcvd_time_iteration(self.h, C.c_int32(iters), C.c_double(radius), C.byref(a), C.byref(b), C.byref(c), C.byref(d)))
        return {"iter_ms": a.value, "accumulate_ms": b.value, "linear_ms": c.value, "cost_ms": d.value}

    def last_iteration(self):
        g, xc, out = np.empty(self.U, np.float64), np.empty(self.U, np.float64), (C.c_double * 2)()
        _check(self.L.rcvd_debug_last_iteration(self.h, _p(g, C.c_double), _p(xc, C.c_double), out))
        return {"gradient": g.reshape(self.N, self.stride), "candidate_state": xc.reshape(self.N, self.stride), "cost": out[0], "candidate_cost": out[1]}

    def structure_info(self):
        out = (C.c_int32 * 8)()
        _check(self.L.rcvd_structure_info(self.h, out))
        keys = ["frames", "offdiag_factor_blocks", "levels", "h_blocks", "npad", "stride", "tiles", "update_tasks"]
        return dict(zip(keys, list(out)))

    def linear_residual(self, radius=1e4):
        out = (C.c_double * 6)()
        _check(self.L.rcvd_debug_linear_residual(self.h, C.c_double(radius), out))
        keys = ["rel_residual", "rhs_norm", "cost", "grad_norm", "step_norm", "pivot_fail"]
        return dict(zip(keys, list(out)))

    def profile_linear(self, reps=3):
        out = (C.c_double * 8)()
        _check(self.L.rcvd_debug_profile_linear(self.h, C.c_int32(reps), out))
        keys = ["load_ms", "potrf_ms", "trinv_ms", "trsm_ms", "gemm_ms", "solve_ms", "gemm_launches", "gemm_flops"]
        return dict(zip(keys, list(out)))

    def set_fast_path(self, on=True):
        _check(self.L.rcvd_debug_set_fast_path(self.h, C.c_int32(int(on))))

    def set_update_kernel(self, tma=True, side_items_per_cta=0):
        _check(self.L.rcvd_debug_set_update_kernel(self.h, C.c_int32(1 if tma else 0), C.c_int32(side_items_per_cta)))

    def set_eval_only(self, on=True):
        _check(self.L.rcvd_debug_set_eval_only(self.h, C.c_int32(1 if on else 0)))

    def set_distributed(self, on=True):
        _check(self.L.rcvd_debug_set_distributed(self.h, C.c_int32(1 if on else 0)))

    def distribution_info(self):
        out = (C.c_int32 * 4)()
        _check(self.L.rcvd_distribution_info(self.h, out))
        return dict(zip(["distributed", "first_replicated_level", "levels", "frames_owned"], list(out)))

    def set_order_slack(self, slack):
        _check(self.L.rcvd_debug_set_order_slack(self.h, C.c_int32(slack)))

    def set_overlap(self, on=True):
        _check(self.L.rcvd_debug_set_overlap(self.h, C.c_int32(1 if on else 0)))

    def launch_count(self):
        return int(self.L.rcvd_launch_count(self.h))


def nccl_unique_id():
    out = np.zeros(128, np.uint8)
    _check(lib().rcvd_nccl_unique_id(_p(out, C.c_uint8)))
    return out


def depth_apply(cfg, depth_params, src, device=0):
    src = np.ascontiguousarray(src, np.float32); h, w = src.shape
    dp = np.ascontiguousarray(depth_params, np.float64); dst = np.empty_like(src)
    _check(lib().rcvd_depth_apply(C.byref(cfg), C.c_int32(device), _p(dp, C.c_double), _p(src, C.c_float), _p(dst, C.c_float), C.c_int32(h), C.c_int32(w)))
    return dst


def depth_param_map(cfg, depth_params, h, w, device=0):
    k = 2 if cfg.value_xform == abi.VALUE_SCALESHIFT else 1
    dp = np.ascontiguousarray(depth_params, np.float64); out = np.empty((h, w, k), np.float64)
    _check(lib().rcvd_depth_param_map(C.byref(cfg), C.c_int32(device), _p(dp, C.c_double), _p(out, C.c_double), C.c_int32(h), C.c_int32(w)))
    return out[:, :, 0] if k == 1 else out


def spatial_warp(cfg, spatial_params, h, w, device=0):
    sp = np.ascontiguousarray(spatial_params, np.float64); out = np.empty((h, w, 2), np.float32)
    _check(lib().rcvd_spatial_warp(C.byref(cfg), C.c_int32(device), _p(sp, C.c_double), _p(out, C.c_float), C.c_int32(h), C.c_int32(w)))
    return out


def flow_guided_filter(depth, cams, fwd_flow, fwd_mask, bwd_flow, bwd_mask, first_out, num_out, frame_radius, spatial_radius=0, median=False,
                       inv_aspect=1.0, far_pairs=None, far_flow=None, far_mask=None, device=0):
    depth = np.ascontiguousarray(depth, np.float32); cams = np.ascontiguousarray(cams, np.float32)
    F, hd, wd = depth.shape
    arrs = []
    for a, dt in ((fwd_flow, np.float32), (fwd_mask, np.uint8), (bwd_flow, np.float32), (bwd_mask, np.uint8), (far_flow, np.float32), (far_mask, np.uint8)):
        arrs.append(None if a is None else np.ascontiguousarray(a, dt))
    ff, fm, bf, bm, rf, rm = arrs
    ref_mask = fm if fm is not None else rm
    if ref_mask is None:
        raise ValueError("flow masks are needed to define the output resolution")
    h, w = ref_mask.shape[1:3]
    nfar = 0 if far_pairs is None else len(far_pairs)
    fp = None if nfar == 0 else np.ascontiguousarray(far_pairs, np.int32).reshape(-1, 2)
    prm = abi.FilterParams(num_frames=F, first_out=first_out, num_out=num_out, width=w, height=h, depth_width=wd, depth_height=hd,
                           frame_radius=frame_radius, spatial_radius=spatial_radius, median=1 if median else 0, num_far=nfar, inv_aspect=inv_aspect)
    out = np.zeros((num_out, h, w), np.float32)
    _check(lib().rcvd_flow_guided_filter(C.byref(prm), C.c_int32(device), _p(depth, C.c_float), _p(cams, C.c_float),
                                         _p(ff, C.c_float), _p(fm, C.c_uint8), _p(bf, C.c_float), _p(bm, C.c_uint8),
                                         _p(fp, C.c_int32), _p(rf, C.c_float), _p(rm, C.c_uint8), _p(out, C.c_float)))
    return out


def bilateral_filter(depth, out_frames, color_bgr=None, frame_radius=2, spatial_radius=0, depth_sigma=0.3, color_sigma=0.0, median=False,
                     in_place=False, xform_cfg=None, xform_params=None, device=0):
    depth = np.ascontiguousarray(depth, np.float32)
    F, h, w = depth.shape
    of = np.ascontiguousarray(out_frames, np.int32).reshape(-1)
    col = None if color_bgr is None else np.ascontiguousarray(color_bgr, np.float32)
    if col is not None and col.shape != (F, h, w, 3):
        raise ValueError(f"colour stack has shape {col.shape}, expected {(F, h, w, 3)}")
    xp = None if xform_params is None else np.ascontiguousarray(xform_params, np.float64)
    prm = abi.BilateralParams(num_frames=F, width=w, height=h, num_out=len(of), frame_radius=frame_radius, spatial_radius=spatial_radius,
                              median=1 if median else 0, depth_sigma=depth_sigma, color_sigma=color_sigma, in_place=1 if in_place else 0)
    out = np.zeros((len(of), h, w), np.float32)
    _check(lib().rcvd_bilateral_filter(C.byref(prm), C.c_int32(device), _p(depth, C.c_float), _p(col, C.c_float), _p(of, C.c_int32),
                                       None if xform_cfg is None else C.byref(xform_cfg), _p(xp, C.c_double), _p(out, C.c_float)))
    return out


def build_constraints(color_bgr, pair_frames,pair_flow, pair_mask, match_separation, inv_aspect, dyn_dist=None, min_dynamic_distance=-1.0,
                      trip_frames=None, trip_flow=None, trip_mask=None, device=0):
    color = np.ascontiguousarray(color_bgr, np.float32)
    F, h, w = color.shape[:3]
    pf = np.ascontiguousarray(pair_frames, np.int32).reshape(-1, 2); P = len(pf)
    pfl = np.ascontiguousarray(pair_flow, np.float32) if P else None; pm = np.ascontiguousarray(pair_mask, np.uint8) if P else None
    T = 0 if trip_frames is None else len(trip_frames)
    tf = np.ascontiguousarray(trip_frames, np.int32) if T else None
    tfl = np.ascontiguousarray(trip_flow, np.float32) if T else None; tm = np.ascontiguousarray(trip_mask, np.uint8) if T else None
    dd = None if dyn_dist is None else np.ascontiguousarray(dyn_dist, np.float32)
    prm = abi.BuilderParams(num_frames=F, width=w, height=h, dyn_width=0 if dd is None else dd.shape[2], dyn_height=0 if dd is None else dd.shape[1],
                            match_separation=match_separation, num_pairs=P, num_triplets=T, min_dynamic_distance=min_dynamic_distance, inv_aspect=inv_aspect)
    poff = np.zeros(P + 1, np.int64); toff = np.zeros(T + 1, np.int64)
    pcap, tcap = 0, 0
    for attempt in range(2):
# ... 41 lines not shown
```

Before: 73.78 million.

## Stream Cholesky panels into TRSM via progress flags and programmatic dependent launch

The shared-memory Cholesky kernel now writes each finished column panel to global memory and publishes a per-frame progress counter with release semantics. A streamed TRSM variant launched with programmatic dependent launch polls that counter and stages panels as they become ready, so it overlaps with the factorisation instead of waiting for it to finish. The triangular-inverse kernel moves to its own low-priority stream so it no longer shares a stream with the second update batch, and that batch's fork is delayed when the next level is streamed. The risks are spin-waiting, which can deadlock if the TRSM grid does not fit co-resident with the Cholesky blocks, and the extra synchronisation and publish traffic inside the Cholesky kernel.

```diff
diff --git a/include/rcvd_hooks.h b/include/rcvd_hooks.h
--- a/include/rcvd_hooks.h
+++ b/include/rcvd_hooks.h
@@ -21,7 +21,7 @@
 
 int32_t rcvd_debug_solve_matrix(rcvd_problem* p, const double* H, const double* D2, const double* b, double* y);
 int32_t rcvd_debug_factor_dense(rcvd_problem* p, int32_t* order, double* L, double* Linv);
-int32_t rcvd_debug_linear_paths(rcvd_problem* p, int64_t out[13]);
+int32_t rcvd_debug_linear_paths(rcvd_problem* p, int64_t out[14]);
 
 int32_t rcvd_debug_linear_residual(rcvd_problem* p, double radius, double out[6]);
 
diff --git a/robust_cvd_b200/csrc/rcvd_api.cu b/robust_cvd_b200/csrc/rcvd_api.cu
--- a/robust_cvd_b200/csrc/rcvd_api.cu
+++ b/robust_cvd_b200/csrc/rcvd_api.cu
@@ -161,7 +161,7 @@
 }
 
 enum { LP_POTRF_SMEM = 0, LP_POTRF_PANEL, LP_TRSM_LL4, LP_TRSM_LL2, LP_TRSM_GEMM, LP_UPD_TMA1, LP_UPD_TMA2, LP_UPD_GEMM, LP_SUB_LEVEL, LP_SUB_FUSED,
-       LP_TRINV, LP_OTHER, LP_UPD_TMA1_MULTI, LP_N };
+       LP_TRINV, LP_OTHER, LP_UPD_TMA1_MULTI, LP_TRSM_STREAMED, LP_N };
 
 struct rcvd_problem {
   rcvd_config cfg; Layout L; int N = 0; int device = 0;
@@ -183,6 +183,8 @@
   int npartial = 0;
   double *d_H = nullptr, *d_Lb = nullptr, *d_T = nullptr, *d_invL = nullptr, *d_invT = nullptr;
   HBlock *d_hblocks = nullptr, *d_lblocks = nullptr; int* d_fail = nullptr;
+  int* d_potrf_progress = nullptr;
+  int trsm2_ctas_per_sm = 0;
   FactorPlan plan;
   int *d_lvl_frames = nullptr; GemmTask *d_trsm_tasks = nullptr, *d_upd_tasks = nullptr; int2 *d_trsm_pairs = nullptr, *d_upd_pairs = nullptr;
   SubTask* d_sub_tasks = nullptr; int* d_sub_counters = nullptr; int* d_sub_need = nullptr;
@@ -193,6 +195,7 @@
   int64_t launches = 0, graph_launches = 0;
   std::vector<double> h_state; bool state_dirty = false; bool use_fast = true; bool overlap = true; int order_slack = 4;
   cudaStream_t side_stream = nullptr; cudaEvent_t ev_fork = nullptr, ev_join = nullptr;
+  cudaStream_t inv_stream = nullptr; cudaEvent_t ev_inv_join = nullptr;
   double *d_g2 = nullptr, *d_delta = nullptr; int* h_fail = nullptr;
   cudaEvent_t ev[8] = {nullptr};
   std::vector<void*> allocs;
@@ -224,6 +227,7 @@
 static void free_all(rcvd_problem* p) {
   if (p->solve_graph) { cudaGraphExecDestroy(p->solve_graph); p->solve_graph = nullptr; }
   if (p->side_stream) cudaStreamSynchronize(p->side_stream);
+  if (p->inv_stream) cudaStreamSynchronize(p->inv_stream);
   for (void* q : p->allocs) cudaFreeAsync(q, p->stream);
   p->allocs.clear();
   if (p->stream) cudaStreamSynchronize(p->stream);
@@ -324,6 +328,7 @@
   DA(p->d_S, Upad); DA(p->d_lmdiag, Upad); DA(p->d_D2, Upad); DA(p->d_gs, Upad); DA(p->d_rhs, Upad);
   DA(p->d_g2, Upad + 8); DA(p->d_delta, Upad);
   DA(p->d_ytmp, Upad); DA(p->d_y, Upad); DA(p->d_Sy, Upad); DA(p->d_Hy, Upad); DA(p->d_scal, SC_N); DA(p->d_active, Upad); DA(p->d_fail, 1);
+  DA(p->d_potrf_progress, (size_t)N);
   const RegCounts rcn = reg_counts(p->cfg, L, N, p->nscale);
   p->npartial = p->num_tiles + (rcn.total + 127) / 128 + p->num_trip_tiles + 1;
   DA(p->d_partial, (size_t)p->npartial);
@@ -375,7 +380,15 @@
   CK(cudaFuncSetAttribute(k_accumulate_fast, cudaFuncAttributeMaxDynamicSharedMemorySize, kFastSmem));
   CK(cudaFuncSetAttribute(k_accumulate_runs, cudaFuncAttributeMaxDynamicSharedMemorySize, kRunSmem));
   p->use_trsm_ll = trsm_ll_smem_bytes(npad) <= 220 * 1024;
-  if (p->use_trsm_ll) { CK(cudaFuncSetAttribute(k_trsm_ll<2>, cudaFuncAttributeMaxDynamicSharedMemorySize, (int)trsm_ll_smem_bytes(npad, 2))); if (trsm_ll_smem_bytes(npad, 4) <= 220 * 1024) CK(cudaFuncSetAttribute(k_trsm_ll<4>, cudaFuncAttributeMaxDynamicSharedMemorySize, (int)trsm_ll_smem_bytes(npad, 4))); }
+  if (p->use_trsm_ll) {
+    CK(cudaFuncSetAttribute(k_trsm_ll<2>, cudaFuncAttributeMaxDynamicSharedMemorySize, (int)trsm_ll_smem_bytes(npad, 2)));
+    CK(cudaFuncSetAttribute(k_trsm_ll<2, true>, cudaFuncAttributeMaxDynamicSharedMemorySize, (int)trsm_ll_smem_bytes(npad, 2)));
+    CK(cudaOccupancyMaxActiveBlocksPerMultiprocessor(&p->trsm2_ctas_per_sm, k_trsm_ll<2, true>, 128, trsm_ll_smem_bytes(npad, 2)));
+    if (trsm_ll_smem_bytes(npad, 4) <= 220 * 1024) {
+      CK(cudaFuncSetAttribute(k_trsm_ll<4>, cudaFuncAttributeMaxDynamicSharedMemorySize, (int)trsm_ll_smem_bytes(npad, 4)));
+      CK(cudaFuncSetAttribute(k_trsm_ll<4, true>, cudaFuncAttributeMaxDynamicSharedMemorySize, (int)trsm_ll_smem_bytes(npad, 4)));
+    }
+  }
   if (potrf_smem_bytes(npad) <= 220 * 1024) CK(cudaFuncSetAttribute(k_potrf_smem, cudaFuncAttributeMaxDynamicSharedMemorySize, (int)potrf_smem_bytes(npad)));
   return RCVD_OK;
 }
@@ -430,27 +443,50 @@
     k_gemm_nt<<<dim3(tiles, tiles, ntasks), 128, 0, cs>>>(dstp, A, B, tasks, prs, npad, beta != 0.0 ? neff : npad, alpha, beta);
   };
   mark(-1);
+  CK(cudaMemsetAsync(p->d_potrf_progress, 0, (size_t)N * sizeof(int), st));
   k_load_factor<<<dim3((npad * npad + 255) / 256, p->plan.dist ? (int)p->plan.own_lblocks.size() : nL), 256, 0, st>>>(p->d_H, p->d_Lb, p->d_lblocks, p->d_S, p->d_D2, npad, L.nf, p->plan.dist ? p->d_own_lblocks : nullptr);
   p->launches += 1; p->paths[LP_OTHER]++; mark(P_LOAD);
-  cudaStream_t side = p->side_stream;
-  bool side_pending = false, side_used = false;
+  cudaStream_t side = p->side_stream, inv = p->inv_stream;
+  bool side_pending = false, side_used = false, inv_used = false;
+  auto join_inv = [&]() -> int {
+    if (inv_used) { CK(cudaEventRecord(p->ev_inv_join, inv)); CK(cudaStreamWaitEvent(st, p->ev_inv_join, 0)); inv_used = false; }
+    return RCVD_OK;
+  };
   const size_t bsz = (size_t)npad * npad;
   auto phase_boundary = [&]() -> int {
     if (side_pending || side_used) { CK(cudaEventRecord(p->ev_join, side)); CK(cudaStreamWaitEvent(st, p->ev_join, 0)); side_pending = false; }
-    std::vector<Seg> inv, tr;
-    for (int q = 0; q < p->nranks; ++q) inv.push_back({(size_t)p->plan.fa_off[q], (size_t)p->plan.fa_cnt[q]});
+    if (int rc = join_inv()) return rc;
+    std::vector<Seg> invs, tr;
+    for (int q = 0; q < p->nranks; ++q) invs.push_back({(size_t)p->plan.fa_off[q], (size_t)p->plan.fa_cnt[q]});
     for (int q = 0; q < p->nranks; ++q) tr.push_back({(size_t)p->plan.fb_off[q], (size_t)p->plan.fb_cnt[q]});
     for (int q = 0; q < p->nranks; ++q) tr.push_back({(size_t)N + (size_t)p->plan.bseg[2 * q], (size_t)p->plan.bseg[2 * q + 1]});
-    int rc = grouped(p, p->d_invL, bsz, inv, true); if (rc) return rc;
+    int rc = grouped(p, p->d_invL, bsz, invs, true); if (rc) return rc;
     return grouped(p, p->d_Lb, bsz, tr, true);
   };
+  const int strips = (npad + kTrsmStrip - 1) / kTrsmStrip;
+  auto trsm_deep = [&](const Level& v) { return strips * v.ntrsm <= p->num_sms && trsm_ll_smem_bytes(npad, 4) <= 220 * 1024; };
+  auto streamed = [&](const Level& v) {
+    return p->use_trsm_ll && v.nown > 0 && v.ntrsm > 0 && potrf_smem_bytes(npad) <= 220 * 1024 &&
+           strips * v.ntrsm <= (trsm_deep(v) ? 1 : p->trsm2_ctas_per_sm) * p->num_sms;
+  };
+  auto pdl_attr = [](cudaLaunchAttribute& a) { a.id = cudaLaunchAttributeProgrammaticStreamSerialization; a.val.programmaticStreamSerializationAllowed = 1; };
   for (size_t li = 0; li < p->plan.levels.size(); ++li) {
     const Level& lv = p->plan.levels[li]; prof_level = (int)li;
+    const bool chain = streamed(lv);
+    const bool fork_u2_late = p->overlap && p->gemm_tma && li + 1 < p->plan.levels.size() && streamed(p->plan.levels[li + 1]);
     if (p->plan.dist && (int)li == p->plan.LB) { int rc = phase_boundary(); if (rc) return rc; }
     const int* lframes = p->d_lvl_own + lv.own_off; const int nfr = lv.nown;
     if (nfr > 0) {
     if (potrf_smem_bytes(npad) <= 220 * 1024) {
-      k_potrf_smem<<<nfr, kPotrfSmemThreads, potrf_smem_bytes(npad), st>>>(p->d_Lb, p->d_invT, lframes, npad, p->d_fail);
+      if (chain && li > 0) {
+        cudaLaunchAttribute attr[1]; pdl_attr(attr[0]);
+        cudaLaunchConfig_t lc = {};
+        lc.gridDim = dim3(nfr); lc.blockDim = dim3(kPotrfSmemThreads); lc.dynamicSmemBytes = potrf_smem_bytes(npad); lc.stream = st;
+        lc.attrs = attr; lc.numAttrs = 1;
+        CK(cudaLaunchKernelEx(&lc, k_potrf_smem, p->d_Lb, p->d_invT, lframes, npad, p->d_fail, p->d_potrf_progress));
+      } else {
+        k_potrf_smem<<<nfr, kPotrfSmemThreads, potrf_smem_bytes(npad), st>>>(p->d_Lb, p->d_invT, lframes, npad, p->d_fail, p->d_potrf_progress);
+      }
       p->paths[LP_POTRF_SMEM]++;
     } else {
       const int nt16 = npad / 16;
@@ -465,18 +501,27 @@
     p->launches += 1; mark(P_POTRF);
     if (p->use_trsm_ll) {
       cudaStream_t is = st;
-      if (p->overlap) { CK(cudaEventRecord(p->ev_fork, st)); CK(cudaStreamWaitEvent(side, p->ev_fork, 0)); is = side; side_used = true; }
+      if (p->overlap) { CK(cudaEventRecord(p->ev_fork, st)); CK(cudaStreamWaitEvent(inv, p->ev_fork, 0)); is = inv; inv_used = true; }
       k_trinv<<<dim3(npad / 16, nfr), 256, (npad * 16 + 16 * (npad + 1)) * sizeof(double), is>>>(p->d_Lb, p->d_invT, p->d_invL, lframes, npad);
       p->launches += 1; p->paths[LP_TRINV]++; mark(P_TRINV);
       if (lv.ntrsm > 0) {
-        const int strips = (npad + kTrsmStrip - 1) / kTrsmStrip;
-        if (strips * lv.ntrsm <= p->num_sms && trsm_ll_smem_bytes(npad, 4) <= 220 * 1024) {
-          k_trsm_ll<4><<<dim3(strips, lv.ntrsm), 128, trsm_ll_smem_bytes(npad, 4), st>>>(p->d_T, p->d_Lb, p->d_invT, p->d_trsm_ll + lv.trsm_off, npad);
-          p->paths[LP_TRSM_LL4]++;
+        const bool deep = trsm_deep(lv);
+        const TrsmTask* tasks = p->d_trsm_ll + lv.trsm_off;
+        if (chain) {
+          cudaLaunchAttribute attr[1]; pdl_attr(attr[0]);
+          cudaLaunchConfig_t lc = {};
+          lc.gridDim = dim3(strips, lv.ntrsm); lc.blockDim = dim3(128); lc.dynamicSmemBytes = trsm_ll_smem_bytes(npad, deep ? 4 : 2); lc.stream = st;
+          lc.attrs = attr; lc.numAttrs = 1;
+          const double *Lb = p->d_Lb, *invT = p->d_invT; const int* progress = p->d_potrf_progress;
+          CK(deep ? cudaLaunchKernelEx(&lc, k_trsm_ll<4, true>, p->d_T, Lb, invT, tasks, npad, progress)
+                  : cudaLaunchKernelEx(&lc, k_trsm_ll<2, true>, p->d_T, Lb, invT, tasks, npad, progress));
+          p->paths[LP_TRSM_STREAMED]++;
+        } else if (deep) {
+          k_trsm_ll<4><<<dim3(strips, lv.ntrsm), 128, trsm_ll_smem_bytes(npad, 4), st>>>(p->d_T, p->d_Lb, p->d_invT, tasks, npad, nullptr);
         } else {
-          k_trsm_ll<2><<<dim3(strips, lv.ntrsm), 128, trsm_ll_smem_bytes(npad, 2), st>>>(p->d_T, p->d_Lb, p->d_invT, p->d_trsm_ll + lv.trsm_off, npad);
-          p->paths[LP_TRSM_LL2]++;
+          k_trsm_ll<2><<<dim3(strips, lv.ntrsm), 128, trsm_ll_smem_bytes(npad, 2), st>>>(p->d_T, p->d_Lb, p->d_invT, tasks, npad, nullptr);
         }
+        p->paths[deep ? LP_TRSM_LL4 : LP_TRSM_LL2]++;
         p->launches++; mark(P_TRSM);
       }
     } else {
@@ -490,9 +535,8 @@
       for (int q = 0; q < p->nranks; ++q) segs.push_back({(size_t)p->plan.tseg[(li * p->nranks + q) * 2], (size_t)p->plan.tseg[(li * p->nranks + q) * 2 + 1]});
       int rc = grouped(p, p->d_T, bsz, segs, true); if (rc) return rc;
     }
-    if (lv.nupd2 > 0 && p->overlap) {
-      CK(cudaEventRecord(p->ev_fork, st)); CK(cudaStreamWaitEvent(side, p->ev_fork, 0));
-    }
+    auto fork_u2 = [&]() -> int { CK(cudaEventRecord(p->ev_fork, st)); CK(cudaStreamWaitEvent(side, p->ev_fork, 0)); return RCVD_OK; };
+    if (lv.nupd2 > 0 && p->overlap && !fork_u2_late) { if (int rc = fork_u2()) return rc; }
     if (side_pending) { CK(cudaStreamWaitEvent(st, p->ev_join, 0)); side_pending = false; }
     auto update = [&](cudaStream_t cs, int off, int n) {
       if (n <= p->num_sms) {
@@ -508,6 +552,7 @@
     if (p->gemm_tma) {
       if (lv.nit > 0) { update(st, lv.it_off, lv.nit); p->launches++; mark(P_GEMM); }
       if (lv.nit2 > 0) {
+        if (fork_u2_late) { if (int rc = fork_u2()) return rc; }
         update(p->overlap ? side : st, lv.it2_off, lv.nit2); p->launches++; mark(P_GEMM);
         if (p->overlap) { CK(cudaEventRecord(p->ev_join, side)); side_pending = true; side_used = true; }
       }
@@ -521,6 +566,7 @@
   }
   if (p->plan.dist && p->plan.LB >= (int)p->plan.levels.size()) { int rc = phase_boundary(); if (rc) return rc; }
   if (side_pending || side_used) { CK(cudaEventRecord(p->ev_join, side)); CK(cudaStreamWaitEvent(st, p->ev_join, 0)); }
+  if (int rc = join_inv()) return rc;
   CK(cudaMemcpyAsync(p->d_rhs, p->d_gs, (size_t)N * npad * sizeof(double), cudaMemcpyDeviceToDevice, st));
   const int nlv = (int)p->plan.levels.size();
   const int LS = p->plan.sub_first_level;
@@ -952,8 +998,10 @@
   int prio_lo = 0, prio_hi = 0; cudaDeviceGetStreamPriorityRange(&prio_lo, &prio_hi);
   e = cudaStreamCreateWithPriority(&p->stream, cudaStreamNonBlocking, prio_hi);
   if (e == cudaSuccess) e = cudaStreamCreateWithPriority(&p->side_stream, cudaStreamNonBlocking, prio_lo);
+  if (e == cudaSuccess) e = cudaStreamCreateWithPriority(&p->inv_stream, cudaStreamNonBlocking, prio_lo);
   if (e == cudaSuccess) e = cudaEventCreateWithFlags(&p->ev_fork, cudaEventDisableTiming);
   if (e == cudaSuccess) e = cudaEventCreateWithFlags(&p->ev_join, cudaEventDisableTiming);
+  if (e == cudaSuccess) e = cudaEventCreateWithFlags(&p->ev_inv_join, cudaEventDisableTiming);
   if (e != cudaSuccess) { delete p; return set_err(RCVD_ERR_CUDA, "cudaStreamCreate: %s", cudaGetErrorString(e)); }
   *out = p; return RCVD_OK;
 }
@@ -965,7 +1013,9 @@
   if (p->comm && nccl::CommDestroy) nccl::CommDestroy(p->comm);
   if (p->ev_fork) cudaEventDestroy(p->ev_fork);
   if (p->ev_join) cudaEventDestroy(p->ev_join);
+  if (p->ev_inv_join) cudaEventDestroy(p->ev_inv_join);
   if (p->side_stream) cudaStreamDestroy(p->side_stream);
+  if (p->inv_stream) cudaStreamDestroy(p->inv_stream);
   if (p->stream) cudaStreamDestroy(p->stream);
   delete p;
 }
@@ -1123,7 +1173,7 @@
   if (!p->structure_ready || !p->factored) return set_err(RCVD_ERR_INVALID, "no factorisation has run on this handle");
   if (p->plan.dist) return set_err(RCVD_ERR_INVALID, "the distributed factorisation keeps its blocks on their owners");
   SET_DEVICE(p->device);
-  CK(cudaStreamSynchronize(p->side_stream)); CK(cudaStreamSynchronize(p->stream));
+  CK(cudaStreamSynchronize(p->side_stream)); CK(cudaStreamSynchronize(p->inv_stream)); CK(cudaStreamSynchronize(p->stream));
   const int N = p->N, nf = p->L.nf, npad = p->L.npad, nT = p->plan.nLoff; const size_t U = (size_t)N * nf, bs = (size_t)npad * npad;
   std::vector<double> hL((size_t)N * bs), hT((size_t)nT * bs);
   CK(cudaMemcpy(hL.data(), p->d_Lb, hL.size() * sizeof(double), cudaMemcpyDeviceToHost));
@@ -1146,9 +1196,9 @@
   }
   return RCVD_OK;
 }
-RCVD_API int32_t rcvd_debug_linear_paths(rcvd_problem* p, int64_t out[13]) {
+RCVD_API int32_t rcvd_debug_linear_paths(rcvd_problem* p, int64_t out[14]) {
   if (!p || !out) return set_err(RCVD_ERR_INVALID, "null argument");
-  static_assert(LP_N == 13, "include/rcvd_hooks.h documents thirteen counters");
+  static_assert(LP_N == 14, "include/rcvd_hooks.h documents fourteen counters");
   std::copy(p->paths, p->paths + LP_N, out);
   return RCVD_OK;
 }
@@ -1216,7 +1266,7 @@
     evs.clear(); p->prof = &evs;
     rc = enqueue_factor_solve(p);
     p->prof = nullptr; p->factored = true;
-    cudaStreamSynchronize(p->stream); cudaStreamSynchronize(p->side_stream);
+    cudaStreamSynchronize(p->stream); cudaStreamSynchronize(p->side_stream); cudaStreamSynchronize(p->inv_stream);
     double ngemm = 0;
     for (size_t i = 1; i < evs.size(); ++i) {
       float ms = 0; cudaEventElapsedTime(&ms, evs[i - 1].second, evs[i].second);
diff --git a/robust_cvd_b200/csrc/rcvd_linalg.cuh b/robust_cvd_b200/csrc/rcvd_linalg.cuh
--- a/robust_cvd_b200/csrc/rcvd_linalg.cuh
+++ b/robust_cvd_b200/csrc/rcvd_linalg.cuh
@@ -86,6 +86,9 @@
   asm volatile("mma.sync.aligned.m8n8k4.row.col.f64.f64.f64.f64 {%0,%1}, {%2}, {%3}, {%0,%1};"
                : "+d"(c0), "+d"(c1) : "d"(a), "d"(b));
 }
+__device__ __forceinline__ int ld_acquire_gpu(const int* p) { int v; asm volatile("ld.acquire.gpu.global.s32 %0, [%1];" : "=r"(v) : "l"(p) : "memory"); return v; }
+__device__ __forceinline__ void st_release_gpu(int* p, int v) { asm volatile("st.release.gpu.global.s32 [%0], %1;" ::"l"(p), "r"(v) : "memory"); }
+__device__ __forceinline__ void red_release_add(int* p, int v) { asm volatile("red.release.gpu.global.add.s32 [%0], %1;" ::"l"(p), "r"(v) : "memory"); }
 
 __device__ __forceinline__ void tile_mma_nt(const double* __restrict__ At, const double* __restrict__ Bt, double acc[2][2][2], int g, int t) {
 #pragma unroll
@@ -181,7 +184,10 @@
 
 
 __global__ void __launch_bounds__(kPotrfSmemThreads) k_potrf_smem(double* __restrict__ Lb, double* __restrict__ invT,
-                                                                   const int* __restrict__ frames, int npad, int* __restrict__ fail) {
+                                                                   const int* __restrict__ frames, int npad, int* __restrict__ fail,
+                                                                   int* __restrict__ progress) {
+  asm volatile("griddepcontrol.wait;" ::: "memory");
+  asm volatile("griddepcontrol.launch_dependents;" ::: "memory");
   extern __shared__ __align__(16) double tiles[];
   const int frame = frames[blockIdx.x];
   double* A = Lb + (size_t)frame * npad * npad;
@@ -190,6 +196,16 @@
   double* pinv = tiles + (size_t)ntl * kTileSz;
   const int tid = threadIdx.x, warp = tid >> 5, lane = tid & 31, nw = kPotrfSmemThreads / 32;
   const int g = lane >> 2, t = lane & 3;
+  auto publish = [&](int jc) {
+    for (int idx = tid - 32; idx < (nt - jc) * 128; idx += kPotrfSmemThreads - 32) {
+      const int ti = jc + (idx >> 7), e = idx & 127, r = e >> 3, c = (e & 7) * 2;
+      double2 v = *reinterpret_cast<const double2*>(&tiles[(size_t)(ti * (ti + 1) / 2 + jc) * kTileSz + swz(r, c)]);
+      if (ti == jc) { if (c > r) v.x = 0.0; if (c + 1 > r) v.y = 0.0; }
+      *reinterpret_cast<double2*>(&A[(size_t)(ti * 16 + r) * npad + jc * 16 + c]) = v;
+    }
+    asm volatile("bar.sync 3, %0;" ::"n"(kPotrfSmemThreads - 32) : "memory");
+    if (tid == 32) st_release_gpu(progress + frame, jc + 1);
+  };
 #ifdef RCVD_POTRF_PHASES
   long long last_ = clock64();
 #endif
@@ -215,7 +231,10 @@
     int prow = -1;
     const int nwork = nw - 1, widx = warp - 1;
     if (warp == 0) { if (lane < 16 && rows > 0) prow = lane; } else if (widx * 32 + lane < rows - 16) prow = 16 + widx * 32 + lane;
-    if (warp != 0) asm volatile("bar.sync 2, %0;" ::"n"(kPotrfSmemThreads) : "memory");
+    if (warp != 0) {
+      if (jb > 0) publish(jb - 1);
+      asm volatile("bar.sync 2, %0;" ::"n"(kPotrfSmemThreads) : "memory");
+    }
     if (prow >= 0) {
       const int ti = jb + 1 + (prow >> 4), r = prow & 15;
       double* Tt = tiles + (size_t)(ti * (ti + 1) / 2 + jb) * kTileSz;
@@ -290,16 +309,7 @@
     __syncthreads();
     POTRF_PHASE(7);
   }
-  for (int idx = tid; idx < ntl * 128; idx += kPotrfSmemThreads) {
-    const int tl = idx >> 7, e = idx & 127, r = e >> 3, c = (e & 7) * 2;
-    int ti = (int)((sqrtf(8.f * tl + 1.f) - 1.f) * 0.5f);
-    while ((ti + 1) * (ti + 2) / 2 <= tl) ++ti;
-    while (ti * (ti + 1) / 2 > tl) --ti;
-    const int tj = tl - ti * (ti + 1) / 2;
-    double2 v = *reinterpret_cast<const double2*>(&tiles[(size_t)tl * kTileSz + swz(r, c)]);
-    if (ti == tj) { if (c > r) v.x = 0.0; if (c + 1 > r) v.y = 0.0; }
-    *reinterpret_cast<double2*>(&A[(size_t)(ti * 16 + r) * npad + tj * 16 + c]) = v;
-  }
+  if (warp != 0) publish(nt - 1);
 }
 
 __global__ void __launch_bounds__(256) k_trinv(const double* __restrict__ Lb, const double* __restrict__ invT, double* __restrict__ invL,
@@ -505,10 +515,16 @@
 constexpr int kTrsmStrip = 4 * kTrsmRW;
 __host__ __device__ inline size_t trsm_ll_smem_bytes(int npad, int ahead = 2) { return ((size_t)kTrsmStrip * (npad + 4) + ahead * 16 * (size_t)(npad + 4) + ahead * 16 * 20) * sizeof(double); }
 
-template <int kTrsmAhead>
+__device__ __forceinline__ void cp_async_wait_upto3(int n) {
+  if (n >= 3) cp_async_wait<3>(); else if (n == 2) cp_async_wait<2>(); else if (n == 1) cp_async_wait<1>(); else cp_async_wait<0>();
+}
+
+template <int kTrsmAhead, bool kStreamed = false>
 __global__ void __launch_bounds__(128) k_trsm_ll(double* __restrict__ T, const double* __restrict__ Lb, const double* __restrict__ invT,
-                                                  const TrsmTask* __restrict__ tasks, int npad) {
+                                                  const TrsmTask* __restrict__ tasks, int npad, const int* progress) {
+  static_assert(!kStreamed || kTrsmAhead <= 4, "cp_async_wait_upto3 leaves at most three groups in flight");
   extern __shared__ __align__(16) double smx[];
+  __shared__ int s_ready;
   const int ld = npad + 4;
   double* Xs = smx;
   double* Ls = smx + (size_t)kTrsmStrip * ld;
@@ -537,12 +553,31 @@
     }
     cp_async_commit();
   };
-#pragma unroll
-  for (int q = 0; q < kTrsmAhead; ++q) stage(q);
+  if constexpr (kStreamed) {
+    cp_async_commit();
+  } else {
+#pragma unroll
+    for (int q = 0; q < kTrsmAhead; ++q) stage(q);
+  }
   constexpr int NI = kTrsmRW / 8;
   const int wr = warp * kTrsmRW;
+  int staged = 0, ready = 0;
   for (int jt = 0; jt < nt; ++jt) {
-    cp_async_wait<kTrsmAhead - 1>();
+    if constexpr (kStreamed) {
+      if (ready < min(nt, jt + kTrsmAhead)) {
+        if (tid == 0) {
+          int v = ld_acquire_gpu(progress + task.kframe);
+          while (v <= jt) { __nanosleep(32); v = ld_acquire_gpu(progress + task.kframe); }
+          s_ready = v;
+        }
+        __syncthreads();
+        ready = s_ready;
+      }
+      for (; staged < min(ready, jt + kTrsmAhead); ++staged) stage(staged);
+      cp_async_wait_upto3(staged - 1 - jt);
+    } else {
+      cp_async_wait<kTrsmAhead - 1>();
+    }
     __syncthreads();
     const double* ls = Ls + (size_t)(jt % kTrsmAhead) * 16 * ld; const double* dsm = Ds + (jt % kTrsmAhead) * 320;
     double acc[NI][2][2];
@@ -613,8 +648,9 @@
         if (r < rows) *reinterpret_cast<double2*>(&X[(size_t)(m0 + r) * npad + cidx]) = v;
       }
     __syncthreads();
-    stage(jt + kTrsmAhead);
-  }
+    if constexpr (!kStreamed) stage(jt + kTrsmAhead);
+  }
+  if constexpr (kStreamed) asm volatile("griddepcontrol.wait;" ::: "memory");
 }
 
 
@@ -694,10 +730,8 @@
 struct SubTask { int type; int blk; int r; int k; int chunk; };
 struct SubCounters { int* ticket; int* fin; int* fdone; int* bin; int* bdone; const int* fin_need; const int* bin_need; };
 
-__device__ __forceinline__ int ld_acquire_gpu(const int* p) { int v; asm volatile("ld.acquire.gpu.global.s32 %0, [%1];" : "=r"(v) : "l"(p) : "memory"); return v; }
 __device__ __forceinline__ void sub_wait(const int* c, int need) { while (ld_acquire_gpu(c) < need) __nanosleep(20); }
 
-__device__ __forceinline__ void red_release_add(int* p, int v) { asm volatile("red.release.gpu.global.add.s32 [%0], %1;" ::"l"(p), "r"(v) : "memory"); }
 __device__ __forceinline__ double2 ldcg2(const double* p) { return __ldcg(reinterpret_cast<const double2*>(p)); }
 
 __global__ void __launch_bounds__(kSubThreads) k_substitution(const double* __restrict__ invL, const double* __restrict__ T, double* rhs, double* y, double* x,
diff --git a/robust_cvd_b200/csrc/rcvd_update.cuh b/robust_cvd_b200/csrc/rcvd_update.cuh
--- a/robust_cvd_b200/csrc/rcvd_update.cuh
+++ b/robust_cvd_b200/csrc/rcvd_update.cuh
@@ -121,6 +121,7 @@
                                                                const UpdItem* __restrict__ items, int nitems, const int2* __restrict__ pairs,
                                                                int npad, int neff, int rb, int dbg) {
   extern __shared__ __align__(1024) unsigned char ring[];
+  asm volatile("griddepcontrol.launch_dependents;" ::: "memory");
   if (smem_u32(ring) & 1023u) __trap();
   constexpr int kUpdStages = UpdShape<TEAMS>::stages;
   const int tile_bytes = rb * 128, stage_bytes = 2 * tile_bytes;
diff --git a/robust_cvd_b200/solver.py b/robust_cvd_b200/solver.py
--- a/robust_cvd_b200/solver.py
+++ b/robust_cvd_b200/solver.py
@@ -155,7 +155,7 @@
         return order, Lf, Li
 
     LINEAR_PATHS = ("potrf_smem", "potrf_panel", "trsm_ll4", "trsm_ll2", "trsm_gemm", "update_tma1", "update_tma2", "update_gemm",
-                    "substitution_levels", "substitution_fused", "trinv", "other", "update_tma1_multi_item")
+                    "substitution_levels", "substitution_fused", "trinv", "other", "update_tma1_multi_item", "trsm_ll_streamed")
 
     def linear_paths(self):
         out = (C.c_int64 * len(self.LINEAR_PATHS))()
```

New measurement: 77.54 million (median of 6 runs). 1.05x the previous value.
